# falcon-computing/bwa-flow

Measured on AMD Instinct MI355X. Metric: million reads/sec (2×150 bp PE) end-to-end align; SW-extend GCUPS at 1/2/4/8 MI355X, higher is better.
Workload: dtype int32

## Files before the change

### bwa-flow_amd/csrc/capi.hip

```cpp
#include <hip/hip_runtime.h>
#include <string.h>

#include <algorithm>
#include <chrono>
#include <cstdio>
#include <mutex>
#include <new>
#include <string>
#include <thread>
#include <vector>

#include "batch_host.h"
#include "ctx.h"
#include "engine.h"
#include "regpost.h"

using namespace bwagpu;

namespace {


__global__ void side_probe_spin(uint64_t ticks) {
  const uint64_t t0 = __builtin_amdgcn_s_memrealtime();
  while (__builtin_amdgcn_s_memrealtime() - t0 < ticks) __builtin_amdgcn_s_sleep(8);
// ... 49 lines not shown
    off[nr] = part[t];
    h_off[nr] = part[t];
  }
}

__global__ void __launch_bounds__(256) dense_copy_kernel(const bwagpu_alnreg_t* __restrict__ out,
                                                         const int32_t* __restrict__ n,
                                                         const int32_t* __restrict__ off,
                                                         const int32_t* __restrict__ rco,
                                                         const int32_t* __restrict__ cso, int nr,
                                                         bwagpu_alnreg_t* __restrict__ dense) {
  constexpr int kW = (int)(sizeof(bwagpu_alnreg_t) / 8);
  const int r = (int)((blockIdx.x * 256u + threadIdx.x) >> 4), l = (int)(threadIdx.x & 15);
  if (r >= nr) return;
  const int words = n[r] * kW;
  const uint2* src = reinterpret_cast<const uint2*>(out + cso[rco[r]]);
  uint2* dst = reinterpret_cast<uint2*>(dense + off[r]);
  for (int w = l; w < words; w += 16) dst[w] = src[w];
}

}

namespace {

bool make_opt(const bwagpu_opt_t* o, DevOpt* d, std::string* why) {
  if (!o) { *why = "opt is NULL"; return false; }
  if (o->e_del <= 0 || o->e_ins <= 0) { *why = "gap extension penalties must be > 0"; return false; }
  if (o->w < 0 || o->a < 0) { *why = "negative band width or match score"; return false; }
  if (o->a > 127 || o->e_del > 65535 || o->e_ins > 65535 || o->o_del < 0 || o->o_del > 65535 || o->o_ins < 0 ||
      o->o_ins > 65535 || o->pen_clip5 < 0 || o->pen_clip5 >= (1 << 20) || o->pen_clip3 < 0 ||
      o->pen_clip3 >= (1 << 20) || o->w > (1 << 20)) {
    *why = "scoring option out of range";
    return false;
  }
  memset(d, 0, sizeof(*d));
  d->a = o->a;
  d->o_del = o->o_del;
  d->e_del = o->e_del;
  d->o_ins = o->o_ins;
  d->e_ins = o->e_ins;
  d->oe_del = o->o_del + o->e_del;
  d->oe_ins = o->o_ins + o->e_ins;
  d->pen_clip5 = o->pen_clip5;
  d->pen_clip3 = o->pen_clip3;
  d->w = o->w;
  d->zdrop = o->zdrop;
  int mx = 0;
  for (int i = 0; i < 25; ++i) mx = std::max<int>(mx, o->mat[i]);
  d->max_mat = mx;
  d->row_bound = 1;
  memcpy(d->mat, o->mat, 25);
  for (int q = 0; q < 5; ++q) {
    uint32_t w = 0;
    for (int t = 0; t < 4; ++t) w |= (uint32_t)(uint8_t)o->mat[t * 5 + q] << (8 * t);
    d->qprof[q] = w;
    d->qprof4[q] = o->mat[20 + q];
  }
  return true;
}

int create_common(int device, const bwagpu_opt_t* opt, const bwagpu_bns_t* bns, bwagpu_ctx_t** out,
                  bwagpu_ctx_t** made) {
  if (!out || !bns || bns->l_pac <= 0 || bns->n_seqs <= 0 || !bns->ann_offset || !bns->ann_len)
    return BWAGPU_E_INVAL;
  int n = 0;
  if (hipGetDeviceCount(&n) != hipSuccess || n <= 0) return BWAGPU_E_NODEVICE;
  if (device < 0 || device >= n) return BWAGPU_E_NODEVICE;
  bwagpu_ctx_t* ctx = new (std::nothrow) bwagpu_ctx_t();
  if (!ctx) return BWAGPU_E_NOMEM;
  std::string why;
  if (!make_opt(opt, &ctx->opt, &why)) {
    delete ctx;
    return BWAGPU_E_INVAL;
  }
  ctx->device = device;
  ctx->opt_b = opt->b;
  ctx->ext_form = set_ext_form(-1);
  ctx->ext_short = ext_short_default();
  ctx->ext_short_fill = ext_short_fill_default();
  ctx->light_pack = light_pack_default();
  ctx->ungapped = ungapped_default();
  ctx->ungapped_right = ungapped_right_default();
  ctx->emu_finish = emu_finish_default();
  *made = ctx;
  HIPC(hipSetDevice(device), "hipSetDevice");
  HIPC(hipMalloc(&ctx->d_ann_off, sizeof(int64_t) * bns->n_seqs), "hipMalloc(ann_offset)");
  HIPC(hipMalloc(&ctx->d_ann_len, sizeof(int32_t) * bns->n_seqs), "hipMalloc(ann_len)");
  HIPC(hipMemcpy(ctx->d_ann_off, bns->ann_offset, sizeof(int64_t) * bns->n_seqs, hipMemcpyHostToDevice),
       "upload ann_offset");
  HIPC(hipMemcpy(ctx->d_ann_len, bns->ann_len, sizeof(int32_t) * bns->n_seqs, hipMemcpyHostToDevice),
       "upload ann_len");
  for (auto& s : ctx->slot) {
    HIPC(hipEventCreate(&s.ev0), "hipEventCreate");
    HIPC(hipEventCreate(&s.ev1), "hipEventCreate");
    HIPC(hipEventCreate(&s.ev2), "hipEventCreate");
    HIPC(hipEventCreate(&s.ev3), "hipEventCreate");
  }
  ctx->ref.l_pac = bns->l_pac;
  ctx->ref.n_seqs = bns->n_seqs;
  ctx->ref.ann_offset = ctx->d_ann_off;
  ctx->ref.ann_len = ctx->d_ann_len;
  return BWAGPU_OK;
}

std::vector<Slot*> all_slots(bwagpu_ctx_t* ctx) {
  std::vector<Slot*> v;
  for (auto& x : ctx->slot) v.push_back(&x);
  for (auto& x : ctx->dev_scratch) v.push_back(&x);
  v.push_back(&ctx->ch_slot);
  return v;
}

void destroy_ctx(bwagpu_ctx_t* ctx) {
  if (!ctx) return;
  (void)hipSetDevice(ctx->device);
  std::vector<hipStream_t> busy = ctx->side_graveyard;
  for (Slot* s : all_slots(ctx)) busy.insert(busy.end(), {s->stream, s->spec.side});
  busy.insert(busy.end(), ctx->dev_stream, ctx->dev_stream + BWAGPU_NUM_SLOTS);
  busy.insert(busy.end(), ctx->a2_st, ctx->a2_st + bwagpu_ctx::kA2Streams);
  busy.insert(busy.end(), ctx->ch_cs.side, ctx->ch_cs.side + 2);
  for (hipStream_t x : busy)
    if (x) (void)hipStreamSynchronize(x);
  if (ctx->sdh_done) (void)hipEventSynchronize(ctx->sdh_done);
  if (ctx->r2d_done && ctx->r2d_pending) (void)hipEventSynchronize(ctx->r2d_done);
  std::vector<hipStream_t> own = ctx->side_graveyard;
  own.insert(own.end(), ctx->a2_st, ctx->a2_st + bwagpu_ctx::kA2Streams);
  own.insert(own.end(), ctx->ch_cs.side, ctx->ch_cs.side + 2);
  for (hipStream_t x : own)
    if (x) (void)hipStreamDestroy(x);
  std::vector<hipEvent_t> evs = ctx->prof_ev;
  evs.insert(evs.end(), {ctx->sdh_done, ctx->r2d_done, ctx->r2d_ev[0], ctx->r2d_ev[1], ctx->a2_fork, ctx->ch_cs.fork,
                         ctx->ch_cs.join[0], ctx->ch_cs.join[1]});
  evs.insert(evs.end(), ctx->a2_join, ctx->a2_join + bwagpu_ctx::kA2Streams);
  evs.insert(evs.end(), ctx->rs_ev, ctx->rs_ev + 4 * kRescueMaxRounds);
  for (hipEvent_t e : evs)
    if (e) (void)hipEventDestroy(e);
  if (ctx->own_pac && ctx->d_pac) (void)hipFree(ctx->d_pac);
  if (ctx->d_ann_off) (void)hipFree(ctx->d_ann_off);
  if (ctx->d_ann_len) (void)hipFree(ctx->d_ann_len);
  delete ctx;
}

bool use_read_kernels() {
  const char* e = getenv("BWAGPU_C2A_PATH");
  return e && (strcmp(e, "fast") == 0 || strcmp(e, "read") == 0);
}

size_t variant_lds(const DevOpt& o, int v, int lq_max) {
  const Variant& vk = kVariants[v];
  const int lqv = std::min(lq_max, vk.max_len());
  const int tb = tb_bytes_for(o, std::max(lqv, 1));
  return vk.kind == VK_FAST ? (size_t)(kBlock / 64) * fast_wave_lds(tb) : (size_t)tb * (kBlock / vk.G);
}

}

int bwagpu::check_lds(bwagpu_ctx_t* ctx, int lq_max) {
  if (!use_read_kernels()) {
    if (spec_redo_cap(tb_bytes_for(ctx->opt, std::max(lq_max, 1))) < 64)
      return fail(ctx, BWAGPU_E_UNSUPPORTED, "LDS row buffer too large for these options (w, pen_clip, read length)");
    return BWAGPU_OK;
  }
  for (int v = 0; v < kNumVariants; ++v) {
    if (variant_lds(ctx->opt, v, lq_max) > 64 * 1024)
      return fail(ctx, BWAGPU_E_UNSUPPORTED, "LDS row buffer too large for these options (w, pen_clip, read length)");
  }
// ... 37 lines not shown
    hipStream_t c = nullptr;
    if ((e = hipStreamCreateWithFlags(&c, hipStreamNonBlocking)) != hipSuccess) break;
    bool ok = true;
    for (hipStream_t a : avoid)
      if (!streams_concurrent(c, a)) {
        ok = false;
        break;
      }
    if (ok) pick = c;
    else tried.push_back(c);
  }
  for (hipStream_t c : tried) (void)hipStreamDestroy(c);
  if (e != hipSuccess) return e;
  s.spec.side = pick;
  s.side_chosen = true;
  *snap = s.spec;
  return hipSuccess;
}

int enqueue_spec(bwagpu_ctx_t* ctx, Slot& s, const DevBatch& db, int lq_max, bwagpu_alnreg_t* d_out, int32_t* d_n,
                 int64_t* d_stats, hipStream_t st) {
  const size_t nc = (size_t)std::max(db.n_chains, 1), ns = (size_t)std::max(db.n_seeds, 1),
               nr = (size_t)std::max(db.n_reads, 1);
  const size_t n_tasks = kSpecBins * (nc + (kSpecRounds - 1) * ns);
  SpecArgs a;
  HIPC(s.d_win.get(a.win, nc), "hipMalloc(win)");
  HIPC(s.d_cread.get(a.chain_read, nc), "hipMalloc(chain_read)");
  HIPC(s.d_prog.get(a.prog, ns), "hipMalloc(prog)");
  HIPC(s.d_ext.get(a.ext, ns), "hipMalloc(ext)");
  HIPC(s.d_tasks.get(a.tasks, n_tasks), "hipMalloc(tasks)");
  HIPC(s.d_ctr.get(a.ctr, SPC_WORDS), "hipMalloc(ctr)");
  HIPC(s.d_regpos.get(a.regpos, ns), "hipMalloc(regpos)");
  HIPC(s.d_skipf.get(a.skipf, ns), "hipMalloc(skipf)");
  HIPC(s.d_heavy.get(a.heavy, nr), "hipMalloc(heavy)");
  HIPC(s.d_redo.get(a.redo, nr), "hipMalloc(redo)");
  HIPC(s.d_rbits.get(a.rbits, 2 * (nr / 32 + 1)), "hipMalloc(rbits)");
  a.fbits = a.rbits + (nr / 32 + 1);
  HIPC(s.d_rlist.get(a.rlist, nr), "hipMalloc(rlist)");
  HIPC(s.d_desc.get(a.rdesc, nr), "hipMalloc(desc)");
  HIPC(s.d_schain.get(a.seedchain, ns), "hipMalloc(seedchain)");
  HIPC(s.d_hinfo.get(a.hinfo, nr), "hipMalloc(hinfo)");
  HIPC(s.d_cov.get(a.cov, ns), "hipMalloc(cov)");
  HIPC(s.d_hflag.get(a.hflag, ns), "hipMalloc(hflag)");
  HIPC(s.d_colent.get(a.colent, ns), "hipMalloc(colent)");
  HIPC(s.d_longc.get(a.longc, nc), "hipMalloc(longc)");
  HIPC(s.d_qh.get(a.qh, kQHWords), "hipMalloc(qh)");
  HIPC(s.d_sorth.get(a.sorth, kSortWords), "hipMalloc(sorth)");
  HIPC(s.d_stasks.get(a.stasks, n_tasks), "hipMalloc(stasks)");
  HIPC(s.d_ftask.get(a.ftask, n_tasks), "hipMalloc(ftask)");
  HIPC(s.d_ftaskR.get(a.ftaskR, n_tasks), "hipMalloc(ftaskR)");
  a.ung = nullptr;
  if (ctx->ungapped && ctx->opt.row_bound) HIPC(s.d_ung.get(a.ung, n_tasks), "hipMalloc(ung)");
  a.ungt = nullptr;
  if (a.ung && ctx->ungapped_right) HIPC(s.d_ungt.get(a.ungt, n_tasks), "hipMalloc(ungt)");
  HIPC(s.d_mat.get(a.mat, (size_t)std::max<int64_t>(1 << 20, 16 * (int64_t)ns)), "hipMalloc(mat)");
  a.mat_words = (int64_t)(s.d_mat.cap / sizeof(uint64_t));
  static const int ext_prefetch = [] {
    const char* e = getenv("BWAGPU_EXT_PREFETCH");
    return e ? std::max(0, atoi(e)) : 0;
  }();
  a.ext_prefetch = ext_prefetch;
  static const int risky_first = [] {
    const char* e = getenv("BWAGPU_LIGHT_RISKY_FIRST");
    return e && e[0] == '1';
  }();
  a.risky_first = risky_first;
  static const int emu_strict = [] {
    const char* e = getenv("BWAGPU_EMU_STRICT");
    return !(e && e[0] == '0');
  }();
  a.emu_strict = emu_strict;
  a.light_pack = ctx->light_pack;
  a.emu_finish = ctx->emu_finish;
  a.out = d_out;
  a.out_n = d_n;
  a.stats = d_stats;
  SpecStreams ss;
  HIPC(choose_side(ctx, s, st, &ss), "side stream");
  a.lq_bound = lq_max;
  const int tb = tb_bytes_for(ctx->opt, std::max(lq_max, 1));
  ss.form = ctx->ext_form;
  ss.short_q = ctx->ext_short;
  ss.short_fill = ctx->ext_short_fill;
  ss.pool = ctx->prof_ev.empty() ? nullptr : ctx->prof_ev.data();
  ss.pool_n = (int)ctx->prof_ev.size();
  ss.pool_used = &ctx->prof_used;
  HIPC(launch_spec_clear(a, db.n_reads, db.n_seeds, st), "spec clear");
  HIPC(launch_spec_chain2aln(ctx->opt, ctx->ref, db, a, tb, lq_max, st, ss), "spec chain2aln launch");
  return BWAGPU_OK;
}

}

int bwagpu::enqueue_chain2aln(bwagpu_ctx_t* ctx, Slot& s, const DevBatch& db, int lq_max, bwagpu_alnreg_t* d_out,
                              int32_t* d_n, int64_t* d_stats, hipStream_t st) {
  if (!use_read_kernels()) return enqueue_spec(ctx, s, db, lq_max, d_out, d_n, d_stats, st);
  ChainWin* win = nullptr;
  bwagpu_seed_t* prog = nullptr;
  ReadDesc* desc = nullptr;
  C2AArgs a;
  HIPC(s.d_win.get(win, (size_t)db.n_chains), "hipMalloc(win)");
  HIPC(s.d_srt.get(a.srt, (size_t)db.n_seeds), "hipMalloc(srt)");
  HIPC(s.d_prog.get(prog, (size_t)db.n_seeds), "hipMalloc(prog)");
  const size_t nr = (size_t)std::max(db.n_reads, 1);
  HIPC(s.d_desc.get(desc, nr), "hipMalloc(desc)");
  HIPC(s.d_lists.ensure(2 * sizeof(int32_t) * nr), "hipMalloc(lists)");
  int32_t* bins = s.d_lists.as<int32_t>();
  int32_t* read_list = bins + nr;
  HIPC(s.d_counts.get(a.counts, kCountWords), "hipMalloc(counts)");
  HIPC(hipMemsetAsync(a.counts, 0, sizeof(int32_t) * kCountWords, st), "memset counts");
  if (db.n_reads) HIPC(hipMemsetAsync(d_n, 0, sizeof(int32_t) * db.n_reads, st), "memset out_n");
  HIPC(launch_chain_prep(ctx->opt, ctx->ref, db, win, a.srt, prog, d_stats, st), "chain_prep launch");
  HIPC(launch_read_order(db, bins, a.counts + kHistOff, a.counts, desc, read_list, d_stats, st), "read order launch");
  a.read_list = read_list;
  a.desc = desc;
  a.win = win;
  a.prog = prog;
  a.out = d_out;
  a.out_n = d_n;
  a.stats = d_stats;
  for (int v = 0; v < kNumVariants; ++v) {
    const int lqv = std::min(lq_max, kVariants[v].max_len());
    const int tb = tb_bytes_for(ctx->opt, std::max(lqv, 1));
    HIPC(launch_chain2aln(v, ctx->opt, ctx->ref, db, db.n_reads, tb, a, st), "chain2aln launch");
  }
  return BWAGPU_OK;
}

extern "C" {

int bwagpu_abi_version(void) { return BWAGPU_ABI_VERSION; }

int bwagpu_device_count(int* n) {
  if (!n) return BWAGPU_E_INVAL;
  int k = 0;
  if (hipGetDeviceCount(&k) != hipSuccess) k = 0;
  *n = k;
  return k > 0 ? BWAGPU_OK : BWAGPU_E_NODEVICE;
}

int bwagpu_create(int device, const bwagpu_opt_t* opt, const bwagpu_bns_t* bns, const uint8_t* pac_host,
                  bwagpu_ctx_t** out) {
  if (!pac_host) return BWAGPU_E_INVAL;
  bwagpu_ctx_t* ctx = nullptr;
  int rc = create_common(device, opt, bns, out, &ctx);
  if (rc == BWAGPU_OK) {
    const size_t pac_bytes = (size_t)(bns->l_pac / 4 + 1);
    hipError_t e = hipMalloc(&ctx->d_pac, pac_bytes);
    if (e == hipSuccess) {
      ctx->own_pac = true;
      e = hipMemcpy(ctx->d_pac, pac_host, pac_bytes, hipMemcpyHostToDevice);
    }
    if (e != hipSuccess) rc = hip_fail(ctx, e, "pac upload");
    ctx->ref.pac = (const uint8_t*)ctx->d_pac;
  }
  if (rc != BWAGPU_OK) {
    destroy_ctx(ctx);
    return rc;
  }
  *out = ctx;
  return BWAGPU_OK;
}

int bwagpu_create_resident(int device, const bwagpu_opt_t* opt, const bwagpu_bns_t* bns, const void* pac_device,
                           bwagpu_ctx_t** out) {
  if (!pac_device) return BWAGPU_E_INVAL;
// ... 391 lines not shown
  if (!ctx) return BWAGPU_E_INVAL;
  const int prev = ctx->ext_short;
  if (q >= 0) ctx->ext_short = q > 63 ? 63 : q;
  return prev;
}

int bwagpu_ctx_ext_short_fill(bwagpu_ctx_t* ctx, int percent) {
  if (!ctx) return BWAGPU_E_INVAL;
  const int prev = ctx->ext_short_fill;
  if (percent >= 0) ctx->ext_short_fill = percent > 100000 ? 100000 : percent;
  return prev;
}

int bwagpu_ctx_light_pack(bwagpu_ctx_t* ctx, int on) {
  if (!ctx) return BWAGPU_E_INVAL;
  const int prev = ctx->light_pack;
  if (on >= 0) ctx->light_pack = on != 0;
  return prev;
}

int bwagpu_debug_spec_short(bwagpu_ctx_t* ctx, void* stream, int64_t* out) {
  if (!ctx || !out) return BWAGPU_E_INVAL;
  int32_t c[SPC_WORDS];
  if (int rc = spec_ctr_words(ctx, stream, c)) return rc;
  out[0] = c[SPC_SHORT_N];
  for (int r = 0; r < 2; ++r) {
    const int l = r * kSpecBins;
    out[1 + 4 * r] = c[SPC_LCNT + l];
    out[2 + 4 * r] = c[SPC_LLONG + l];
    out[3 + 4 * r] = c[SPC_RCNT + l];
    out[4 + 4 * r] = c[SPC_RLONG + l];
  }
  return BWAGPU_OK;
}

int bwagpu_ctx_ungapped(bwagpu_ctx_t* ctx, int on) {
  if (!ctx) return BWAGPU_E_INVAL;
  const int prev = ctx->ungapped;
  if (on >= 0) ctx->ungapped = on ? 1 : 0;
  return prev;
}

int bwagpu_debug_spec_ungapped(bwagpu_ctx_t* ctx, void* stream, int64_t* out) {
  if (!ctx || !out) return BWAGPU_E_INVAL;
  int32_t c[SPC_WORDS];
  if (int rc = spec_ctr_words(ctx, stream, c)) return rc;
  for (int r = 0; r < kSpecRounds; ++r) {
    out[4 * r + 0] = c[SPC_UNG_N + r];
    out[4 * r + 1] = c[SPC_UNG_Q + r];
    out[4 * r + 2] = out[4 * r + 3] = 0;
    for (int bin = 0; bin < kSpecBins; ++bin) {
      out[4 * r + 2] += c[SPC_LCNT + r * kSpecBins + bin];
      out[4 * r + 3] += c[SPC_RCNT + r * kSpecBins + bin];
    }
  }
  return BWAGPU_OK;
}

int bwagpu_ctx_ungapped_right(bwagpu_ctx_t* ctx, int on) {
  if (!ctx) return BWAGPU_E_INVAL;
  const int prev = ctx->ungapped_right;
  if (on >= 0) ctx->ungapped_right = on ? 1 : 0;
  return prev;
}

int bwagpu_debug_spec_ungapped_right(bwagpu_ctx_t* ctx, void* stream, int64_t* out) {
  if (!ctx || !out) return BWAGPU_E_INVAL;
  int32_t c[SPC_WORDS];
  if (int rc = spec_ctr_words(ctx, stream, c)) return rc;
  for (int r = 0; r < kSpecRounds; ++r) {
    out[2 * r + 0] = c[SPC_UNGR_N + r];
    out[2 * r + 1] = c[SPC_UNGR_Q + r];
  }
  return BWAGPU_OK;
}

int bwagpu_ctx_emu_finish(bwagpu_ctx_t* ctx, int on) {
  if (!ctx) return BWAGPU_E_INVAL;
  const int prev = ctx->emu_finish;
  if (on >= 0) ctx->emu_finish = on ? 1 : 0;
  return prev;
}

int bwagpu_debug_spec_finish(bwagpu_ctx_t* ctx, void* stream, int64_t* out) {
  if (!ctx || !out) return BWAGPU_E_INVAL;
  int32_t c[SPC_WORDS];
  if (int rc = spec_ctr_words(ctx, stream, c)) return rc;
  out[0] = c[SPC_FIN_NAR];
  out[1] = c[SPC_FIN_WIDE];
  out[2] = c[SPC_LIST_N];
  out[3] = c[SPC_LIGHT_N];
  return BWAGPU_OK;
}

int bwagpu_ctx_row_bound(bwagpu_ctx_t* ctx, int on) {
  if (!ctx) return BWAGPU_E_INVAL;
  const int prev = ctx->opt.row_bound;
  if (on >= 0) ctx->opt.row_bound = on ? 1 : 0;
  return prev;
}

int bwagpu_debug_ext_kernel(bwagpu_ctx_t* ctx, int32_t lq_max) {
  if (!ctx || lq_max < 1 || lq_max > BWAGPU_MAX_READ_LEN) return BWAGPU_E_INVAL;
  return ext_kernel_for(ctx->opt, ctx->ext_form, tb_bytes_for(ctx->opt, lq_max));
}

int bwagpu_prof_start(bwagpu_ctx_t* ctx, int max_launches) {
  if (!ctx || max_launches < 0) return BWAGPU_E_INVAL;
  HIPC(hipSetDevice(ctx->device), "hipSetDevice");
  for (hipEvent_t e : ctx->prof_ev) HIPC(hipEventSynchronize(e), "hipEventSynchronize");
  for (hipEvent_t e : ctx->prof_ev) (void)hipEventDestroy(e);
  ctx->prof_ev.clear();
  ctx->prof_used = 0;
  for (int i = 0; i < 2 * max_launches; ++i) {
    hipEvent_t e = nullptr;
    HIPC(hipEventCreate(&e), "hipEventCreate");
    ctx->prof_ev.push_back(e);
  }
  return BWAGPU_OK;
}

int bwagpu_prof_read(bwagpu_ctx_t* ctx, double* total_ms, int32_t* launches) {
  if (!ctx || !total_ms || !launches) return BWAGPU_E_INVAL;
  HIPC(hipSetDevice(ctx->device), "hipSetDevice");
  double t = 0;
  for (int i = 0; i + 1 < ctx->prof_used; i += 2) {
    HIPC(hipEventSynchronize(ctx->prof_ev[i + 1]), "hipEventSynchronize");
    float ms = 0;
    HIPC(hipEventElapsedTime(&ms, ctx->prof_ev[i], ctx->prof_ev[i + 1]), "hipEventElapsedTime");
    t += ms;
  }
  *total_ms = t;
  *launches = ctx->prof_used / 2;
  return BWAGPU_OK;
}

int bwagpu_prof_intervals(bwagpu_ctx_t* ctx, double* start_ms, double* end_ms, int32_t max, int32_t* n) {
  if (!ctx || !n || max < 0 || (max && (!start_ms || !end_ms))) return BWAGPU_E_INVAL;
  HIPC(hipSetDevice(ctx->device), "hipSetDevice");
  int k = 0;
  for (int i = 0; i + 1 < ctx->prof_used && k < max; i += 2, ++k) {
    HIPC(hipEventSynchronize(ctx->prof_ev[i + 1]), "hipEventSynchronize");
    float a = 0, b = 0;
    HIPC(hipEventElapsedTime(&a, ctx->prof_ev[0], ctx->prof_ev[i]), "hipEventElapsedTime");
    HIPC(hipEventElapsedTime(&b, ctx->prof_ev[0], ctx->prof_ev[i + 1]), "hipEventElapsedTime");
    start_ms[k] = a;
    end_ms[k] = b;
  }
  *n = k;
  return BWAGPU_OK;
}

int bwagpu_last_stats(const bwagpu_ctx_t* ctx, int slot, bwagpu_stats_t* out) {
  if (!ctx || !out || slot < 0 || slot >= BWAGPU_NUM_SLOTS) return BWAGPU_E_INVAL;
  *out = ctx->slot[slot].last;
  return BWAGPU_OK;
}

}
```

### bwa-flow_amd/csrc/ctx.h

```cpp
#pragma once
#include <hip/hip_runtime.h>
#include <stdint.h>

#include <algorithm>
#include <atomic>
#include <chrono>
#include <mutex>
#include <string>
#include <type_traits>
#include <vector>

#include "bwagpu.h"
#include "chain.h"
#include "engine.h"
#include "rescue.h"
#include "seed.h"
#include "stage_host.h"
#include "task_host.h"

namespace bwagpu {

inline std::atomic<int64_t> g_live_bufs{0}, g_live_bytes{0};

template <bool kPinned>
// ... 31 lines not shown
      g_live_bytes.fetch_sub((int64_t)cap, std::memory_order_relaxed);
    }
    p = nullptr;
    cap = 0;
  }
  template <class T>
  T* as() const { return (T*)p; }
};
using DevBuf = GrowBuf<false>;
using HostBuf = GrowBuf<true>;
static_assert(!std::is_copy_constructible<DevBuf>::value, "a copy would free the buffer twice");

struct Slot {
  hipStream_t stream = nullptr;
  std::once_flag stream_once;
  hipError_t stream_err = hipSuccess;
  hipEvent_t ev0 = nullptr, ev1 = nullptr, ev2 = nullptr, ev3 = nullptr;
  DevBuf d_in, d_win, d_srt, d_prog, d_desc, d_out, d_n, d_stats, d_lists, d_counts;
  DevBuf d_cread, d_ext, d_tasks, d_ctr, d_regpos, d_skipf, d_heavy, d_redo, d_rbits, d_rlist;
  DevBuf d_schain, d_hinfo, d_mat, d_cov, d_hflag, d_colent, d_qh, d_longc, d_sorth, d_stasks, d_ftask, d_ftaskR, d_ung, d_ungt;
  SpecStreams spec;
  bool side_chosen = false;
  HostBuf h_in, h_out, h_n, h_stats;
  HostBuf h_dense, h_off;
  DevBuf d_off;
  size_t in_rco = 0, in_cso = 0;
  bool slot_view = false;
  bool busy = false;
  bool has_results = false;
  bool kept = false;
  std::vector<int32_t> keep_rco, keep_cso;
  int32_t n_reads = 0, n_chains = 0, n_seeds = 0;
  std::chrono::steady_clock::time_point t_submit;
  bwagpu_stats_t last{};
  int64_t h2d = 0, d2h = 0;
  ~Slot() {
    for (hipStream_t x : {stream, spec.side})
      if (x) {
        (void)hipStreamSynchronize(x);
        (void)hipStreamDestroy(x);
      }
    for (hipEvent_t e : {ev0, ev1, ev2, ev3, spec.fork, spec.join})
      if (e) (void)hipEventDestroy(e);
  }
};

inline hipError_t lazy_stream(Slot& s, hipStream_t* st) {
  std::call_once(s.stream_once, [&s] { s.stream_err = hipStreamCreateWithFlags(&s.stream, hipStreamNonBlocking); });
  *st = s.stream;
  return s.stream_err;
}

struct Staging {
  DevBuf regs, out_regs;
  DevBuf seq;
  DevBuf seq_off, reg_off, out_off;
  DevBuf n, out_n, n_pri, status, n_sw, mapq, sel;
  DevBuf pes;
};

}

struct bwagpu_ctx {
  using DevBuf = bwagpu::DevBuf;
  using HostBuf = bwagpu::HostBuf;
  using Slot = bwagpu::Slot;
  int device = 0;
  std::mutex side_mu;
  std::vector<hipStream_t> callers, side_graveyard;
  bwagpu::DevOpt opt{};
  bwagpu::DevRef ref{};
  bool own_pac = false;
  void* d_pac = nullptr;
  int64_t* d_ann_off = nullptr;
  int32_t* d_ann_len = nullptr;
  int watchdog_ms = 10000;
  int ext_form = 0;
  int ext_short = 0;
  int light_pack = 0;
  int ext_short_fill = 0;
  int ungapped = 1;
  int ungapped_right = 1;
  int emu_finish = 1;
  Slot slot[BWAGPU_NUM_SLOTS];
  hipStream_t dev_stream[BWAGPU_NUM_SLOTS] = {};
  Slot dev_scratch[BWAGPU_NUM_SLOTS];
  DevBuf ex_tasks, ex_list, ex_q, ex_t, ex_res, ex_stats;
  DevBuf a2_tasks, a2_q, a2_t, a2_out, a2_scratch, a2_lists, a2_counts, a2_boff;
  DevBuf r2_tasks, r2_q, r2_out, r2_cig, r2_md, r2_lists, r2_z, r2_stats;
  DevBuf r2d_keys, r2d_lists, r2d_tab, r2d_z, r2d_sums;
  HostBuf r2d_htab;
  hipEvent_t r2d_done = nullptr, r2d_ev[2] = {};
  bool r2d_pending = false, r2d_timing = false, r2d_timed = false;
  double r2d_wait_ms = 0, r2d_call_ms = 0;
  int32_t r2d_jobs = 0;
  static constexpr int kA2Streams = 4;
  hipStream_t a2_st[kA2Streams] = {};
  hipEvent_t a2_fork = nullptr, a2_join[kA2Streams] = {};
  DevBuf bwt_words, sa_d, sa_in, sa_out, occ_d, sup_d, sa_full;
  bwagpu::DevBwt bwt{};
  bool has_bwt = false;
  DevBuf sd_off, sd_seq, sd_out, sd_n, sd_scratch, sd_poff, sd_pack, sd_heavy, sd_dbg;
  DevBuf ch_npos, ch_posoff, ch_frac, ch_nout, ch_noseed, ch_nsw, ch_need, ch_swtab, ch_alt;
  DevBuf ch_kpos, ch_rbeg, ch_qinfo, ch_label, ch_score, ch_slist, ch_ord, ch_chains, ch_nodes;
  DevBuf ch_ochains, ch_oslist, ch_bins, ch_dbg;
  DevBuf ch_swoff, ch_swtasks, ch_swt, ch_swskip, ch_swres, ch_swscr;
  DevBuf ch_ocoff, ch_osoff, ch_rco, ch_cso, ch_rid, ch_cfrac, ch_out, ch_seeds;
  DevBuf ch_regoff, ch_regc;
  HostBuf chh_tot, chh_rco, chh_cso, chh_chains, chh_seeds, chh_regs, chh_n;
  HostBuf sdh_in;
  hipEvent_t sdh_done = nullptr;
  Slot ch_slot;
  bwagpu::ChainStreams ch_cs{};
  bool has_alt = false;
  bwagpu::Staging stg;
  int opt_b = 0;
  bwagpu_postopt_t post_opt{};
  int32_t post_flags = 0;
  int64_t post_id0 = 0;
  DevBuf rp_stats;
  DevBuf pe_isize, pe_cnt;
  DevBuf rs_pair, rs_soff, rs_tab, rs_toff, rs_boff, rs_qpool, rs_ctr, rs_scr;
  DevBuf rs_tasks[bwagpu::kRescueMaxRounds], rs_tpool[bwagpu::kRescueMaxRounds], rs_res[bwagpu::kRescueMaxRounds];
  int32_t rescue_drop = 0;
  hipEvent_t rs_ev[4 * bwagpu::kRescueMaxRounds] = {};
  int rs_ev_rounds = 0;
  hipStream_t rs_ev_stream = nullptr;
  DevBuf ps_scratch, ps_log, ps_erfc;
  bool ps_log_ready = false;
  DevBuf st_buf, st_start, st_q, st_tasks, st_lists, st_seen, st_ctr, st_out;
  int seed_budget = 1024;
  int sup_shift = 32;
  int dev_read_len = BWAGPU_MAX_READ_LEN;
  int fail_after = -1, fail_code = 0;
  std::vector<hipEvent_t> prof_ev;
  int prof_used = 0;
  std::string err;
};

namespace bwagpu {

inline int fail(bwagpu_ctx_t* c, int code, const std::string& msg) {
  if (c) c->err = msg;
  return code;
}

inline int hip_fail(bwagpu_ctx_t* c, hipError_t e, const char* what) {
  std::string m = std::string(what) + ": " + hipGetErrorString(e);
  if (e == hipErrorOutOfMemory || e == hipErrorMemoryAllocation) return fail(c, BWAGPU_E_NOMEM, m);
  return fail(c, BWAGPU_E_DEVICE, m);
}

#define HIPC(call, what)                             \
  do {                                               \
    hipError_t e_ = (call);                          \
    if (e_ != hipSuccess) return hip_fail(ctx, e_, what); \
  } while (0)
#define TRY(call)                     \
  do {                                \
    if (int rc_ = (call)) return rc_; \
  } while (0)

inline int refuse(bwagpu_ctx_t* c, int code, const char* why) { return why && *why ? fail(c, code, why) : code; }

inline int entry_stream(bwagpu_ctx_t* ctx, void* stream, hipStream_t* st) {
  HIPC(hipSetDevice(ctx->device), "hipSetDevice");
// ... 130 lines not shown
```

### bwa-flow_amd/csrc/engine.h

```cpp
#pragma once
#include <hip/hip_runtime.h>
#include <stdint.h>

#include "bwagpu.h"
#include "bwagpu_debug.h"
#include "pure.h"
#include "spec_plan.h"
#include "ungapped.h"

namespace bwagpu {

struct ReadDesc {
  int64_t qoff;
  int32_t rd;
  int32_t lq;
  int32_t c0;
  int32_t nch;
  int32_t s0;
  int32_t ns;
};

struct ChainWin {
  int64_t lo, hi;
};
// ... 17 lines not shown
  const int32_t* ann_len;
};

enum { ST_CELLS = 0, ST_ROWS = 1, ST_CALLS = 2, ST_ERR = 3, ST_N = 4 };
enum { ERR_RID = 1, ERR_LEN = 2, ERR_A2_RANGE = 4 };

constexpr int kFastMaxSeeds = 32;
constexpr int kFastMaxChains = 32;
constexpr int kSeqLds = 256;
constexpr int kNumVariants = 3;
extern const Variant kVariants[kNumVariants];
constexpr int kHistOff = 128;
constexpr int kCountWords = kHistOff + kNumVariants * 256;

hipError_t launch_chain_prep(const DevOpt& o, const DevRef& ref, const DevBatch& b, ChainWin* win, uint64_t* srt,
                             bwagpu_seed_t* prog, int64_t* stats, hipStream_t st);
hipError_t launch_read_order(const DevBatch& b, int32_t* bins, int32_t* hist, int32_t* counts, ReadDesc* desc,
                             int32_t* list, int64_t* stats, hipStream_t st);
struct C2AArgs {
  const int32_t* read_list;
  const ReadDesc* desc;
  int32_t* counts;
  const ChainWin* win;
  uint64_t* srt;
  const bwagpu_seed_t* prog;
  bwagpu_alnreg_t* out;
  int32_t* out_n;
  int64_t* stats;
};
hipError_t launch_chain2aln(int variant, const DevOpt& o, const DevRef& ref, const DevBatch& b, int32_t max_list,
                            int tb_bytes, const C2AArgs& a, hipStream_t st);
size_t fast_wave_lds(int tb);

hipError_t launch_extend(int variant, bool t5, const DevOpt& o, int32_t n_tasks,
                         const bwagpu_ext_task_t* tasks, const int32_t* task_list, int32_t n_list,
                         const uint8_t* qpool, const uint8_t* tpool, int tb_bytes,
                         bwagpu_ext_result_t* res, int64_t* stats, hipStream_t st);
hipError_t launch_extend4(const DevOpt& o, const bwagpu_ext_task_t* tasks, const int32_t* task_list, int32_t n_list,
                          const uint8_t* qpool, const uint8_t* tpool, int tb_bytes, bwagpu_ext_result_t* res,
                          int64_t* stats, hipStream_t st);

struct SeedExt {
  int64_t rb, re;
  int32_t qb, qe, score, truesc, w;
  int32_t cells, rows, calls;
};

constexpr int kSpecRounds = 3;
constexpr int kOrderLane = 8;
constexpr int kSelLight = 64;
constexpr int kSelRegLds = 256;
constexpr int kSelMatMaxSeeds = 4096;
enum {
  SPC_CNT = 0,
  SPC_HEAVY_N = 16,
  SPC_SEL_CUR = 17,
  SPC_REDO_N = 20,
  SPC_SPEC64 = 24,
  SPC_MISS = 26,
  SPC_MATW64 = 28,
  SPC_HCOLS = 30,
  SPC_LONG_N = 31,
  SPC_LCNT = 64,
  SPC_RCNT = 73,
  SPC_LIGHT_CUR = 82,
  SPC_LLONG = 84,
  SPC_RLONG = 93,
  SPC_SHORT_N = 102,
  SPC_UNG_N = 103,
  SPC_UNG_Q = 106,
  SPC_FIN_NAR = 109,
  SPC_FIN_WIDE = 110,
  SPC_LIST_N = 111,
  SPC_LIGHT_N = 112,
  SPC_UNGR_N = 113,
  SPC_UNGR_Q = 116,
  SPC_WORDS = 128
};
constexpr int kQHStride = 32;
constexpr int kQHShort = 2 * kSpecRounds * kSpecBins * 8 * kQHStride;
constexpr int kQHWords = 2 * kQHShort;
constexpr int kSortKeys = 1024;
constexpr int kSortWordsR = kSpecRounds * 2 * kSortKeys;
constexpr int kSortWords = 2 * kSortWordsR;
__host__ __device__ inline size_t spec_list_off(int list, int n_chains, int n_seeds) {
  const int round = list / kSpecBins, bin = list % kSpecBins;
  return round == 0 ? (size_t)bin * n_chains
                    : (size_t)kSpecBins * n_chains + ((size_t)(round - 1) * kSpecBins + bin) * n_seeds;
}
struct FatTask {
  int64_t rbeg, qoff;
  int32_t pos;
  int32_t dlo, dhi;
  uint32_t qls;
};
static_assert(sizeof(FatTask) == 32, "FatTask layout");
static_assert(BWAGPU_MAX_READ_LEN < 1024, "FatTask packs qbeg / len / lq in 10 bits each");
struct UngRec {
  struct Side {
    int32_t ok;
    UngappedSide s;
  } side[2];
};
static_assert(sizeof(UngRec) == 32, "UngRec layout");
struct UngTask {
  int64_t rbeg;
  int32_t pos;
  uint32_t qls;
};
static_assert(sizeof(UngTask) == 16, "UngTask layout");
struct SpecArgs {
  int lq_bound;
  ChainWin* win;
  int32_t* chain_read;
  bwagpu_seed_t* prog;
  SeedExt* ext;
  int2* tasks;
  int32_t* ctr;
  int32_t* regpos;
  int32_t* skipf;
  int32_t* heavy;
  int32_t* redo;
  uint32_t* rbits;
  uint32_t* fbits;
  int32_t* rlist;
  ReadDesc* rdesc;
  int32_t* seedchain;
  int4* hinfo;
  int32_t* colent;
  int32_t* longc;
  uint64_t* mat;
  int64_t mat_words;
  int32_t* cov;
  int32_t* hflag;
  int32_t* qh;
  int32_t* sorth;
  int2* stasks;
  FatTask* ftask;
  FatTask* ftaskR;
  UngRec* ung;
  UngTask* ungt;
  int risky_first;
  int emu_strict;
  int light_pack;
  int emu_finish;
  int ext_prefetch;
  bwagpu_alnreg_t* out;
  int32_t* out_n;
  int64_t* stats;
};
struct SpecStreams {
  hipStream_t side = nullptr;
  hipEvent_t fork = nullptr, join = nullptr;
  hipEvent_t* pool = nullptr;
  int pool_n = 0;
  int* pool_used = nullptr;
  int form = 0;
  int short_q = 0;
  int short_fill = 0;
};
int ungapped_default();
int ungapped_right_default();
int emu_finish_default();
int set_ext_form(int form);
int ext_short_default();
int ext_short_fill_default();
int light_pack_default();
int ext_kernel_for(const DevOpt& o, int form, int tb_bytes);
hipError_t launch_spec_clear(const SpecArgs& a, int n_reads, int n_seeds, hipStream_t st);
hipError_t launch_spec_chain2aln(const DevOpt& o, const DevRef& ref, const DevBatch& b, const SpecArgs& a,
                                 int tb_bytes, int lq_max, hipStream_t st, const SpecStreams& ss);
size_t spec_select_lds(int tb_bytes);
int spec_redo_cap(int tb_bytes);

struct StreamTask {
  bwagpu_seed_t s;
  int64_t lo, hi;
  int64_t qoff;
  int32_t lq, pad_;
};
enum { STR_ERR_RECORD = 1, STR_ERR_TASK = 2, STR_ERR_DUP = 4, STR_ERR_SEED = 8, STR_ERR_BASE = 16 };
enum { kStrDecoded = 4, kStrMax = 5, kStrErr = 6, kStrHeads = 64 };
constexpr int kStrCtrWords = kStrHeads + kSpecBins * 8 * kQHStride;
struct StreamArgs {
  const int32_t* buf;
  const int64_t* rstart;
  int32_t n_reads, cap;
  int64_t l_pac;
  uint8_t* qpool;
  StreamTask* tasks;
  int32_t* lists;
  int32_t* seen;
  int32_t* ctr;
  int32_t* out;
};
hipError_t launch_sw_stream(const DevOpt& o, const DevRef& ref, const StreamArgs& a, int tb_bytes, hipStream_t st);

hipError_t set_trace(void* dev_ptr);
hipError_t set_trace_spec(void* dev_ptr);

}
```

### bwa-flow_amd/csrc/spec.hip

```cpp
#include "spec_dev.h"

namespace bwagpu {

__device__ uint32_t* g_trace = nullptr;
hipError_t set_trace_spec(void* p) { return hipMemcpyToSymbol(HIP_SYMBOL(g_trace), &p, sizeof(p)); }


__global__ void __launch_bounds__(256) spec_chain_kernel(DevOpt o, DevRef ref, DevBatch b, SpecArgs a) {
  sel_prio();
  const int c = blockIdx.x * blockDim.x + threadIdx.x;
  bool task = false, longc = false;
  int bin = 0, s0 = 0;
  if (c < b.n_chains) {
    const int rd = a.chain_read[c];
    s0 = b.chain_seed_off[c];
    const int ns = b.chain_seed_off[c + 1] - s0;
    const int lq = (int)(b.seq_off[rd + 1] - b.seq_off[rd]);
    if (ns <= 0) {
      a.win[c] = ChainWin{0, 0};
    } else {
      int64_t wlo = ref.l_pac << 1, whi = 0;
      longc = ns > kOrderLane;
      if (!longc) {
        uint64_t key[kOrderLane];
// ... 811 lines not shown
enum { SEL_EMULATE = 0, SEL_FINAL = 1, SEL_REDO = 2 };
struct RegRec {
  int64_t rb, re;
  int32_t qb, qe, w, seedlen0;
};
constexpr int kSelHeavyLds = 64 * 1024;
constexpr int kSelExtCache = 256;
__host__ __device__ constexpr int sel_light_wave_lds() { return kSelLight * (int)sizeof(RegRec); }
__host__ __device__ constexpr int sel_heavy_cap(int mode, int tb) {
  return (kSelHeavyLds - 4 * (BWAGPU_MAX_READ_LEN + 1) - kSelExtCache * (int)(sizeof(SeedExt) + sizeof(bwagpu_seed_t)) -
          (mode == SEL_REDO ? 2 * tb : 0)) / (int)sizeof(RegRec);
}

constexpr int kMglN = BWAGPU_MAX_READ_LEN + 1;

__device__ __forceinline__ bool seed_near(const int32_t* MG, const bwagpu_seed_t& s, const RegRec& p) {
  const int qd1 = s.qbeg - p.qb;
  const int64_t rd1 = s.rbeg - p.rb;
  const int g1 = MG[min(max(qd1 < rd1 ? qd1 : (int)rd1, 0), kMglN - 1)];
  const int bw1 = g1 < p.w ? g1 : p.w;
  const int qd2 = p.qe - (s.qbeg + s.len);
  const int64_t rd2 = p.re - (s.rbeg + s.len);
  const int g2 = MG[min(max(qd2 < rd2 ? qd2 : (int)rd2, 0), kMglN - 1)];
  const int bw2 = g2 < p.w ? g2 : p.w;
  return (qd1 - rd1 < bw1 && rd1 - qd1 < bw1) || (qd2 - rd2 < bw2 && rd2 - qd2 < bw2);
}

__device__ __forceinline__ void write_region(bwagpu_alnreg_t* dst, const SeedExt& e, int rid, int cov, int slen,
                                             float frac) {
  const int r = (int)(threadIdx.x & 63);
  const int dw = r < 21 ? r : 21;
  uint32_t v = 0;
  v = dw == 0 ? (uint32_t)e.rb : v;
  v = dw == 1 ? (uint32_t)((uint64_t)e.rb >> 32) : v;
  v = dw == 2 ? (uint32_t)e.re : v;
  v = dw == 3 ? (uint32_t)((uint64_t)e.re >> 32) : v;
  v = dw == 4 ? (uint32_t)e.qb : v;
  v = dw == 5 ? (uint32_t)e.qe : v;
  v = dw == 6 ? (uint32_t)rid : v;
  v = dw == 7 ? (uint32_t)e.score : v;
  v = dw == 8 ? (uint32_t)e.truesc : v;
  v = dw == 13 ? (uint32_t)e.w : v;
  v = dw == 14 ? (uint32_t)cov : v;
  v = dw == 17 ? (uint32_t)slen : v;
  v = dw == 19 ? __float_as_uint(frac) : v;
  reinterpret_cast<uint32_t*>(dst)[dw] = v;
}

__device__ __forceinline__ void put_regrec(RegRec* dst, const SeedExt& e, int slen) {
  const int r = (int)(threadIdx.x & 63);
  const int f = r < 8 ? r : 7;
  int32_t v = 0;
  v = f == 0 ? (int32_t)(uint32_t)e.rb : v;
  v = f == 1 ? (int32_t)((uint64_t)e.rb >> 32) : v;
  v = f == 2 ? (int32_t)(uint32_t)e.re : v;
  v = f == 3 ? (int32_t)((uint64_t)e.re >> 32) : v;
  v = f == 4 ? e.qb : v;
  v = f == 5 ? e.qe : v;
  v = f == 6 ? e.w : v;
  v = f == 7 ? slen : v;
  if (r < 8) reinterpret_cast<int32_t*>(dst)[f] = v;
  __builtin_amdgcn_fence(__ATOMIC_RELEASE, "wavefront");
  __builtin_amdgcn_wave_barrier();
  __builtin_amdgcn_fence(__ATOMIC_ACQUIRE, "wavefront");
}

__device__ __forceinline__ void trace_read(int pass, int n_reads, int rd, uint64_t t0, int ns, int nreg, int shape) {
  uint32_t* const tr = g_trace;
  if (!tr) return;
  const uint64_t t1 = __builtin_amdgcn_s_memrealtime();
  const int r = (int)(threadIdx.x & 63);
  const int d = r < 7 ? r : 7;
  uint32_t v = (uint32_t)shape;
  v = d == 0 ? (uint32_t)t0 : v;
  v = d == 1 ? (uint32_t)(t0 >> 32) : v;
  v = d == 2 ? (uint32_t)t1 : v;
  v = d == 3 ? (uint32_t)(t1 >> 32) : v;
  v = d == 4 ? (uint32_t)ns : v;
  v = d == 5 ? (uint32_t)nreg : v;
  v = d == 6 ? __builtin_amdgcn_s_getreg((31 << 11) | 20) : v;
  if (r < 8) tr[((size_t)pass * n_reads + rd) * 8 + d] = v;
}

template <int MODE, bool HEAVY>
__global__ void __launch_bounds__(64) spec_select_kernel(DevOpt o, DevRef ref, DevBatch b, SpecArgs a, int tb_bytes) {
  sel_prio();
  static_assert(HEAVY, "one-wave heavy shape only");
  constexpr bool WRITE = MODE != SEL_EMULATE;
  extern __shared__ __attribute__((aligned(16))) uint8_t lds[];
  const int r = (int)(threadIdx.x & 63);
  int32_t* const MG = reinterpret_cast<int32_t*>(lds);
  bwagpu_seed_t* const SC = reinterpret_cast<bwagpu_seed_t*>(lds + 4 * kMglN);
  SeedExt* const EC = reinterpret_cast<SeedExt*>(SC + kSelExtCache);
  RegRec* const R = reinterpret_cast<RegRec*>(EC + kSelExtCache);
  const int cap_reg = sel_heavy_cap(MODE, tb_bytes);
  uint8_t* const tbl = reinterpret_cast<uint8_t*>(R + cap_reg);
  uint8_t* const tbr = tbl + tb_bytes;
  for (int x = r; x < kMglN; x += 64) MG[x] = max_gap_len(o, x);
  Tally tl{0, 0, 0};
  const int n_list = uni(__hip_atomic_load(&a.ctr[MODE == SEL_REDO ? SPC_REDO_N : SPC_HEAVY_N], __ATOMIC_RELAXED,
                                           __HIP_MEMORY_SCOPE_AGENT));
  const int32_t* const hlist = MODE == SEL_REDO ? a.redo : a.heavy;
  for (;;) {
    int t = 0;
    if (r == 0) t = atomicAdd(&a.ctr[SPC_SEL_CUR + MODE], 1);
    t = uni(__shfl(t, 0, 64));
    if (t >= n_list) break;
    if (MODE != SEL_REDO && uni(a.hinfo[t].y) >= 0) continue;
    const int rd = uni(hlist[t]);
    const uint64_t t_start = g_trace ? __builtin_amdgcn_s_memrealtime() : 0;
    const ReadDesc d = uniform_desc(a.rdesc[rd]);
    if (d.lq > a.lq_bound) continue;
    const uint8_t* const q = b.seq + d.qoff;
    const int rep_lim = (int)floor(.1 * d.lq) + 1;
    bool redo = false;
    Tally rt{0, 0, 0};
    int nreg = 0, n_inline = 0;
    for (int c = d.c0; c < d.c0 + d.nch && !redo; ++c) {
      const int s0 = uni(b.chain_seed_off[c]), ns = uni(b.chain_seed_off[c + 1]) - s0;
      if (ns == 0) continue;
      ChainWin cw = a.win[c];
      cw.lo = uni64(cw.lo);
      cw.hi = uni64(cw.hi);
      if (cw.hi < cw.lo) continue;
      const int rid = uni(b.chain_rid[c]);
      const float frac = __int_as_float(uni(__float_as_int(b.chain_frac_rep[c])));
      const bool big = ns > kSelExtCache;
      for (int i = r; i < min(ns, kSelExtCache); i += 64) {
        bwagpu_seed_t v = a.prog[s0 + i];
        v.pad_ = v.pad_ != 0 ? 1 : 0;
        SC[i] = v;
        const uint32_t* src = reinterpret_cast<const uint32_t*>(a.ext + s0 + i);
        uint32_t* dst = reinterpret_cast<uint32_t*>(EC + i);
#pragma unroll
        for (int w = 0; w < 12; ++w) dst[w] = __hip_atomic_load(src + w, __ATOMIC_RELAXED, __HIP_MEMORY_SCOPE_WORKGROUP);
      }
      if (big)
        for (int i = r; i < ns; i += 64)
          __hip_atomic_store(&a.skipf[s0 + i], a.prog[s0 + i].pad_ != 0 ? 1 : 0, __ATOMIC_RELAXED,
                             __HIP_MEMORY_SCOPE_WORKGROUP);
      mem_fence_group();
      auto seed_at = [&](int i) -> bwagpu_seed_t { return i < kSelExtCache ? SC[i] : a.prog[s0 + i]; };
      auto flag_at = [&](int i) -> int {
        return i < kSelExtCache ? SC[i].pad_
                                : __hip_atomic_load(&a.skipf[s0 + i], __ATOMIC_RELAXED, __HIP_MEMORY_SCOPE_WORKGROUP);
      };
      auto set_flag = [&](int i, int f) {
        if (r == 0) {
          if (i < kSelExtCache) SC[i].pad_ |= f;
          else __hip_atomic_store(&a.skipf[s0 + i], f | 0, __ATOMIC_RELAXED, __HIP_MEMORY_SCOPE_WORKGROUP);
        }
        mem_fence_group();
      };
      for (int k = 0; k < ns; ++k) {
        const bwagpu_seed_t s = uni_seed(seed_at(k));
        bool hit = false;
        for (int base = 0; base < nreg && !hit; base += 64) {
          const int i = min(base + r, nreg - 1);
          RegRec p;
          if (i < cap_reg) {
            p = R[i];
          } else {
            const int pp = __hip_atomic_load(&a.regpos[d.s0 + i], __ATOMIC_RELAXED, __HIP_MEMORY_SCOPE_WORKGROUP);
            const SeedExt* pe = a.ext + pp;
            p.rb = __hip_atomic_load(&pe->rb, __ATOMIC_RELAXED, __HIP_MEMORY_SCOPE_WORKGROUP);
            p.re = __hip_atomic_load(&pe->re, __ATOMIC_RELAXED, __HIP_MEMORY_SCOPE_WORKGROUP);
            p.qb = __hip_atomic_load(&pe->qb, __ATOMIC_RELAXED, __HIP_MEMORY_SCOPE_WORKGROUP);
            p.qe = __hip_atomic_load(&pe->qe, __ATOMIC_RELAXED, __HIP_MEMORY_SCOPE_WORKGROUP);
            p.w = __hip_atomic_load(&pe->w, __ATOMIC_RELAXED, __HIP_MEMORY_SCOPE_WORKGROUP);
            p.seedlen0 = a.prog[pp].len;
          }
          const bool inside = base + r < nreg &&
                              !(s.rbeg < p.rb || s.rbeg + s.len > p.re || s.qbeg < p.qb || s.qbeg + s.len > p.qe) &&
                              !(s.len - p.seedlen0 >= rep_lim);
          if (__builtin_amdgcn_ballot_w64(inside) == 0) continue;
          hit = __builtin_amdgcn_ballot_w64(inside && seed_near(MG, s, p)) != 0;
        }
        if (hit) {
          const int len95 = uni((int)ceil(s.len * .95));
          bool ov = false;
          for (int base = 0; base < k && !ov; base += 64) {
            const int i = min(base + r, k - 1);
            const bwagpu_seed_t t = seed_at(i);
            const bool tsk = (flag_at(i) & 1) != 0;
            const bool a1 = s.qbeg <= t.qbeg && s.qbeg + s.len - t.qbeg >= s.len >> 2 && (int64_t)(t.qbeg - s.qbeg) != t.rbeg - s.rbeg;
            const bool b1 = t.qbeg <= s.qbeg && t.qbeg + t.len - s.qbeg >= s.len >> 2 && (int64_t)(s.qbeg - t.qbeg) != s.rbeg - t.rbeg;
            ov = __builtin_amdgcn_ballot_w64(base + r < k && !tsk && t.len >= len95 && (a1 || b1)) != 0;
          }
          if (!ov) {
            set_flag(k, 1);
            continue;
          }
        }
        const int pos = s0 + k;
        const SeedExt* const pe = k < kSelExtCache ? EC + k : a.ext + pos;
        SeedExt e;
        e.calls = uni(__hip_atomic_load(&pe->calls, __ATOMIC_RELAXED, __HIP_MEMORY_SCOPE_WORKGROUP));
        if (e.calls == 0) {
          if constexpr (MODE == SEL_REDO) {
            e = extend_seed<16>(o, ref, s, d.lq, q, cw, tbl, tbr);
            store_ext(a.ext + pos, e);
            mem_fence_group();
            if (r == 0) atomicAdd(&a.ctr[SPC_MISS], 1);
            ++n_inline;
          } else if constexpr (MODE == SEL_EMULATE) {
            set_flag(k, 2);
            continue;
          } else {
            const int list = 2 * kSpecBins + spec_bin(d.lq);
            if (r == 0) {
              const int p = atomicAdd(&a.ctr[SPC_CNT + list], 1);
              a.tasks[spec_list_off(list, b.n_chains, b.n_seeds) + p] = make_int2(pos, c);
              a.redo[atomicAdd(&a.ctr[SPC_REDO_N], 1)] = rd;
            }
            redo = true;
            break;
          }
        } else {
          e.rb = uni64(__hip_atomic_load(&pe->rb, __ATOMIC_RELAXED, __HIP_MEMORY_SCOPE_WORKGROUP));
          e.re = uni64(__hip_atomic_load(&pe->re, __ATOMIC_RELAXED, __HIP_MEMORY_SCOPE_WORKGROUP));
          e.qb = uni(__hip_atomic_load(&pe->qb, __ATOMIC_RELAXED, __HIP_MEMORY_SCOPE_WORKGROUP));
          e.qe = uni(__hip_atomic_load(&pe->qe, __ATOMIC_RELAXED, __HIP_MEMORY_SCOPE_WORKGROUP));
          e.score = uni(__hip_atomic_load(&pe->score, __ATOMIC_RELAXED, __HIP_MEMORY_SCOPE_WORKGROUP));
          e.truesc = uni(__hip_atomic_load(&pe->truesc, __ATOMIC_RELAXED, __HIP_MEMORY_SCOPE_WORKGROUP));
          e.w = uni(__hip_atomic_load(&pe->w, __ATOMIC_RELAXED, __HIP_MEMORY_SCOPE_WORKGROUP));
          e.cells = uni(__hip_atomic_load(&pe->cells, __ATOMIC_RELAXED, __HIP_MEMORY_SCOPE_WORKGROUP));
          e.rows = uni(__hip_atomic_load(&pe->rows, __ATOMIC_RELAXED, __HIP_MEMORY_SCOPE_WORKGROUP));
        }
        if constexpr (WRITE) {
          long long cov = 0;
          for (int base = 0; base < ns; base += 64) {
            const int i = base + r;
            const bwagpu_seed_t t = seed_at(min(i, ns - 1));
            const bool in = i < ns && t.qbeg >= e.qb && t.qbeg + t.len <= e.qe && t.rbeg >= e.rb && t.rbeg + t.len <= e.re;
            cov += in ? t.len : 0;
          }
          cov = grp_sum64(cov, 64);
          write_region(a.out + d.s0 + nreg, e, rid, (int)cov, s.len, frac);
          rt.cells += e.cells;
          rt.rows += e.rows;
          rt.calls += e.calls - 1;
        }
        if (nreg < cap_reg) {
          put_regrec(R + nreg, e, s.len);
        } else {
          if (r == 0) __hip_atomic_store(&a.regpos[d.s0 + nreg], pos, __ATOMIC_RELAXED, __HIP_MEMORY_SCOPE_WORKGROUP);
          mem_fence_group();
        }
        ++nreg;
      }
      if constexpr (MODE == SEL_EMULATE) {
        const int list = kSpecBins + spec_bin(d.lq);
        for (int base = 0; base < ns; base += 64) {
          const int i = base + r;
          const bool pnd = i < ns && (flag_at(min(i, ns - 1)) & 2) != 0;
          const int p = wave_append(&a.ctr[SPC_CNT + list], pnd);
          if (p >= 0) a.tasks[spec_list_off(list, b.n_chains, b.n_seeds) + p] = make_int2(s0 + i, c);
        }
      }
    }
    trace_read(MODE, b.n_reads, rd, t_start, d.ns, nreg, 2 | (MODE == SEL_REDO ? n_inline << 4 : 0));
    if constexpr (WRITE) {
      if (!redo) {
        a.out_n[rd] = nreg;
        tl.cells += rt.cells;
        tl.rows += rt.rows;
        tl.calls += rt.calls;
      }
    }
  }
  if constexpr (WRITE) {
    if (r != 0) tl = Tally{0, 0, 0};
    block_stats<64>(tl, a.stats);
  }
}

#ifndef BWAGPU_LIGHT_INLINE
#define BWAGPU_LIGHT_INLINE 1
#endif
template <int MODE>
__device__ __forceinline__ bool light_read(const DevOpt& o, const DevRef& ref, const DevBatch& b, const SpecArgs& a,
                                           const int32_t* MG, uint8_t* tbl, uint8_t* tbr, int rd, const ReadDesc& d,
                                           Tally& tl) {
  constexpr bool WRITE = MODE != SEL_EMULATE;
  const int r = (int)(threadIdx.x & 63);
  const uint64_t lt_mask = r ? (~0ull >> (64 - r)) : 0ull;
  const uint64_t t_start = g_trace ? __builtin_amdgcn_s_memrealtime() : 0;
  bool finished = false;
    for (;;) {
    const int ci = min(r, max(d.nch - 1, 0)), si = min(r, d.ns - 1);
    const int cs_l = b.chain_seed_off[d.c0 + ci] - d.s0, ce_l = b.chain_seed_off[d.c0 + ci + 1] - d.s0;
    const ChainWin cw_l = a.win[d.c0 + ci];
    const int rid_l = b.chain_rid[d.c0 + ci];
    const float fr_l = b.chain_frac_rep[d.c0 + ci];
    const bwagpu_seed_t sd = a.prog[d.s0 + si];
    const SeedExt x = a.ext[d.s0 + si];
    int cid = 0, rid = 0;
    float frac = 0.f;
    bool vchain = false;
    for (int c = 0; c < d.nch; ++c) {
      const int cs = __builtin_amdgcn_readlane(cs_l, c), ce = __builtin_amdgcn_readlane(ce_l, c);
      const bool in = r >= cs && r < ce;
      const bool ok = readlane64(cw_l.hi, c) >= readlane64(cw_l.lo, c);
      cid = in ? c : cid;
      vchain = in ? ok : vchain;
      rid = in ? __builtin_amdgcn_readlane(rid_l, c) : rid;
      frac = in ? __int_as_float(__builtin_amdgcn_readlane(__float_as_int(fr_l), c)) : frac;
    }
    const bool present = r < d.ns && vchain;
    const bool computed = present && x.calls != 0;
    const uint64_t present_m = __builtin_amdgcn_ballot_w64(present);
    const uint64_t computed_m = __builtin_amdgcn_ballot_w64(computed);
    const uint64_t pad_m = __builtin_amdgcn_ballot_w64(r < d.ns && sd.pad_ != 0);
    const int rep_lim = (int)floor(.1 * d.lq) + 1;
    const int S = d.ns <= 8 ? 8 : d.ns <= 16 ? 16 : d.ns <= 32 ? 32 : 64;
    const int lgS = S == 8 ? 3 : S == 16 ? 4 : S == 32 ? 5 : 6;
    const int npass = (S * S) >> 6;
    uint32_t c_lo = 0, c_hi = 0, o_lo = 0, o_hi = 0;
    int cov = 0;
    const int j = r & (S - 1);
    const int jl = min(j, d.ns - 1) << 2;
    const int64_t j_rbeg = (int64_t)((uint64_t)(uint32_t)__builtin_amdgcn_ds_bpermute(jl, (int)(sd.rbeg >> 32)) << 32 |
                                     (uint32_t)__builtin_amdgcn_ds_bpermute(jl, (int)sd.rbeg));
    const int j_qbeg = __builtin_amdgcn_ds_bpermute(jl, sd.qbeg), j_len = __builtin_amdgcn_ds_bpermute(jl, sd.len);
    const int j_cid = __builtin_amdgcn_ds_bpermute(jl, cid);
    const bool j_pad = __builtin_amdgcn_ds_bpermute(jl, sd.pad_) != 0;
    const bool j_done = __builtin_amdgcn_ds_bpermute(jl, computed ? 1 : 0) != 0;
    RegRec pj;
    pj.rb = (int64_t)((uint64_t)(uint32_t)__builtin_amdgcn_ds_bpermute(jl, (int)(x.rb >> 32)) << 32 |
                      (uint32_t)__builtin_amdgcn_ds_bpermute(jl, (int)x.rb));
    pj.re = (int64_t)((uint64_t)(uint32_t)__builtin_amdgcn_ds_bpermute(jl, (int)(x.re >> 32)) << 32 |
                      (uint32_t)__builtin_amdgcn_ds_bpermute(jl, (int)x.re));
    pj.qb = __builtin_amdgcn_ds_bpermute(jl, x.qb);
    pj.qe = __builtin_amdgcn_ds_bpermute(jl, x.qe);
    pj.w = __builtin_amdgcn_ds_bpermute(jl, x.w);
    pj.seedlen0 = j_len;
    for (int it = 0; it < npass; ++it) {
      const int k = (it << (6 - lgS)) + (r >> lgS);
      const int kl = min(k, d.ns - 1) << 2;
      bwagpu_seed_t sk;
      sk.rbeg = (int64_t)((uint64_t)(uint32_t)__builtin_amdgcn_ds_bpermute(kl, (int)(sd.rbeg >> 32)) << 32 |
                          (uint32_t)__builtin_amdgcn_ds_bpermute(kl, (int)sd.rbeg));
      sk.qbeg = __builtin_amdgcn_ds_bpermute(kl, sd.qbeg);
      sk.len = __builtin_amdgcn_ds_bpermute(kl, sd.len);
      const int k_cid = __builtin_amdgcn_ds_bpermute(kl, cid);
      const bool valid = k < d.ns && j < d.ns;
      const bool inside = valid && j < k && j_done &&
                          !(sk.rbeg < pj.rb || sk.rbeg + sk.len > pj.re || sk.qbeg < pj.qb || sk.qbeg + sk.len > pj.qe) &&
                          !(sk.len - j_len >= rep_lim);
      uint64_t cm = __builtin_amdgcn_ballot_w64(inside);
      if (cm) cm = __builtin_amdgcn_ballot_w64(inside && seed_near(MG, sk, pj));
      const int len95 = (int)ceil(sk.len * .95);
// ... 484 lines not shown
      if (MODE == SEL_EMULATE) {
        const bool a1 = s.qbeg <= sc.qbeg && s.qbeg + s.len - sc.qbeg >= s.len >> 2 &&
                        (int64_t)(sc.qbeg - s.qbeg) != sc.rbeg - s.rbeg;
        const bool b1 = sc.qbeg <= s.qbeg && sc.qbeg + sc.len - s.qbeg >= s.len >> 2 &&
                        (int64_t)(s.qbeg - sc.qbeg) != s.rbeg - sc.rbeg;
        const uint64_t om =
            __builtin_amdgcn_ballot_w64(j < k && cc == ck && sc.pad_ == 0 && sc.len >= len95 && (a1 || b1));
        if (r == 0) a.mat[woff + tri_off(ns) + tri_off(k) + w] = om;
      }
      if (k_cov)
        cov += (j < ns && cc == ck && sc.qbeg >= kqb && sc.qbeg + sc.len <= kqe && sc.rbeg >= krb &&
                sc.rbeg + sc.len <= kre) ? sc.len : 0;
    }
    if (k_cov) {
      for (int w = nlow; w < nw; ++w) {
        const int j = 64 * w + r, jj = min(j, ns - 1);
        const bwagpu_seed_t sc = a.prog[d.s0 + jj];
        const int cc = a.seedchain[d.s0 + jj];
        cov += (j < ns && cc == ck && sc.qbeg >= kqb && sc.qbeg + sc.len <= kqe && sc.rbeg >= krb &&
                sc.rbeg + sc.len <= kre) ? sc.len : 0;
      }
      cov = (int)grp_sum64(cov, 64);
      if (r == 0) a.cov[d.s0 + k] = cov;
    } else if (MODE == SEL_EMULATE) {
      if (r == 0) a.cov[d.s0 + k] = -1;
    }
    hi = hin;
  }
}

__device__ __forceinline__ uint64_t lane64(uint64_t v, int l) { return (uint64_t)readlane64((int64_t)v, l); }

constexpr int kScanLds = 64 * 1024;

__device__ __forceinline__ void heavy_fill_missing(const DevOpt& o, const DevRef& ref, const DevBatch& b,
                                                   const SpecArgs& a, const ReadDesc& d, int k, int ns,
                                                   uint64_t* C, uint8_t* tbl, uint8_t* tbr) {
  const int r = (int)(threadIdx.x & 63);
  const bwagpu_seed_t sk = uni_seed(a.prog[d.s0 + k]);
  const int ck = uni(a.seedchain[d.s0 + k]);
  ChainWin cw = a.win[ck];
  cw.lo = uni64(cw.lo);
  cw.hi = uni64(cw.hi);
  const SeedExt e = d.lq <= 192 ? extend_seed<3>(o, ref, sk, d.lq, b.seq + d.qoff, cw, tbl, tbr)
                                 : extend_seed<4>(o, ref, sk, d.lq, b.seq + d.qoff, cw, tbl, tbr);
  store_ext(a.ext + d.s0 + k, e);
  if (r == 0) atomicAdd(&a.ctr[SPC_MISS], 1);
  RegRec p;
  p.rb = e.rb;
  p.re = e.re;
  p.qb = e.qb;
  p.qe = e.qe;
  p.w = e.w;
  p.seedlen0 = sk.len;
  const int rep_lim = (int)floor(.1 * d.lq) + 1;
  int cov = 0;
  for (int base = 0; base < ns; base += 64) {
    const int j = base + r, jj = min(j, ns - 1);
    const bwagpu_seed_t sj = a.prog[d.s0 + jj];
    bool in = j > k && j < ns && !(sj.rbeg < p.rb || sj.rbeg + sj.len > p.re || sj.qbeg < p.qb || sj.qbeg + sj.len > p.qe) &&
              !(sj.len - sk.len >= rep_lim);
    if (in) {
      const int qd1 = sj.qbeg - p.qb;
      const int64_t rd1 = sj.rbeg - p.rb;
      const int g1 = max_gap_len(o, max(qd1 < rd1 ? qd1 : (int)rd1, 0));
      const int bw1 = g1 < p.w ? g1 : p.w;
      const int qd2 = p.qe - (sj.qbeg + sj.len);
      const int64_t rd2 = p.re - (sj.rbeg + sj.len);
      const int g2 = max_gap_len(o, max(qd2 < rd2 ? qd2 : (int)rd2, 0));
      const int bw2 = g2 < p.w ? g2 : p.w;
      in = (qd1 - rd1 < bw1 && rd1 - qd1 < bw1) || (qd2 - rd2 < bw2 && rd2 - qd2 < bw2);
    }
    if (in) C[tri_off(j) + (k >> 6)] |= 1ull << (k & 63);
    const int cj = a.seedchain[d.s0 + jj];
    cov += (j < ns && cj == ck && sj.qbeg >= p.qb && sj.qbeg + sj.len <= p.qe && sj.rbeg >= p.rb &&
            sj.rbeg + sj.len <= p.re) ? sj.len : 0;
  }
  cov = (int)grp_sum64(cov, 64);
  if (r == 0) a.cov[d.s0 + k] = cov;
  __builtin_amdgcn_fence(__ATOMIC_SEQ_CST, "workgroup");
  __builtin_amdgcn_wave_barrier();
}

template <int MODE>
__global__ void __launch_bounds__(64) spec_scan_kernel(DevOpt o, DevRef ref, DevBatch b, SpecArgs a, int tb_bytes) {
  sel_prio();
  constexpr bool WRITE = MODE != SEL_EMULATE;
  extern __shared__ __attribute__((aligned(16))) uint64_t M[];
  uint8_t* const tbl = reinterpret_cast<uint8_t*>(M) + kScanLds;
  uint8_t* const tbr = tbl + tb_bytes;
  const int r = (int)(threadIdx.x & 63);
  const uint64_t lt_mask = r ? (~0ull >> (64 - r)) : 0ull;
  const int nh = uni(__hip_atomic_load(&a.ctr[SPC_HEAVY_N], __ATOMIC_RELAXED, __HIP_MEMORY_SCOPE_AGENT));
  Tally tl{0, 0, 0};
  for (int t = (int)blockIdx.x; t < nh; t += (int)gridDim.x) {
    const int4 hi = a.hinfo[t];
    const int rd = uni(hi.x), woff = uni(hi.y), ns = uni(hi.w);
    if (woff < 0) continue;
    const uint64_t t_start = g_trace ? __builtin_amdgcn_s_memrealtime() : 0;
    const int nw = (ns + 63) >> 6;
    const ReadDesc d = uniform_desc(a.rdesc[rd]);
    if (d.lq > a.lq_bound) continue;
    const int64_t tw = tri_off(ns);
    const uint64_t* Cg = a.mat + woff;
    const bool staged = 2 * tw * 8 <= kScanLds;
    if (staged) {
      for (int i = r; i < 2 * tw; i += 64) M[i] = Cg[i];
      __builtin_amdgcn_fence(__ATOMIC_RELEASE, "wavefront");
      __builtin_amdgcn_wave_barrier();
      __builtin_amdgcn_fence(__ATOMIC_ACQUIRE, "wavefront");
    }
    uint64_t* C = staged ? M : a.mat + woff;
    const uint64_t* O = C + tw;
    uint64_t present_w = 0, computed_w = 0, skip_w = 0;
    for (int w = 0; w < nw; ++w) {
      const int j = 64 * w + r;
      const int f = j < ns ? a.hflag[d.s0 + j] : 0;
      const uint64_t pm = __builtin_amdgcn_ballot_w64(f & 1);
      const uint64_t cm = __builtin_amdgcn_ballot_w64((f & 3) == 3);
      const uint64_t km = __builtin_amdgcn_ballot_w64(f & 4);
      present_w = r == w ? pm : present_w;
      computed_w = r == w ? cm : computed_w;
      skip_w = r == w ? km : skip_w;
    }
    uint64_t ext_w = 0, pend_w = 0, unc_w = 0;
    const bool strict = MODE == SEL_EMULATE && a.emu_strict;
    int fp = ns;
    int miss = -1;
    for (int bw = 0; bw < nw && miss < 0; ++bw) {
      const int kb = 64 * bw, k = kb + r;
      const bool valid = k < ns;
      const int64_t row = tri_off(valid ? k : ns - 1);
      bool cb = false, cbc = false;
      for (int w = 0; w < bw; ++w) {
        const uint64_t x = C[row + w] & lane64(ext_w, w);
        cb |= x != 0;
        if (strict) cbc |= (x & ~lane64(unc_w, w)) != 0;
      }
      uint64_t cin = valid && r > 0 ? C[row + bw] : 0;
      bool need = valid && (cb || cin != 0), ob = false, ou = false;
      uint64_t oin = 0;
      if (__builtin_amdgcn_ballot_w64(need)) {
        if (need) {
          for (int w = 0; w < bw; ++w) {
            const uint64_t x = O[row + w];
            ob |= (x & ~lane64(skip_w, w)) != 0;
            if (strict) ou |= (x & lane64(unc_w, w)) != 0;
          }
          oin = r > 0 ? O[row + bw] : 0;
        }
      }
      const uint64_t pres = lane64(present_w, bw);
      uint64_t comp = lane64(computed_w, bw), skp = lane64(skip_w, bw), ext = 0, pend = 0, spend = 0;
      uint64_t uncb = 0;
      const int nb = min(64, ns - kb);
      bool resolved = false;
      {
        const uint64_t skp0 = skp;
        const bool prs = (pres >> r) & 1, cmp = (comp >> r) & 1;
        const bool cb_k = valid && cb, ob_k = valid && ob, cbc_k = valid && cbc, ou_k = valid && ou;
        uint64_t e = 0, sk = skp0, pn = 0, sp = 0, un = 0, lack = 0;
        for (int it = 0; it <= nb + 1; ++it) {
          bool is_skip = false, is_ext = false, is_pend = false, is_spend = false, is_unc = false, is_lack = false;
          if (prs) {
            if ((cb_k || (cin & e)) && !ob_k && !(oin & ~sk)) {
              is_skip = true;
              if (strict && (!(cbc_k || (cin & e & ~un)) || ou_k || (oin & un))) {
                is_unc = true;
                is_spend = !cmp;
              }
            } else if (!cmp) {
              if (MODE == SEL_EMULATE) is_pend = is_unc = true;
              else is_lack = true;
            } else {
              is_ext = true;
              is_unc = strict && (fp < k || (pn & lt_mask));
            }
// ... 96 lines not shown
          const int p = atomicAdd(&a.ctr[SPC_CNT + list], 1);
          a.tasks[spec_list_off(list, b.n_chains, b.n_seeds) + p] = make_int2(d.s0 + miss, a.seedchain[d.s0 + miss]);
          a.redo[atomicAdd(&a.ctr[SPC_REDO_N], 1)] = rd;
        }
        continue;
      }
      for (int w = 0; w < nw; ++w) {
        const uint64_t ew = (uint64_t)__builtin_amdgcn_readlane((uint32_t)(ext_w >> 32), w) << 32 |
                            (uint32_t)__builtin_amdgcn_readlane((uint32_t)ext_w, w);
        const int j = 64 * w + r;
        if ((ew >> r) & 1) {
          const int slot = nreg + (int)__popcll(ew & lt_mask);
          const SeedExt x = a.ext[d.s0 + j];
          const int c = a.seedchain[d.s0 + j];
          uint2* dst = reinterpret_cast<uint2*>(a.out + d.s0 + slot);
          dst[0] = make_uint2((uint32_t)x.rb, (uint32_t)((uint64_t)x.rb >> 32));
          dst[1] = make_uint2((uint32_t)x.re, (uint32_t)((uint64_t)x.re >> 32));
          dst[2] = make_uint2((uint32_t)x.qb, (uint32_t)x.qe);
          dst[3] = make_uint2((uint32_t)b.chain_rid[c], (uint32_t)x.score);
          dst[4] = make_uint2((uint32_t)x.truesc, 0u);
          dst[5] = make_uint2(0u, 0u);
          dst[6] = make_uint2(0u, (uint32_t)x.w);
          dst[7] = make_uint2((uint32_t)a.cov[d.s0 + j], 0u);
          dst[8] = make_uint2(0u, (uint32_t)a.prog[d.s0 + j].len);
          dst[9] = make_uint2(0u, __float_as_uint(b.chain_frac_rep[c]));
          dst[10] = make_uint2(0u, 0u);
          tl.cells += x.cells;
          tl.rows += x.rows;
          tl.calls += x.calls - 1;
        }
        nreg += (int)__popcll(ew);
      }
      if (r == 0) a.out_n[rd] = nreg;
    }
    trace_read(MODE, b.n_reads, rd, t_start, ns, nreg, 3);
  }
  if constexpr (WRITE) block_stats<64>(tl, a.stats);
}

constexpr int kScanGrid = 1024;

#ifndef BWAGPU_LIGHT_PACK_DEFAULT
#define BWAGPU_LIGHT_PACK_DEFAULT 1
#endif
int light_pack_default() {
  static const int v = [] {
    const char* e = getenv("BWAGPU_LIGHT_PACK");
    return e && e[0] ? (atoi(e) != 0 ? 1 : 0) : BWAGPU_LIGHT_PACK_DEFAULT;
  }();
  return v;
}
#ifndef BWAGPU_LIGHT_PACK_WGS_DEFAULT
#define BWAGPU_LIGHT_PACK_WGS_DEFAULT 2
#endif
static int light_pack_wgs() {
  static const int v = [] {
    const char* e = getenv("BWAGPU_LIGHT_PACK_WGS");
    return std::min(std::max(e && e[0] ? atoi(e) : BWAGPU_LIGHT_PACK_WGS_DEFAULT, 1), 64);
  }();
  return v;
}
#ifndef BWAGPU_LIGHT_LIST_DIV_DEFAULT
#define BWAGPU_LIGHT_LIST_DIV_DEFAULT 4
#endif
static int light_list_div() {
  static const int v = [] {
    const char* e = getenv("BWAGPU_LIGHT_LIST_DIV");
    return std::min(std::max(e && e[0] ? atoi(e) : BWAGPU_LIGHT_LIST_DIV_DEFAULT, 1), 64);
  }();
  return v;
}
static int device_cus() {
  int dev = 0, ncu = 0;
  if (hipGetDevice(&dev) != hipSuccess ||
      hipDeviceGetAttribute(&ncu, hipDeviceAttributeMultiprocessorCount, dev) != hipSuccess || ncu < 1)
    return 256;
  return ncu;
}

template <int MODE>
static void launch_select(const DevOpt& o, const DevRef& ref, const DevBatch& b, const SpecArgs& a, int tb_bytes,
                          hipStream_t st, const SpecStreams& ss) {
  hipStream_t hs = st;
  if (MODE != SEL_REDO && ss.side) {
    (void)hipEventRecord(ss.fork, st);
    (void)hipStreamWaitEvent(ss.side, ss.fork, 0);
    hs = ss.side;
  }
  if (MODE != SEL_REDO) {
    const size_t lds = BWAGPU_LIGHT_INLINE && MODE == SEL_FINAL ? (size_t)(kBlock / 64) * 2 * tb_bytes : 0;
    int nb = resident_blocks(spec_select_light<MODE>, lds);
    if (a.light_pack && !(MODE == SEL_FINAL && a.risky_first)) {
      const int octets = (b.n_reads + kPackW - 1) / kPackW, per_wg = kBlock / 64;
      nb = std::min(nb, std::max(1, std::min((octets + per_wg - 1) / per_wg, light_pack_wgs() * device_cus())));
      if (MODE == SEL_FINAL && a.emu_finish) nb = std::max(1, nb / light_list_div());
    }
    hipLaunchKernelGGL((spec_select_light<MODE>), dim3(nb), dim3(kBlock), lds, st, o, ref, b, a, tb_bytes);
  }
  if (MODE != SEL_REDO) {
    const int nb = resident_blocks(spec_pairs_kernel<MODE>, 0);
    hipLaunchKernelGGL((spec_pairs_kernel<MODE>), dim3(nb), dim3(kBlock), 0, hs, o, b, a);
    hipLaunchKernelGGL((spec_scan_kernel<MODE>), dim3(kScanGrid), dim3(64), (size_t)kScanLds + 2 * (size_t)tb_bytes, hs, o,
                       ref, b, a, tb_bytes);
  }
  hipLaunchKernelGGL((spec_select_kernel<MODE, true>), dim3(MODE == SEL_REDO ? 256 : 1024), dim3(64),
                     (size_t)kSelHeavyLds, hs, o, ref, b, a, tb_bytes);
  if (hs != st) {
    (void)hipEventRecord(ss.join, hs);
    (void)hipStreamWaitEvent(st, ss.join, 0);
  }
}

static std::atomic<int> g_ext_form{0};
int ext_kernel_for(const DevOpt& o, int form, int tb_bytes) { return ext_plan(o, form, tb_bytes, 0).bin[0].code; }
int set_ext_form(int form) {
  const int prev = g_ext_form.load(std::memory_order_relaxed);
  if (form >= 0) g_ext_form.store(form > 2 ? 1 : form, std::memory_order_relaxed);
  return prev;
}

#ifndef BWAGPU_EXT_SHORT_Q_DEFAULT
#define BWAGPU_EXT_SHORT_Q_DEFAULT 63
#endif
int ext_short_default() {
  static const int q = [] {
    const char* e = getenv("BWAGPU_EXT_SHORT_Q");
    const int v = e && e[0] ? atoi(e) : BWAGPU_EXT_SHORT_Q_DEFAULT;
    return std::min(std::max(v, 0), kShortQMax);
  }();
  return q;
}
#ifndef BWAGPU_EXT_SHORT_FILL_DEFAULT
#define BWAGPU_EXT_SHORT_FILL_DEFAULT 150
#endif
int ungapped_default() {
  static const int on = [] {
    const char* e = getenv("BWAGPU_UNGAPPED");
    return !(e && e[0] == '0');
  }();
  return on;
}
int ungapped_right_default() {
  static const int on = [] {
    const char* e = getenv("BWAGPU_UNGAPPED_RIGHT");
    return !(e && e[0] == '0');
  }();
  return on;
}
int emu_finish_default() {
  static const int on = [] {
    const char* e = getenv("BWAGPU_EMU_FINISH");
    return !(e && e[0] == '0');
  }();
  return on;
}
int ext_short_fill_default() {
  static const int f = [] {
    const char* e = getenv("BWAGPU_EXT_SHORT_FILL");
    return std::min(std::max(e && e[0] ? atoi(e) : BWAGPU_EXT_SHORT_FILL_DEFAULT, 0), 100000);
  }();
  return f;
}


static void launch_sort(const ExtBin& k, const ExtRound& r, int bin0, int nbins, int short_q, int short_fill) {
  if (k.phased) launch_side_sort(r, bin0, nbins, short_q, short_fill);
  else launch_task_sort(r, bin0, nbins);
}
static void launch_ext_bin(const ExtBin& k, const ExtRound& r, int list, const ExtPlan& p, int short_fill) {
  if (k.family == SIDE4) launch_side_bin(k, r, list, p, short_fill);
  else launch_task_bin(k, r, list, p.quad);
}

static void launch_ext_round(const DevOpt& o, const DevRef& ref, const DevBatch& b, const SpecArgs& a, int round,
                             int tb_bytes, int lq_max, hipStream_t st, const SpecStreams& ss) {
  const int l = round * kSpecBins;
  const bool bin1 = lq_max > kSpecBinLen[0], bin2 = lq_max > kSpecBinLen[1];
  const ExtPlan plan = ext_plan(o, ss.form, tb_bytes, ss.short_q);
  const ExtRound r{o, ref, b, a, round, tb_bytes, st};
  if (!bin1 || plan.bin[0].phased == plan.bin[1].phased) {
    launch_sort(plan.bin[0], r, 0, bin1 ? 2 : 1, plan.short_q, ss.short_fill);
  } else {
    launch_sort(plan.bin[0], r, 0, 1, plan.short_q, ss.short_fill);
    launch_sort(plan.bin[1], r, 1, 1, 0, ss.short_fill);
  }
  const bool prof = ss.pool && *ss.pool_used + 2 <= ss.pool_n;
  if (prof) (void)hipEventRecord(ss.pool[*ss.pool_used], st);
  launch_ext_bin(plan.bin[0], r, l + 0, plan, ss.short_fill);
  if (prof) {
    (void)hipEventRecord(ss.pool[*ss.pool_used + 1], st);
    *ss.pool_used += 2;
  }
  if (!bin1) return;
  launch_ext_bin(plan.bin[1], r, l + 1, plan, ss.short_fill);
  if (bin2) launch_task_long(r, l + 2);
}

hipError_t launch_spec_chain2aln(const DevOpt& o, const DevRef& ref, const DevBatch& b, const SpecArgs& a,
                                 int tb_bytes, int lq_max, hipStream_t st, const SpecStreams& ss) {
  if (b.n_reads == 0) return hipSuccess;
  hipLaunchKernelGGL(spec_reads_kernel, dim3((b.n_reads + 255) / 256), dim3(256), 0, st, b, a);
  if (b.n_chains) {
    hipLaunchKernelGGL(spec_chain_kernel, dim3((b.n_chains + 255) / 256), dim3(256), 0, st, o, ref, b, a);
    hipLaunchKernelGGL(spec_order_kernel, dim3(kOrderBlocks), dim3(256), 0, st, o, ref, b, a);
  }
  if (b.n_chains) {
    launch_ext_round(o, ref, b, a, 0, tb_bytes, lq_max, st, ss);
    launch_select<SEL_EMULATE>(o, ref, b, a, tb_bytes, st, ss);
    launch_ext_round(o, ref, b, a, 1, tb_bytes, lq_max, st, ss);
  }
  SpecArgs af = a;
  if (!b.n_chains) af.emu_finish = 0;
  launch_select<SEL_FINAL>(o, ref, b, af, tb_bytes, st, ss);
  if (b.n_chains && lq_max > kSpecBinLen[0] && !a.emu_strict) launch_ext_round(o, ref, b, a, 2, tb_bytes, lq_max, st, ss);
  if (b.n_chains) launch_select<SEL_REDO>(o, ref, b, a, tb_bytes, st, ss);
  return hipGetLastError();
}

__global__ void __launch_bounds__(256) spec_clear_kernel(SpecArgs a, int nr, int ns) {
  const int t0 = (int)(blockIdx.x * 256 + threadIdx.x), nt = (int)(gridDim.x * 256);
  switch (blockIdx.y) {
    case 0:
      for (int i = t0; i < 3 * ns; i += nt) reinterpret_cast<uint4*>(a.ext)[i] = make_uint4(0, 0, 0, 0);
      break;
    case 1:
      for (int i = t0; i < nr; i += nt) a.out_n[i] = 0;
      break;
    case 2:
      for (int i = t0; i < nr / 32 + 1; i += nt) a.rbits[i] = a.fbits[i] = 0;
      break;
    case 3:
      for (int i = t0; i < kQHWords; i += nt) a.qh[i] = 0;
      break;
    case 4:
      for (int i = t0; i < kSortWords; i += nt) a.sorth[i] = 0;
      break;
    default:
      for (int i = t0; i < SPC_WORDS; i += nt) a.ctr[i] = 0;
  }
}
static_assert(sizeof(SeedExt) == 48, "spec_clear_kernel clears SeedExt as three uint4");

hipError_t launch_spec_clear(const SpecArgs& a, int n_reads, int n_seeds, hipStream_t st) {
  hipLaunchKernelGGL(spec_clear_kernel, dim3(256, 6), dim3(256), 0, st, a, n_reads, n_seeds);
  return hipGetLastError();
}

size_t spec_select_lds(int tb_bytes) { return (size_t)kSelHeavyLds + 0 * tb_bytes; }
int spec_redo_cap(int tb_bytes) { return sel_heavy_cap(SEL_REDO, tb_bytes); }

}
```

### bwa-flow_amd/csrc/spec_dev.h

```cpp
#pragma once
#include "ksw_dev.h"

namespace bwagpu {

__device__ __forceinline__ void sel_prio() { __builtin_amdgcn_s_setprio(3); }

__host__ __device__ inline int64_t tri_off(int k) {
  if (k <= 1) return 0;
  const int64_t q = (k - 1) >> 6;
  return 32 * q * (q + 1) + (int64_t)(k - 1 - 64 * q) * (q + 1);
}

template <int G = 32>
__device__ __forceinline__ void fill_two_half(uint8_t* tbl, int64_t x0l, int nl, uint8_t* tbr, int64_t x0r, int nr,
                                              const DevRef& ref) {
  const int r = (int)(threadIdx.x & (G - 1));
  const int64_t two1 = (ref.l_pac << 1) - 1;
  const int n = max(nl, nr);
  for (int base = 0; base < n; base += 4 * G) {
    uint32_t raw[8];
    int sh[8], kk[8];
    bool rev[8];
#pragma unroll
    for (int m = 0; m < 8; ++m) {
// ... 70 lines not shown
    fill_two_half<G>(tbl, x0l, nl, tbr, x0r, nr, ref);
    return;
  }
  const int r = (int)(threadIdx.x & (G - 1));
  const int64_t pac_bytes = (ref.l_pac >> 2) + 1;
  const int k0 = r * R;
  fill_side_run<G>(tbl, x0l, -1, k0, min(k0 + R, nl), ref, pac_bytes);
  fill_side_run<G>(tbr, x0r, 1, k0, min(k0 + R, nr), ref, pac_bytes);
  __builtin_amdgcn_fence(__ATOMIC_RELEASE, "wavefront");
  __builtin_amdgcn_wave_barrier();
  __builtin_amdgcn_fence(__ATOMIC_ACQUIRE, "wavefront");
}

template <int G = 32>
__device__ __forceinline__ void store_ext_half(SeedExt* dst, const SeedExt& e) {
  static_assert(G >= 12 || G == 8, "a SeedExt is 12 words");
  const int d = (int)(threadIdx.x & (G - 1));
  const uint32_t* w = reinterpret_cast<const uint32_t*>(&e);
  uint32_t v = 0;
#pragma unroll
  for (int k = 0; k < 12; ++k) v = d == k ? w[k] : v;
  if constexpr (G == 8) {
    reinterpret_cast<uint32_t*>(dst)[d] = v;
    uint32_t u = 0;
#pragma unroll
    for (int k = 0; k < 4; ++k) u = d == k ? w[8 + k] : u;
    if (d < 4) reinterpret_cast<uint32_t*>(dst)[8 + d] = u;
  } else {
    if (d < 12) reinterpret_cast<uint32_t*>(dst)[d] = v;
  }
}

#ifdef BWAGPU_OCC_DIAG
template <int G>
__device__ __forceinline__ void occ_diag(unsigned long long* acc, const QCall& ca, const QCall& cb, const Tally32& ta,
                                         const Tally32& tb) {
  int qm = 0, rm = 0;
  long long lr = 0, lq = 0, cc = 0;
#pragma unroll
  for (int g = 0; g < 64; g += G) {
    const int qa = __builtin_amdgcn_readlane(ca.qlen, g), qb = __builtin_amdgcn_readlane(cb.qlen, g);
    const int ra = __builtin_amdgcn_readlane(ta.rows, g), rb = __builtin_amdgcn_readlane(tb.rows, g);
    qm = max(qm, max(qa, qb));
    rm = max(rm, max(ra, rb));
    lr += ra + rb;
    lq += (long long)ra * (qa + 1) + (long long)rb * (qb + 1);
    cc += __builtin_amdgcn_readlane(ta.cells, g) + __builtin_amdgcn_readlane(tb.cells, g);
  }
  const int cpl = (qm + G) / G;
  acc[0] += 1ull;
  acc[1] += (unsigned long long)rm;
  acc[2] += (unsigned long long)rm * (2 * 64 / G);
  acc[3] += (unsigned long long)lr;
  acc[4] += (unsigned long long)rm * 128ull * cpl;
  acc[5] += (unsigned long long)lr * G * cpl;
  acc[6] += (unsigned long long)lq;
  acc[7] += (unsigned long long)cc;
}
#endif

__device__ __forceinline__ FatTask fat_task(const DevBatch& b, const SpecArgs& a, int2 tk) {
  const bwagpu_seed_t sd = a.prog[tk.x];
  const ChainWin cw = a.win[tk.y];
  const int rd = a.chain_read[tk.y];
  FatTask f;
  f.rbeg = sd.rbeg;
  f.qoff = b.seq_off[rd];
  f.pos = tk.x;
  f.dlo = (int32_t)(sd.rbeg - cw.lo);
  f.dhi = (int32_t)(cw.hi - sd.rbeg);
  const int lq = (int)(b.seq_off[rd + 1] - f.qoff);
  f.qls = (uint32_t)sd.qbeg | (uint32_t)sd.len << 10 | (uint32_t)lq << 20;
  return f;
}


struct ExtRound {
  const DevOpt& o;
  const DevRef& ref;
  const DevBatch& b;
  const SpecArgs& a;
  int round, tb_bytes;
  hipStream_t st;
};
int ext2_grid(int nb, bool packed);
void launch_side_sort(const ExtRound& r, int bin0, int nbins, int short_q, int short_fill);
void launch_side_bin(const ExtBin& k, const ExtRound& r, int list, const ExtPlan& p, int short_fill);
constexpr int ext_key(int family, int g, int pmax, bool k8) { return ((family * 64 + g) * 32 + pmax) * 2 + (k8 ? 1 : 0); }

}
```

### bwa-flow_amd/csrc/spec_side.hip

```cpp
#include "spec_dev.h"

namespace bwagpu {

__device__ __forceinline__ int side_key(int qlen) { return 255 - min(qlen, 255); }


struct UngSide {
  const uint8_t* rd;
  int64_t x0;
  int p0, d, qlen, lq;
};
__device__ __forceinline__ UngSeg ung_pass(const UngSide& s, const DevRef& ref, int base, const int8_t* mat,
                                           const int8_t* mat8, int max_mat) {
  const int last = min(base + 15, s.qlen - 1), cnt = last - base + 1;
  const int64_t two1 = (ref.l_pac << 1) - 1, pac_bytes = (ref.l_pac >> 2) + 1;
  const int64_t xa = s.x0 + (int64_t)s.d * base, xb = s.x0 + (int64_t)s.d * last;
  const bool rev = xa >= ref.l_pac;
  const int64_t fa = rev ? two1 - xa : xa, fb = rev ? two1 - xb : xb;
  UngSeg g;
  if (s.lq >= 16 && pac_bytes >= 8 && (xb >= ref.l_pac) == rev) {
    const int qa = s.p0 + s.d * base;
    const int ws = min(max(min(qa, qa + 15 * s.d), 0), s.lq - 16);
    const int64_t b0 = min(min(fa, fb) >> 2, pac_bytes - 8);
    uint64_t q[2], tw;
    __builtin_memcpy(q, s.rd + ws, 16);
    __builtin_memcpy(&tw, ref.pac + b0, 8);
    uint64_t lo = q[0], hi = q[1];
    int sh = qa - ws;
    if (s.d < 0) {
      lo = __builtin_bswap64(q[1]);
      hi = __builtin_bswap64(q[0]);
      sh = 15 - sh;
    }
    if (sh >= 8) {
      lo = hi;
      hi = 0;
    }
    const int sb = (sh & 7) * 8;
    if (sb) {
      lo = (lo >> sb) | (hi << (64 - sb));
      hi >>= sb;
    }
    constexpr uint64_t k7f = 0x7f7f7f7f7f7f7f7full, k80 = 0x8080808080808080ull, k04 = 0x0404040404040404ull,
                       k05 = 0x0505050505050505ull;
    uint64_t ge = ((((lo & k7f) + (k7f - k04)) | lo) & k80) >> 7;
    lo = (lo & ~(ge * 255)) | (ge * 4);
    ge = ((((hi & k7f) + (k7f - k04)) | hi) & k80) >> 7;
    hi = (hi & ~(ge * 255)) | (ge * 4);
    if (cnt < 8) lo = (lo & ~(~0ull << (8 * cnt))) | (k05 << (8 * cnt));
    if (cnt <= 8) hi = k05;
    else if (cnt < 16) hi = (hi & ~(~0ull << (8 * (cnt - 8)))) | (k05 << (8 * (cnt - 8)));
    const uint64_t T = __builtin_bswap64(tw);
    const int f0 = (int)(fa - (b0 << 2));
    uint32_t w;
    if ((s.d > 0) != rev) {
      w = __builtin_bitreverse32((uint32_t)((T << (2 * f0)) >> 32));
      w = ((w & 0x55555555u) << 1) | ((w >> 1) & 0x55555555u);
    } else {
      w = (uint32_t)(T >> (62 - 2 * f0));
    }
    if (rev) w = ~w;
    const uint32_t qw[4] = {(uint32_t)lo, (uint32_t)(lo >> 32), (uint32_t)hi, (uint32_t)(hi >> 32)};
    int c = 0, key = 31;
#pragma unroll
    for (int m = 0; m < 16; ++m) {
      const uint32_t qv = (qw[m >> 2] >> ((m & 3) * 8)) & 255u, tv = (w >> (2 * m)) & 3u;
      c += mat8[(tv << 3) | qv];
      key = max(key, c * 32 + 30 - m);
    }
    g.n = cnt;
    g.c = c;
    g.P = cnt * max_mat - c;
    g.M = key >> 5;
    g.am = 31 - (key & 31);
  } else {
    for (int j = base; j <= last; ++j)
      g = ungseg_combine(g, ungseg_base(mat[pac_base2(ref.pac, ref.l_pac, s.x0 + (int64_t)s.d * j) * 5 +
                                            min((int)s.rd[s.p0 + s.d * j], 4)], max_mat));
  }
  return g;
}

constexpr int kUngTasks = 128;
constexpr int kUngPassCap = 256 * 9;
struct UngSeg16 {
  int16_t c, P, M, am;
};

__global__ void __launch_bounds__(256) spec_ungapped_kernel(DevOpt o, DevRef ref, DevBatch b, SpecArgs a, int round,
                                                            int bin0, int keep_short) {
  sel_prio();
  __shared__ int8_t mat[25], mat8[32];
  __shared__ UngSide sd[256];
  __shared__ uint32_t plist[kUngPassCap];
  __shared__ UngSeg16 seg[kUngPassCap];
  __shared__ int wsum[4], listed;
  const int tid = (int)threadIdx.x;
  if (tid < 25) mat[tid] = o.mat[tid];
  if (tid < 32) mat8[tid] = (tid & 7) < 5 ? o.mat[(tid >> 3) * 5 + (tid & 7)] : 0;
  if (tid == 0) listed = 0;
  __syncthreads();
  const int bin = bin0 + (int)blockIdx.y;
  const int list = round * kSpecBins + bin;
  const int n = __hip_atomic_load(&a.ctr[SPC_CNT + list], __ATOMIC_RELAXED, __HIP_MEMORY_SCOPE_AGENT);
  const size_t off = spec_list_off(list, b.n_chains, b.n_seeds);
  const int2* tl = a.tasks + off;
  const int oe_min = ungapped_oe_min(o.o_del, o.e_del, o.o_ins, o.e_ins);
  const int keep = bin == 0 ? keep_short : 0;
  for (int t0 = (int)blockIdx.x * kUngTasks; t0 < n; t0 += (int)gridDim.x * kUngTasks) {
    const int i = t0 + (tid >> 1), right = tid & 1;
    UngSide s{};
    UngSeg g;
    bool ok = false;
    int extra = 0;
    if (i < n) {
      const FatTask f = fat_task(b, a, tl[i]);
      if (right && a.ungt) a.ungt[off + i] = UngTask{f.rbeg, f.pos, f.qls};
      const int qb = (int)(f.qls & 1023u), ln = (int)((f.qls >> 10) & 1023u), lq = (int)(f.qls >> 20);
      const int64_t xr = f.rbeg + ln;
      const int qlen = right ? lq - qb - ln : qb;
      const int tlen = right ? (int)(f.rbeg + f.dhi - xr) : f.dlo;
      ok = qlen > keep && ungapped_band_ok(o.w) &&
           ungapped_call_ok(qlen, tlen, ln * o.a, o.w, o.zdrop, o.max_mat, oe_min);
      if (ok) {
        s.rd = b.seq + f.qoff;
        s.p0 = right ? qb + ln : qb - 1;
        s.d = right ? 1 : -1;
        s.x0 = right ? xr : f.rbeg - 1;
        s.qlen = qlen;
        s.lq = lq;
        g = ung_pass(s, ref, 0, mat, mat8, o.max_mat);
        if (!g.dead(oe_min)) extra = (qlen - 1) >> 4;
      }
    }
    int inc = extra;
#pragma unroll
    for (int d = 1; d < 64; d <<= 1) {
      const int y = __shfl_up(inc, d, 64);
      if ((tid & 63) >= d) inc += y;
    }
    if ((tid & 63) == 63) wsum[tid >> 6] = inc;
    __syncthreads();
    int pos = inc - extra;
    for (int w = 0; w < (tid >> 6); ++w) pos += wsum[w];
    const bool fits = pos + extra <= kUngPassCap;
    if (extra > 0 && fits) {
      sd[tid] = s;
      for (int k = 1; k <= extra; ++k) plist[pos + k - 1] = (uint32_t)tid << 8 | (uint32_t)k;
      atomicMax(&listed, pos + extra);
    }
    __syncthreads();
    const int np = listed;
    for (int p = tid; p < np; p += 256) {
      const uint32_t e = plist[p];
      const UngSeg x = ung_pass(sd[e >> 8], ref, (int)(e & 255u) * 16, mat, mat8, o.max_mat);
      seg[p] = UngSeg16{(int16_t)x.c, (int16_t)x.P, (int16_t)x.M, (int16_t)x.am};
    }
    __syncthreads();
    UngRec::Side rec{0, {0, 0, 0}};
    if (ok) {
      for (int k = 1; k <= extra && !g.dead(oe_min); ++k) {
        UngSeg x;
        if (fits) {
          const UngSeg16 y = seg[pos + k - 1];
          x.n = min(16, s.qlen - 16 * k);
          x.c = y.c;
          x.P = y.P;
          x.M = y.M;
          x.am = y.am;
        } else {
          x = ung_pass(s, ref, 16 * k, mat, mat8, o.max_mat);
        }
        g = ungseg_combine(g, x);
      }
      if (!g.dead(oe_min)) rec = UngRec::Side{1, g.side()};
    }
    if (i < n) a.ung[off + i].side[right] = rec;
    if (tid == 0) listed = 0;
    __syncthreads();
  }
}

struct SideLists {
  bool cl, cr, in_l, in_r, late;
};
__device__ __forceinline__ SideLists side_lists(const SpecArgs& a, size_t slot, int qb, int qr) {
  SideLists s{false, false, qb > 0, qr > 0, false};
  if (a.ung) {
    s.cl = qb > 0 && a.ung[slot].side[0].ok;
    s.in_l = qb > 0 && !s.cl;
    const bool okr = qr > 0 && a.ung[slot].side[1].ok;
    s.cr = okr && !s.in_l;
    s.late = okr && s.in_l && a.ungt;
    s.in_r = qr > 0 && !s.cr && !s.late;
  }
  return s;
}

__device__ __forceinline__ void settle_right(const DevOpt& o, SeedExt& e, int64_t rbeg, int qb, int ln, int lq,
                                             const UngappedSide& u) {
  const int h0 = e.score;
  const UngappedOut x = ungapped_result(h0, lq - qb - ln, u);
  const bool local = x.gscore <= 0 || x.gscore <= x.score - o.pen_clip3;
  e.qe = local ? qb + ln + x.qle : lq;
  e.re = rbeg + ln + (local ? x.tle : x.gtle);
  e.score = x.score;
  e.truesc += (local ? x.score : x.gscore) - h0;
}

__device__ __forceinline__ SeedExt settle_sides(const DevOpt& o, const FatTask& f, const UngRec& u, bool right) {
  const int qb = (int)(f.qls & 1023u), ln = (int)((f.qls >> 10) & 1023u), lq = (int)(f.qls >> 20);
  const int qr = lq - qb - ln;
  SeedExt e;
  int calls = 0;
  e.rb = f.rbeg;
  e.qb = 0;
  e.score = e.truesc = ln * o.a;
  if (qb > 0) {
    const UngappedOut x = ungapped_result(ln * o.a, qb, u.side[0].s);
    const bool local = x.gscore <= 0 || x.gscore <= x.score - o.pen_clip5;
    e.rb = f.rbeg - (local ? x.tle : x.gtle);
    e.qb = local ? qb - x.qle : 0;
    e.score = x.score;
    e.truesc = local ? x.score : x.gscore;
    ++calls;
  }
  e.re = f.rbeg + ln;
  e.qe = lq;
  if (right) {
    settle_right(o, e, f.rbeg, qb, ln, lq, u.side[1].s);
    ++calls;
  } else if (qr > 0) {
    e.re = 0;
    e.qe = 0;
  }
  e.w = o.w;
  e.cells = e.rows = 0;
  e.calls = calls + (right || qr == 0 ? 1 : 0);
  return e;
}

__global__ void __launch_bounds__(256) spec_sort2_count(DevBatch b, SpecArgs a, int round, int bin0) {
  sel_prio();
  __shared__ int hist[2][256];
  __shared__ int tot[2];
  const int bin = bin0 + (int)blockIdx.y;
  const int list = round * kSpecBins + bin;
  int32_t* ghL = a.sorth + (round * 2 + bin) * kSortKeys;
  int32_t* ghR = ghL + kSortWordsR;
  for (int k = threadIdx.x; k < 2 * 256; k += 256) hist[k >> 8][k & 255] = 0;
  if (threadIdx.x < 2) tot[threadIdx.x] = 0;
  __syncthreads();
  const int n = __hip_atomic_load(&a.ctr[SPC_CNT + list], __ATOMIC_RELAXED, __HIP_MEMORY_SCOPE_AGENT);
  const size_t off = spec_list_off(list, b.n_chains, b.n_seeds);
  const int2* tl = a.tasks + off;
  const int chunk = (n + (int)gridDim.x - 1) / (int)gridDim.x;
  const int i0 = (int)blockIdx.x * chunk, i1 = min(n, i0 + chunk);
  for (int i = i0 + (int)threadIdx.x; i < i1; i += 256) {
    const FatTask f = fat_task(b, a, tl[i]);
    const int qb = (int)(f.qls & 1023u), ln = (int)((f.qls >> 10) & 1023u), lq = (int)(f.qls >> 20);
    const int qr = lq - qb - ln;
    const SideLists sl = side_lists(a, off + i, qb, qr);
    if (sl.in_l) atomicAdd(&hist[0][side_key(qb)], 1);
    if (sl.in_r) atomicAdd(&hist[1][side_key(qr)], 1);
  }
  __syncthreads();
  for (int k = threadIdx.x; k < 2 * 256; k += 256) {
    const int c = hist[k >> 8][k & 255];
    if (c) {
      atomicAdd((k >> 8) ? &ghR[k & 255] : &ghL[k & 255], c);
      atomicAdd(&tot[k >> 8], c);
    }
  }
  __syncthreads();
  if (threadIdx.x < 2 && tot[threadIdx.x])
    atomicAdd(&a.ctr[(threadIdx.x ? SPC_RCNT : SPC_LCNT) + list], tot[threadIdx.x]);
}

__global__ void __launch_bounds__(256) spec_sort2_scan(SpecArgs a, int round, int bin0, int nbins, int short_q) {
  sel_prio();
  __shared__ int part[256];
  const int bin = bin0 + (int)blockIdx.x % nbins, side = (int)blockIdx.x / nbins;
  int32_t* gh = a.sorth + (round * 2 + bin) * kSortKeys + side * kSortWordsR;
  const int t = (int)threadIdx.x;
  const int v = gh[t];
  part[t] = v;
  __syncthreads();
  for (int o = 1; o < 256; o <<= 1) {
    const int x = t >= o ? part[t - o] : 0;
    __syncthreads();
    part[t] += x;
    __syncthreads();
  }
  gh[t] = part[t] - v;
  if (short_q > 0 && bin == 0 && t == side_key(short_q))
    a.ctr[(side ? SPC_RLONG : SPC_LLONG) + round * kSpecBins + bin] = part[t] - v;
}

__global__ void __launch_bounds__(256) spec_sort2_scatter(DevOpt o, DevBatch b, SpecArgs a, int round, int bin0) {
  sel_prio();
  __shared__ int cnt[2][256];
  __shared__ int ung[2];
  const int bin = bin0 + (int)blockIdx.y;
  const int list = round * kSpecBins + bin;
  int32_t* ghL = a.sorth + (round * 2 + bin) * kSortKeys;
  int32_t* ghR = ghL + kSortWordsR;
  for (int k = threadIdx.x; k < 2 * 256; k += 256) cnt[k >> 8][k & 255] = 0;
  if (threadIdx.x < 2) ung[threadIdx.x] = 0;
  __syncthreads();
  const int n = __hip_atomic_load(&a.ctr[SPC_CNT + list], __ATOMIC_RELAXED, __HIP_MEMORY_SCOPE_AGENT);
  const size_t off = spec_list_off(list, b.n_chains, b.n_seeds);
  const int2* tl = a.tasks + off;
  FatTask* foL = a.ftask + off;
  FatTask* foR = a.ftaskR + off;
  const int chunk = (n + (int)gridDim.x - 1) / (int)gridDim.x;
  const int i0 = (int)blockIdx.x * chunk, i1 = min(n, i0 + chunk);
  constexpr int kPer = 8;
  int kl[kPer], kr[kPer], rl[kPer], rr[kPer];
  FatTask ft[kPer];
  for (int base = i0; base < i1; base += 256 * kPer) {
#pragma unroll
    for (int m = 0; m < kPer; ++m) {
      const int i = base + m * 256 + (int)threadIdx.x;
      kl[m] = kr[m] = -1;
      if (i < i1) {
        ft[m] = fat_task(b, a, tl[i]);
        const int qb = (int)(ft[m].qls & 1023u), ln = (int)((ft[m].qls >> 10) & 1023u), lq = (int)(ft[m].qls >> 20);
        const int qr = lq - qb - ln;
        const SideLists sl = side_lists(a, off + i, qb, qr);
        if (sl.in_l) {
          kl[m] = side_key(qb);
          rl[m] = atomicAdd(&cnt[0][kl[m]], 1);
        }
        if (sl.in_r) {
          kr[m] = side_key(qr);
          rr[m] = atomicAdd(&cnt[1][kr[m]], 1);
        }
        if (!sl.in_l) {
          if (qb > 0 || !sl.in_r)
            a.ext[ft[m].pos] = settle_sides(o, ft[m], sl.cl || sl.cr ? a.ung[off + i] : UngRec{}, sl.cr);
          if (sl.cl || sl.cr) {
            atomicAdd(&ung[0], (sl.cl ? 1 : 0) + (sl.cr ? 1 : 0));
            atomicAdd(&ung[1], (sl.cl ? qb : 0) + (sl.cr ? qr : 0));
          }
        }
      }
    }
    __syncthreads();
    for (int k = threadIdx.x; k < 2 * 256; k += 256) {
      const int c = cnt[k >> 8][k & 255];
      cnt[k >> 8][k & 255] = c ? atomicAdd((k >> 8) ? &ghR[k & 255] : &ghL[k & 255], c) : 0;
    }
    __syncthreads();
#pragma unroll
    for (int m = 0; m < kPer; ++m) {
      if (kl[m] >= 0) foL[cnt[0][kl[m]] + rl[m]] = ft[m];
      if (kr[m] >= 0) foR[cnt[1][kr[m]] + rr[m]] = ft[m];
    }
    __syncthreads();
    for (int k = threadIdx.x; k < 2 * 256; k += 256) cnt[k >> 8][k & 255] = 0;
    __syncthreads();
  }
  if (threadIdx.x < 2 && ung[threadIdx.x])
    atomicAdd(&a.ctr[(threadIdx.x ? SPC_UNG_Q : SPC_UNG_N) + round], ung[threadIdx.x]);
}

__global__ void __launch_bounds__(256) spec_settle_right_kernel(DevOpt o, DevBatch b, SpecArgs a, int round, int bin0) {
  sel_prio();
  __shared__ int tot[2];
  __shared__ unsigned long long cel;
  if (threadIdx.x < 2) tot[threadIdx.x] = 0;
  if (threadIdx.x == 0) cel = 0;
  __syncthreads();
  const int list = round * kSpecBins + bin0 + (int)blockIdx.y;
  const int n = __hip_atomic_load(&a.ctr[SPC_CNT + list], __ATOMIC_RELAXED, __HIP_MEMORY_SCOPE_AGENT);
  const size_t off = spec_list_off(list, b.n_chains, b.n_seeds);
  int sides = 0, bases = 0;
  unsigned long long cells = 0;
  for (int i = (int)(blockIdx.x * 256 + threadIdx.x); i < n; i += (int)gridDim.x * 256) {
    const UngTask t = a.ungt[off + i];
    const int qb = (int)(t.qls & 1023u), ln = (int)((t.qls >> 10) & 1023u), lq = (int)(t.qls >> 20);
    if (!side_lists(a, off + i, qb, lq - qb - ln).late) continue;
    SeedExt e = a.ext[t.pos];
    settle_right(o, e, t.rbeg, qb, ln, lq, a.ung[off + i].side[1].s);
    e.w = max(e.w, o.w);
    e.calls += 2;
    a.ext[t.pos] = e;
    ++sides;
    bases += lq - qb - ln;
    cells += (unsigned long long)e.cells;
  }
  if (sides) {
    atomicAdd(&tot[0], sides);
    atomicAdd(&tot[1], bases);
    atomicAdd(&cel, cells);
  }
  __syncthreads();
  if (threadIdx.x < 2 && tot[threadIdx.x])
    atomicAdd(&a.ctr[(threadIdx.x ? SPC_UNGR_Q : SPC_UNGR_N) + round], tot[threadIdx.x]);
  if (threadIdx.x == 0 && cel) atomicAdd(reinterpret_cast<unsigned long long*>(a.ctr + SPC_SPEC64), cel);
}

struct SideTask {
  int64_t rbeg, qoff, rb;
  int32_t pos, dlo, dhi, qbeg, len, lq;
  int32_t tt, score, h0, truesc, qb, aw0, cells, rows, calls, pad_;
};
static_assert(sizeof(SideTask) <= 96, "SideTask layout");
typedef __attribute__((address_space(3))) SideTask LdsS;
#define SIDE_FIELDS(X) X(rbeg) X(qoff) X(rb) X(pos) X(dlo) X(dhi) X(qbeg) X(len) X(lq) X(tt) X(score) X(h0) \
  X(truesc) X(qb) X(aw0) X(cells) X(rows) X(calls)
__device__ __forceinline__ void spark(LdsS* p, const SideTask& t) {
#define X(f) p->f = t.f;
  SIDE_FIELDS(X)
#undef X
  asm volatile("" ::: "memory");
}
__device__ __forceinline__ SideTask sload(LdsS* p) {
  asm volatile("" ::: "memory");
  SideTask t;
#define X(f) t.f = p->f;
  SIDE_FIELDS(X)
#undef X
  return t;
}
#undef SIDE_FIELDS

template <int G, bool RIGHT>
__device__ __forceinline__ void side_start(SideTask& t, const DevOpt& o, const DevRef& ref, const SpecArgs& a,
                                           const FatTask& f, uint8_t* tb) {
  t.rbeg = f.rbeg;
  t.qoff = f.qoff;
  t.pos = f.pos;
  t.dlo = f.dlo;
// ... 220 lines not shown
    const unsigned long long c2 = __builtin_amdgcn_s_memtime();
    tw[1] += c2 - c1;
#endif
    extend_quad_dispatch<G, PMAX, K8>(o, ca, cb, xa, xb, tla, tlb);
#ifdef BWAGPU_OCC_DIAG
    const unsigned long long c3 = __builtin_amdgcn_s_memtime();
    tw[2] += c3 - c2;
    occ_diag<G>(occ, ca, cb, tla, tlb);
#endif
    if (ha) {
      SideTask t = sload(sa);
      if (side_advance<G, RIGHT>(t, o, a, xa, tla, spec_cells)) ha = false;
      else spark(sa, t);
    }
    if (hb) {
      SideTask t = sload(sb);
      if (side_advance<G, RIGHT>(t, o, a, xb, tlb, spec_cells)) hb = false;
      else spark(sb, t);
    }
#ifdef BWAGPU_OCC_DIAG
    tw[3] += __builtin_amdgcn_s_memtime() - c3;
#endif
  }
  return started;
}

template <int G, int PMAX, bool K8, bool RIGHT>
__global__ void __launch_bounds__(kBlock) spec_side4_kernel(DevOpt o, DevRef ref, DevBatch b, SpecArgs a, int list,
                                                            int tb_bytes, int wave_lds, int short_q, int tb_short,
                                                            int short_fill) {
  extern __shared__ __attribute__((aligned(16))) uint8_t lds[];
  uint8_t* const wlds = lds + (size_t)(threadIdx.x >> 6) * (size_t)wave_lds;
  const int n = uni(__hip_atomic_load(&a.ctr[(RIGHT ? SPC_RCNT : SPC_LCNT) + list], __ATOMIC_RELAXED,
                                      __HIP_MEMORY_SCOPE_AGENT));
  const FatTask* fl = (RIGHT ? a.ftaskR : a.ftask) + spec_list_off(list, b.n_chains, b.n_seeds);
  constexpr bool kShort = G == 16 && K8;
  int n_long = n;
  if constexpr (kShort) {
    if (short_q > 0) {
      n_long = min(n, uni(__hip_atomic_load(&a.ctr[(RIGHT ? SPC_RLONG : SPC_LLONG) + list], __ATOMIC_RELAXED,
                                            __HIP_MEMORY_SCOPE_AGENT)));
      const long long slots = (long long)gridDim.x * (kBlock / 64) * (128 / kShortG);
      if ((long long)(n - n_long) * 100 < slots * short_fill) n_long = n;
    }
  }
  const int hl = RIGHT ? kSpecRounds * kSpecBins + list : list;
  long long spec_cells = 0;
#ifdef BWAGPU_OCC_DIAG
  unsigned long long tw[6] = {0, 0, 0, 0, 0, 0}, occ[8] = {0, 0, 0, 0, 0, 0, 0, 0};
  (void)side_loop<G, PMAX, K8, RIGHT>(o, ref, b, a, fl, n_long, a.qh + 8 * kQHStride * hl, wlds, tb_bytes, spec_cells,
                                      tw, occ);
#else
  (void)side_loop<G, PMAX, K8, RIGHT>(o, ref, b, a, fl, n_long, a.qh + 8 * kQHStride * hl, wlds, tb_bytes, spec_cells);
#endif
  if constexpr (kShort) {
    if (n_long < n) {
      int32_t* const hs = a.qh + kQHShort + 8 * kQHStride * hl;
      long long cells_s = 0;
#ifdef BWAGPU_OCC_DIAG
      const int ns = side_loop<kShortG, kShortPmax, true, RIGHT>(o, ref, b, a, fl + n_long, n - n_long, hs, wlds,
                                                                 tb_short, cells_s, tw, occ);
#else
      const int ns = side_loop<kShortG, kShortPmax, true, RIGHT>(o, ref, b, a, fl + n_long, n - n_long, hs, wlds,
                                                                 tb_short, cells_s);
#endif
      if ((threadIdx.x & (kShortG - 1)) == 0 && ns) {
        atomicAdd(&a.ctr[SPC_SHORT_N], ns);
        atomicAdd(reinterpret_cast<unsigned long long*>(a.ctr + SPC_SPEC64), (unsigned long long)cells_s);
      }
    }
  }
#ifdef BWAGPU_OCC_DIAG
  if ((threadIdx.x & 63) == 0) {
    for (int k = 0; k < 8; ++k) atomicAdd(reinterpret_cast<unsigned long long*>(a.ctr + 32) + k, occ[k]);
    for (int k = 0; k < 4; ++k) atomicAdd(reinterpret_cast<unsigned long long*>(a.ctr + 48) + k, tw[k]);
  }
#endif
  if ((threadIdx.x & (G - 1)) == 0 && spec_cells)
    atomicAdd(reinterpret_cast<unsigned long long*>(a.ctr + SPC_SPEC64), (unsigned long long)spec_cells);
}


void launch_side_sort(const ExtRound& r, int bin0, int nbins, int short_q, int short_fill) {
  if (r.a.ung)
    hipLaunchKernelGGL(spec_ungapped_kernel, dim3(512, nbins), dim3(256), 0, r.st, r.o, r.ref, r.b, r.a, r.round, bin0,
                       short_fill == 0 ? short_q : 0);
  hipLaunchKernelGGL(spec_sort2_count, dim3(256, nbins), dim3(256), 0, r.st, r.b, r.a, r.round, bin0);
  hipLaunchKernelGGL(spec_sort2_scan, dim3(2 * nbins), dim3(256), 0, r.st, r.a, r.round, bin0, nbins, short_q);
  hipLaunchKernelGGL(spec_sort2_scatter, dim3(256, nbins), dim3(256), 0, r.st, r.o, r.b, r.a, r.round, bin0);
}

template <int G, int PMAX, bool K8>
static void launch_side_pair(const ExtRound& r, int list, const ExtPlan& p, int short_fill) {
  const size_t lds = (size_t)(kBlock / 64) * p.wave_lds;
  const int nb = resident_blocks(spec_side4_kernel<G, PMAX, K8, false>, lds);
  const int gr = r.round == 2 ? std::min(nb, 64) : std::min(nb, ext2_grid(1 << 30, true));
  if (!(G == 16 && K8)) short_fill = 0;
  hipLaunchKernelGGL((spec_side4_kernel<G, PMAX, K8, false>), dim3(gr), dim3(kBlock), lds, r.st, r.o, r.ref, r.b, r.a,
                     list, r.tb_bytes, (int)p.wave_lds, p.short_q, p.tb_short, short_fill);
  if (r.a.ungt)
    hipLaunchKernelGGL(spec_settle_right_kernel, dim3(256, 1), dim3(256), 0, r.st, r.o, r.b, r.a, r.round,
                       list % kSpecBins);
  hipLaunchKernelGGL((spec_side4_kernel<G, PMAX, K8, true>), dim3(gr), dim3(kBlock), lds, r.st, r.o, r.ref, r.b, r.a,
                     list, r.tb_bytes, (int)p.wave_lds, p.short_q, p.tb_short, short_fill);
}

void launch_side_bin(const ExtBin& k, const ExtRound& r, int list, const ExtPlan& p, int short_fill) {
  switch (ext_key(k.family, k.G, k.PMAX, k.K8)) {
    case ext_key(SIDE4, 16, 10, true): return launch_side_pair<16, 10, true>(r, list, p, short_fill);
    case ext_key(SIDE4, 32, 5, true): return launch_side_pair<32, 5, true>(r, list, p, short_fill);
    case ext_key(SIDE4, 32, 8, false): return launch_side_pair<32, 8, false>(r, list, p, short_fill);
    default: abort();
  }
}

}
```

### bwa-flow_amd/python/bwagpu/abi.py

```python
from __future__ import annotations

import ctypes as C
import os

import numpy as np

HERE = os.path.dirname(os.path.abspath(__file__))
PKG_ROOT = os.path.normpath(os.path.join(HERE, "..", ".."))
REPO_ROOT = os.path.normpath(os.path.join(PKG_ROOT, ".."))
LIB_DIR = os.path.join(PKG_ROOT, "lib")

ABI_VERSION = 1
OK, E_INVAL, E_NOMEM, E_DEVICE, E_HANG, E_RESULTS, E_UNSUPPORTED, E_NODEVICE = range(8)
ERR_NAMES = {
    OK: "OK", E_INVAL: "E_INVAL", E_NOMEM: "E_NOMEM", E_DEVICE: "E_DEVICE", E_HANG: "E_HANG",
    E_RESULTS: "E_RESULTS", E_UNSUPPORTED: "E_UNSUPPORTED", E_NODEVICE: "E_NODEVICE",
}
MAX_READ_LEN = 1023
NUM_SLOTS = 4

SEED_DTYPE = np.dtype([("rbeg", "<i8"), ("qbeg", "<i4"), ("len", "<i4"), ("score", "<i4"),
                       ("pad", "<i4")])
ALNREG_DTYPE = np.dtype([
    ("rb", "<i8"), ("re", "<i8"), ("qb", "<i4"), ("qe", "<i4"), ("rid", "<i4"), ("score", "<i4"),
# ... 109 lines not shown
                ("drop_ratio", C.c_float), ("flags", C.c_int32)]


def default_selopt(flags: int = 0) -> SelOpt:
    return SelOpt(30, 17, 19, 50.0, 3, 0.50, 0.50, int(flags))


MEM_F_NOPAIRING, MEM_F_ALL, MEM_F_NO_MULTI, MEM_F_PRIMARY5, MEM_F_KEEP_SUPP_MAPQ = 0x4, 0x8, 0x10, 0x800, 0x1000
SEL_MAX_REGS = 512
SEL_DONE, SEL_TOO_MANY, SEL_SKIPPED = 0, 1, 2
SEL_NO_PAIRING, SEL_PAIRED = 0, 1
PAIRSEL_DTYPE = np.dtype([("status", "<i4"), ("branch", "<i4"), ("n_pri", "<i4", (2,)), ("z", "<i4", (2,)),
                          ("mapq", "<i4", (2,)), ("alt", "<i4", (2,)), ("extra_flag", "<i4"), ("o", "<i4"),
                          ("subo", "<i4"), ("n_sub", "<i4"), ("pad", "<i4", (2,))])
assert PAIRSEL_DTYPE.itemsize == 64 and C.sizeof(SelOpt) == 32


class SamOpt(C.Structure):
    _fields_ = [("flags", C.c_int32), ("XA_drop_ratio", C.c_float), ("max_XA_hits", C.c_int32),
                ("max_XA_hits_alt", C.c_int32)]


def default_samopt(flags: int = 0) -> SamOpt:
    return SamOpt(int(flags), 0.80, 5, 200)


def default_chainopt() -> dict:
    return dict(max_occ=500, max_chain_gap=10000, min_chain_weight=0, max_chain_extend=1 << 30, mask_level=0.5,
                drop_ratio=0.5)

_VP = C.c_void_p
PROTOS = {
    "bwagpu_abi_version": (C.c_int, []),
    "bwagpu_device_count": (C.c_int, [C.POINTER(C.c_int)]),
    "bwagpu_create": (C.c_int, [C.c_int, C.POINTER(Opt), C.POINTER(Bns), _VP, C.POINTER(_VP)]),
    "bwagpu_create_resident": (C.c_int, [C.c_int, C.POINTER(Opt), C.POINTER(Bns), _VP, C.POINTER(_VP)]),
    "bwagpu_destroy": (C.c_int, [_VP]),
    "bwagpu_last_error": (C.c_char_p, [_VP]),
    "bwagpu_set_watchdog_ms": (C.c_int, [_VP, C.c_int]),
    "bwagpu_chain2aln_submit": (C.c_int, [_VP, C.c_int, C.POINTER(BatchC)]),
    "bwagpu_chain2aln_wait": (C.c_int, [_VP, C.c_int, _VP, _VP]),
    "bwagpu_chain2aln_stage": (C.c_int, [_VP, C.c_int, C.c_int32, C.c_int32, C.c_int32, C.c_int64,
                                         C.POINTER(BatchC)]),
    "bwagpu_chain2aln_results": (C.c_int, [_VP, C.c_int, C.POINTER(_VP), C.POINTER(_VP)]),
    "bwagpu_chain2aln_results_dense": (C.c_int, [_VP, C.c_int, C.POINTER(_VP), C.POINTER(_VP), C.POINTER(_VP)]),
    "bwagpu_chain2aln": (C.c_int, [_VP, C.POINTER(BatchC), _VP, _VP]),
    "bwagpu_chain2aln_device": (C.c_int, [_VP, C.POINTER(BatchC), _VP, _VP, _VP, _VP]),
    "bwagpu_extend_batch": (C.c_int, [_VP, C.c_int32, _VP, _VP, C.c_int64, _VP, C.c_int64, _VP]),
    "bwagpu_align2_batch": (C.c_int, [_VP, C.c_int32, _VP, _VP, C.c_int64, _VP, C.c_int64, _VP]),
    "bwagpu_align2_device": (C.c_int, [_VP, C.c_int32, _VP, _VP, _VP, _VP, _VP, _VP]),
    "bwagpu_reg2aln_batch": (C.c_int, [_VP, C.c_int32, _VP, _VP, C.c_int64, C.c_int32, C.c_int32, _VP, _VP, _VP]),
    "bwagpu_reg2aln_device": (C.c_int, [_VP, C.c_int32, _VP, _VP, _VP, C.c_int64, C.c_int32, C.c_int32, _VP, _VP,
                                        _VP, _VP]),
    "bwagpu_reg2aln_jobs_device": (C.c_int, [_VP, C.c_int32, _VP, _VP, _VP, _VP, _VP, C.c_int32, _VP, _VP, _VP, _VP]),
    "bwagpu_xa_select_device": (C.c_int, [_VP, C.POINTER(SamOpt), C.c_int32, _VP, _VP, _VP, _VP, _VP, _VP, _VP, _VP]),
    "bwagpu_debug_reg2aln_times": (C.c_int, [_VP, _VP]),
    "bwagpu_last_stats": (C.c_int, [_VP, C.c_int, C.POINTER(Stats)]),
    "bwagpu_debug_set_trace": (C.c_int, [_VP, _VP]),
    "bwagpu_prof_start": (C.c_int, [_VP, C.c_int]),
    "bwagpu_debug_fail_wait": (C.c_int, [_VP, C.c_int, C.c_int]),
    "bwagpu_debug_live_buffers": (C.c_int, [C.POINTER(C.c_int64), C.POINTER(C.c_int64)]),
    "bwagpu_debug_spec_counters": (C.c_int, [_VP, _VP, _VP]),
    "bwagpu_debug_occupancy": (C.c_int, [_VP, _VP, _VP]),
    "bwagpu_debug_spec_ext": (C.c_int, [_VP, _VP, _VP, C.c_int32]),
    "bwagpu_prof_read": (C.c_int, [_VP, C.POINTER(C.c_double), C.POINTER(C.c_int32)]),
    "bwagpu_prof_intervals": (C.c_int, [_VP, _VP, _VP, C.c_int32, C.POINTER(C.c_int32)]),
    "bwagpu_set_bwt": (C.c_int, [_VP, C.POINTER(BwtC)]),
    "bwagpu_debug_seed_budget": (C.c_int, [_VP, C.c_int32]),
    "bwagpu_debug_sup_shift": (C.c_int, [_VP, C.c_int32]),
    "bwagpu_set_device_read_len": (C.c_int, [_VP, C.c_int32]),
    "bwagpu_debug_ext_form": (C.c_int, [C.c_int]),
    "bwagpu_ctx_ext_form": (C.c_int, [_VP, C.c_int]),
    "bwagpu_ctx_ext_short": (C.c_int, [_VP, C.c_int]),
    "bwagpu_ctx_ext_short_fill": (C.c_int, [_VP, C.c_int]),
    "bwagpu_ctx_light_pack": (C.c_int, [_VP, C.c_int]),
    "bwagpu_debug_spec_short": (C.c_int, [_VP, _VP, _VP]),
    "bwagpu_ctx_row_bound": (C.c_int, [_VP, C.c_int]),
    "bwagpu_ctx_ungapped": (C.c_int, [_VP, C.c_int]),
    "bwagpu_debug_spec_ungapped": (C.c_int, [_VP, _VP, _VP]),
    "bwagpu_ctx_ungapped_right": (C.c_int, [_VP, C.c_int]),
    "bwagpu_debug_spec_ungapped_right": (C.c_int, [_VP, _VP, _VP]),
    "bwagpu_ctx_emu_finish": (C.c_int, [_VP, C.c_int]),
    "bwagpu_debug_spec_finish": (C.c_int, [_VP, _VP, _VP]),
    "bwagpu_debug_ext_kernel": (C.c_int, [_VP, C.c_int32]),
    "bwagpu_streams_concurrent": (C.c_int, [_VP, _VP]),
    "bwagpu_bwt_sa": (C.c_int, [_VP, C.c_int64, _VP, _VP]),
    "bwagpu_sw_stream": (C.c_int, [_VP, _VP, C.c_int64, _VP, C.c_int32, C.POINTER(C.c_int32)]),
    "bwagpu_collect_intv": (C.c_int, [_VP, C.POINTER(SeedOpt), C.c_int32, _VP, _VP, C.c_int32, _VP, C.c_int64,
                                       _VP]),
    "bwagpu_set_alt": (C.c_int, [_VP, _VP]),
    "bwagpu_seqs2chains": (C.c_int, [_VP, C.POINTER(SeedOpt), C.POINTER(ChainOpt), C.c_int32, _VP, _VP, C.c_int32,
                                      C.POINTER(ChainsC)]),
    "bwagpu_seqs2regions": (C.c_int, [_VP, C.POINTER(SeedOpt), C.POINTER(ChainOpt), C.c_int32, _VP, _VP, _VP,
                                       C.POINTER(_VP), C.POINTER(C.c_int64)]),
    "bwagpu_regs_post": (C.c_int, [_VP, C.POINTER(PostOpt), C.c_int32, C.c_int64, C.c_int32, _VP, _VP, _VP, _VP,
                                    _VP]),
    "bwagpu_regs_post_device": (C.c_int, [_VP, C.POINTER(PostOpt), C.c_int32, C.c_int64, C.POINTER(BatchC), _VP,
                                           _VP, _VP, _VP]),
    "bwagpu_set_regs_post": (C.c_int, [_VP, C.POINTER(PostOpt), C.c_int32, C.c_int64]),
    "bwagpu_pestat": (C.c_int, [_VP, C.POINTER(PairOpt), C.c_int32, _VP, _VP, _VP, _VP]),
    "bwagpu_pestat_device": (C.c_int, [_VP, C.POINTER(PairOpt), C.c_int32, _VP, _VP, _VP, _VP, _VP]),
    "bwagpu_mate_rescue": (C.c_int, [_VP, C.POINTER(PairOpt), _VP, C.c_int32, _VP, _VP, _VP, _VP, _VP, _VP, _VP, _VP,
                                      _VP, _VP]),
    "bwagpu_mate_rescue_device": (C.c_int, [_VP, C.POINTER(PairOpt), _VP, C.POINTER(BatchC), _VP, _VP, _VP, _VP, _VP,
                                             _VP, _VP, _VP, _VP]),
    "bwagpu_mark_primary": (C.c_int, [_VP, C.POINTER(SelOpt), C.c_int64, C.c_int32, _VP, _VP, _VP, _VP, _VP]),
    "bwagpu_mark_primary_device": (C.c_int, [_VP, C.POINTER(SelOpt), C.c_int64, C.c_int32, _VP, _VP, _VP, _VP, _VP,
                                              _VP]),
    "bwagpu_pair_select": (C.c_int, [_VP, C.POINTER(SelOpt), _VP, C.c_int64, C.c_int32, _VP, _VP, _VP, _VP, _VP, _VP,
                                      _VP]),
    "bwagpu_pair_select_device": (C.c_int, [_VP, C.POINTER(SelOpt), _VP, C.c_int64, C.c_int32, _VP, _VP, _VP, _VP,
                                             _VP, _VP, _VP, _VP]),
    "bwagpu_debug_rescue_drop": (C.c_int, [_VP, C.c_int32]),
    "bwagpu_debug_rescue_times": (C.c_int, [_VP, _VP]),
}

_lib = None


def lib_path() -> str:
    return os.environ.get("BWAGPU_LIB", os.path.join(LIB_DIR, "libbwagpu.so"))


def load() -> C.CDLL:
    global _lib
    if _lib is not None:
        return _lib
    p = lib_path()
    if os.environ.get("BWAGPU_NO_TORCH") != "1":
        try:
            import torch
        except Exception:
            pass
    if not os.path.exists(p):
        raise RuntimeError(f"bwagpu: HIP engine library missing at {p}; run __graft_entry__.build()")
    lib = C.CDLL(p)
    for name, (res, args) in PROTOS.items():
        if (name.startswith("bwagpu_debug_") or name in ("bwagpu_ctx_light_pack", "bwagpu_ctx_ungapped", "bwagpu_ctx_ungapped_right", "bwagpu_ctx_emu_finish")) and not hasattr(lib, name):
            continue
        fn = getattr(lib, name)
        fn.restype = res
        fn.argtypes = args
    if lib.bwagpu_abi_version() != ABI_VERSION:
        raise RuntimeError("bwagpu: ABI version mismatch")
    _lib = lib
    return lib


def opt_from_dict(d: dict) -> Opt:
    o = Opt()
    for k in ("a", "b", "o_del", "e_del", "o_ins", "e_ins", "pen_clip5", "pen_clip3", "w", "zdrop"):
        setattr(o, k, int(d[k]))
    mat = d.get("mat")
    if mat is None:
        mat = fill_scmat(int(d["a"]), int(d["b"]))
    for i in range(25):
        o.mat[i] = int(mat[i])
    return o


def fill_scmat(a: int, b: int) -> np.ndarray:
    m = np.full((5, 5), -1, np.int8)
    for i in range(4):
        for j in range(4):
            m[i, j] = a if i == j else -b
    return m.reshape(-1)


def default_opt() -> dict:
    return dict(a=1, b=4, o_del=6, e_del=1, o_ins=6, e_ins=1, pen_clip5=5, pen_clip3=5, w=100,
                zdrop=100, mat=fill_scmat(1, 4))
```

### bwa-flow_amd/python/bwagpu/engine.py

```python
from __future__ import annotations

import ctypes as C
from dataclasses import dataclass

import numpy as np

from . import abi


class BwaGpuError(RuntimeError):
    def __init__(self, code: int, msg: str):
        super().__init__(f"{abi.ERR_NAMES.get(code, code)}: {msg}")
        self.code = code


def _ptr(a: np.ndarray | None):
    return None if a is None or a.size == 0 else a.ctypes.data_as(C.c_void_p)


@dataclass
class Batch:
    seq_off: np.ndarray
    seq: np.ndarray
    read_chain_off: np.ndarray
# ... 221 lines not shown
            C.c_void_p(dev_select), C.c_void_p(dev_seq_off), int(job_cap),
            C.c_void_p(dev_tasks) if dev_tasks else None, C.c_void_p(dev_job_of), C.c_void_p(dev_n_jobs),
            C.c_void_p(stream) if stream else None), "reg2aln_jobs_device")

    def xa_select_device(self, n_reads: int, dev_reg_off: int, dev_regs: int, dev_n: int, dev_sel: int,
                         dev_out_mapq: int, dev_xa_of: int, dev_job_select: int, xopt: abi.SamOpt | None = None,
                         stream: int | None = None):
        xo = abi.default_samopt() if xopt is None else xopt
        self._check(self.lib.bwagpu_xa_select_device(
            self.ctx, C.byref(xo), int(n_reads), C.c_void_p(dev_reg_off), C.c_void_p(dev_regs), C.c_void_p(dev_n),
            C.c_void_p(dev_sel), C.c_void_p(dev_out_mapq), C.c_void_p(dev_xa_of), C.c_void_p(dev_job_select),
            C.c_void_p(stream) if stream else None), "xa_select_device")

    def debug_reg2aln_times(self) -> dict:
        out = np.zeros(4, np.float64)
        self._check(self.lib.bwagpu_debug_reg2aln_times(self.ctx, _ptr(out)), "debug_reg2aln_times")
        return dict(wait_ms=float(out[0]), bins_ms=float(out[1]), call_ms=float(out[2]), jobs=int(out[3]))

    def set_bwt(self, hdr, words, sa=None, sa_intv: int = 32):
        hdr = np.asarray(hdr, np.int64)
        self._bwt_words = np.ascontiguousarray(words, np.uint32)
        self._bwt_sa = None if sa is None else np.ascontiguousarray(sa, np.uint64)
        b = abi.BwtC()
        b.primary = int(hdr[0])
        for i in range(5):
            b.L2[i] = int(hdr[1 + i])
        b.seq_len = int(hdr[6])
        b.bwt_size = len(self._bwt_words)
        b.bwt = self._bwt_words.ctypes.data
        if self._bwt_sa is not None:
            b.sa_intv = sa_intv
            b.n_sa = len(self._bwt_sa)
            b.sa = self._bwt_sa.ctypes.data
        self._check(self.lib.bwagpu_set_bwt(self.ctx, C.byref(b)), "set_bwt")

    def bwt_sa(self, ks) -> np.ndarray:
        ks = np.ascontiguousarray(ks, np.uint64)
        out = np.zeros(max(len(ks), 1), np.uint64)
        self._check(self.lib.bwagpu_bwt_sa(self.ctx, len(ks), _ptr(ks), _ptr(out)), "bwt_sa")
        return out[:len(ks)]

    def sw_stream(self, words: np.ndarray, cap_tasks: int) -> np.ndarray:
        words = np.ascontiguousarray(words, np.int32)
        out = np.zeros((max(cap_tasks, 1), 10), np.int16)
        n = C.c_int32(0)
        self._check(self.lib.bwagpu_sw_stream(self.ctx, _ptr(words), len(words), _ptr(out), int(cap_tasks),
                                              C.byref(n)), "sw_stream")
        return out[:n.value]

    EXT_KERNELS = {2: "spec_ext2_kernel<5>",
                   18: "spec_side4_kernel<16, 10, true>", 14: "spec_side4_kernel<32, 5, true>",
                   15: "spec_side4_kernel<32, 8, false>"}

    def ext_kernel(self, lq_max: int = 256) -> str:
        k = self.lib.bwagpu_debug_ext_kernel(self.ctx, int(lq_max))
        if k not in self.EXT_KERNELS:
            raise BwaGpuError(k, "debug_ext_kernel")
        return self.EXT_KERNELS[k]

    def ext_form(self, form: int = -1) -> int:
        return self.lib.bwagpu_ctx_ext_form(self.ctx, int(form))

    def ext_short(self, q: int = -1) -> int:
        return self.lib.bwagpu_ctx_ext_short(self.ctx, int(q))

    def ext_short_fill(self, percent: int = -1) -> int:
        return self.lib.bwagpu_ctx_ext_short_fill(self.ctx, int(percent))

    def light_pack(self, on: int = -1) -> int:
        return self.lib.bwagpu_ctx_light_pack(self.ctx, int(on))

    def ungapped(self, on: int = -1) -> int:
        return self.lib.bwagpu_ctx_ungapped(self.ctx, int(on))

    def ungapped_right(self, on: int = -1) -> int:
        return self.lib.bwagpu_ctx_ungapped_right(self.ctx, int(on))

    def ungapped_right_counters(self, stream=None):
        out = np.zeros(6, np.int64)
        self._check(self.lib.bwagpu_debug_spec_ungapped_right(self.ctx, C.c_void_p(stream), _ptr(out)),
                    "debug_spec_ungapped_right")
        return out.reshape(3, 2)

    def emu_finish(self, on: int = -1) -> int:
        return self.lib.bwagpu_ctx_emu_finish(self.ctx, int(on))

    def row_bound(self, on: int = -1) -> int:
        return self.lib.bwagpu_ctx_row_bound(self.ctx, int(on))

    def set_device_read_len(self, max_len: int):
        self._check(self.lib.bwagpu_set_device_read_len(self.ctx, int(max_len)), "set_device_read_len")

    def sup_shift(self, shift: int):
        self._check(self.lib.bwagpu_debug_sup_shift(self.ctx, shift), "sup_shift")

    def seed_budget(self, budget: int):
        self._check(self.lib.bwagpu_debug_seed_budget(self.ctx, budget), "seed_budget")

    def collect_intv(self, seq_off: np.ndarray, seq: np.ndarray, min_seed_len: int = 19, split_width: int = 10,
                     max_mem_intv: int = 20, split_factor: float = 1.5, max_per_read: int = 256,
                     out_cap: int | None = None, out: np.ndarray | None = None):
        seq_off = np.ascontiguousarray(seq_off, np.int64)
        seq = np.ascontiguousarray(seq, np.uint8)
        n = len(seq_off) - 1
        o = abi.SeedOpt(min_seed_len, split_width, max_mem_intv, split_factor)
        if out is not None:
            if out.dtype != abi.INTV_DTYPE or not out.flags.c_contiguous:
                raise ValueError("out must be a contiguous INTV_DTYPE array")
            cap = len(out)
        else:
            cap = max(n, 1) * max_per_read if out_cap is None else out_cap
            out = np.zeros(max(cap, 1), abi.INTV_DTYPE)
        cnt = np.zeros(max(n, 1), np.int32)
        self._check(self.lib.bwagpu_collect_intv(self.ctx, C.byref(o), n, _ptr(seq_off), _ptr(seq), max_per_read,
                                                 _ptr(out), cap, _ptr(cnt)), "collect_intv")
        cnt = cnt[:n]
        return cnt, out[:int(cnt.sum())]

    def set_alt(self, is_alt):
        self._alt = None if is_alt is None else np.ascontiguousarray(is_alt, np.uint8)
        self._check(self.lib.bwagpu_set_alt(self.ctx, None if self._alt is None else _ptr(self._alt)), "set_alt")

    @staticmethod
    def _seed_chain_opts(seedopt, split_factor, chainopt):
        so = np.asarray(seedopt, np.int32)
        co = abi.default_chainopt() if chainopt is None else chainopt
        return (abi.SeedOpt(int(so[0]), int(so[1]), int(so[2]), float(split_factor)),
                abi.ChainOpt(int(co["max_occ"]), int(co["max_chain_gap"]), int(co["min_chain_weight"]),
                             int(co["max_chain_extend"]), float(co["mask_level"]), float(co["drop_ratio"])))

    def seqs2chains(self, seq_off, seq, seedopt=(19, 10, 20), split_factor: float = 1.5, chainopt: dict | None = None,
                    raw: bool = False, copy: bool = True):
        seq_off = np.ascontiguousarray(seq_off, np.int64)
        seq = np.ascontiguousarray(seq, np.uint8)
        n = len(seq_off) - 1
        so, co = self._seed_chain_opts(seedopt, split_factor, chainopt)
        out = abi.ChainsC()
        self._check(self.lib.bwagpu_seqs2chains(self.ctx, C.byref(so), C.byref(co), n, _ptr(seq_off), _ptr(seq),
                                                int(raw), C.byref(out)), "seqs2chains")
        nc, ns = out.n_chains, out.n_seeds

        def view(p, dt, k):
            if k == 0:
                return np.zeros(0, dt)
            v = np.frombuffer((C.c_char * (k * np.dtype(dt).itemsize)).from_address(p), dt)
            return v.copy() if copy else v
        return (view(out.read_chain_off, np.int32, n + 1), view(out.chains, abi.CHAIN_DTYPE, nc),
                view(out.chain_seed_off, np.int32, nc + 1), view(out.seeds, abi.SEED_DTYPE, ns))

    def seqs2regions(self, seq_off, seq, seedopt=(19, 10, 20), split_factor: float = 1.5,
                     chainopt: dict | None = None, copy: bool = True):
        seq_off = np.ascontiguousarray(seq_off, np.int64)
        seq = np.ascontiguousarray(seq, np.uint8)
        n = len(seq_off) - 1
        so, co = self._seed_chain_opts(seedopt, split_factor, chainopt)
        cnt = np.zeros(max(n, 1), np.int32)
        regs, nreg = C.c_void_p(), C.c_int64()
        self._check(self.lib.bwagpu_seqs2regions(self.ctx, C.byref(so), C.byref(co), n, _ptr(seq_off), _ptr(seq),
                                                 _ptr(cnt), C.byref(regs), C.byref(nreg)), "seqs2regions")
        k = nreg.value
        out = np.zeros(0, abi.ALNREG_DTYPE) if k == 0 else np.frombuffer(
            (C.c_char * (k * abi.ALNREG_DTYPE.itemsize)).from_address(regs.value), abi.ALNREG_DTYPE)
        return cnt[:n], (out.copy() if copy else out)

    def regs_post(self, seq_off, seq, reg_off, regs, n, flags: int, id0: int = 0, popt: abi.PostOpt | None = None):
        seq_off = np.ascontiguousarray(seq_off, np.int64)
# ... 165 lines not shown
```

### include/bwagpu.h

```cpp
#ifndef BWAGPU_H
#define BWAGPU_H

#include <stddef.h>
#include <stdint.h>

#ifdef __cplusplus
extern "C" {
#endif

#define BWAGPU_ABI_VERSION 1

enum {
  BWAGPU_OK = 0,
  BWAGPU_E_INVAL = 1,
  BWAGPU_E_NOMEM = 2,
  BWAGPU_E_DEVICE = 3,
  BWAGPU_E_HANG = 4,
  BWAGPU_E_RESULTS = 5,
  BWAGPU_E_UNSUPPORTED = 6,
  BWAGPU_E_NODEVICE = 7
};

#define BWAGPU_MAX_READ_LEN 1023
#define BWAGPU_NUM_SLOTS 4
// ... 99 lines not shown
  uint64_t primary;
  uint64_t L2[5];
  uint64_t seq_len;
  uint64_t bwt_size;
  const uint32_t *bwt;
  int32_t sa_intv;
  int32_t pad_;
  uint64_t n_sa;
  const uint64_t *sa;
} bwagpu_bwt_t;

typedef struct {
  uint64_t x[3];
  uint64_t info;
} bwagpu_intv_t;

typedef struct {
  int32_t min_seed_len;
  int32_t split_width;
  int32_t max_mem_intv;
  float split_factor;
} bwagpu_seedopt_t;

#define BWAGPU_MAX_SEED_READ 4096

typedef struct {
  int32_t max_occ;
  int32_t max_chain_gap;
  int32_t min_chain_weight;
  int32_t max_chain_extend;
  float mask_level;
  float drop_ratio;
} bwagpu_chainopt_t;

typedef struct {
  int64_t pos;
  int32_t rid;
  int32_t n;
  int32_t w;
  int32_t kept;
  int32_t first;
  int32_t is_alt;
  float frac_rep;
  int32_t pad_;
} bwagpu_chain_t;

typedef struct {
  double kernel_ms;
  double total_ms;
  int64_t cells;
  int64_t rows;
  int64_t ext_calls;
  int64_t h2d_bytes, d2h_bytes;
} bwagpu_stats_t;

typedef struct bwagpu_ctx bwagpu_ctx_t;

int bwagpu_abi_version(void);
int bwagpu_device_count(int *n);

int bwagpu_create(int device, const bwagpu_opt_t *opt, const bwagpu_bns_t *bns,
                  const uint8_t *pac_host, bwagpu_ctx_t **ctx);
int bwagpu_create_resident(int device, const bwagpu_opt_t *opt, const bwagpu_bns_t *bns,
                           const void *pac_device, bwagpu_ctx_t **ctx);
int bwagpu_destroy(bwagpu_ctx_t *ctx);
const char *bwagpu_last_error(const bwagpu_ctx_t *ctx);

int bwagpu_set_watchdog_ms(bwagpu_ctx_t *ctx, int ms);

int bwagpu_chain2aln_submit(bwagpu_ctx_t *ctx, int slot, const bwagpu_batch_t *batch);
int bwagpu_chain2aln_wait(bwagpu_ctx_t *ctx, int slot, bwagpu_alnreg_t *out_regs, int32_t *out_n);
int bwagpu_chain2aln(bwagpu_ctx_t *ctx, const bwagpu_batch_t *batch, bwagpu_alnreg_t *out_regs,
                     int32_t *out_n);

int bwagpu_chain2aln_stage(bwagpu_ctx_t *ctx, int slot, int32_t n_reads, int32_t n_chains, int32_t n_seeds,
                           int64_t seq_bytes, bwagpu_batch_t *view);
int bwagpu_chain2aln_results(bwagpu_ctx_t *ctx, int slot, const bwagpu_alnreg_t **regs, const int32_t **n);
int bwagpu_chain2aln_results_dense(bwagpu_ctx_t *ctx, int slot, const bwagpu_alnreg_t **regs, const int32_t **n,
                                   const int32_t **off);
int bwagpu_chain2aln_device(bwagpu_ctx_t *ctx, const bwagpu_batch_t *dev_batch,
                            bwagpu_alnreg_t *dev_out, int32_t *dev_n, int64_t *dev_stats,
                            void *stream);
int bwagpu_set_device_read_len(bwagpu_ctx_t *ctx, int32_t max_len);

int bwagpu_extend_batch(bwagpu_ctx_t *ctx, int32_t n_tasks, const bwagpu_ext_task_t *tasks,
                        const uint8_t *qpool, int64_t qpool_len, const uint8_t *tpool,
                        int64_t tpool_len, bwagpu_ext_result_t *results);

int bwagpu_align2_batch(bwagpu_ctx_t *ctx, int32_t n_tasks, const bwagpu_align2_task_t *tasks,
                        const uint8_t *qpool, int64_t qpool_len, const uint8_t *tpool, int64_t tpool_len,
                        bwagpu_kswr_t *results);
int bwagpu_align2_device(bwagpu_ctx_t *ctx, int32_t n_tasks, const bwagpu_align2_task_t *dev_tasks,
                         const uint8_t *dev_qpool, const uint8_t *dev_tpool, bwagpu_kswr_t *dev_results,
                         void *dev_scratch, void *stream);

int bwagpu_reg2aln_batch(bwagpu_ctx_t *ctx, int32_t n_tasks, const bwagpu_reg2aln_task_t *tasks,
                         const uint8_t *qpool, int64_t qpool_len, int32_t max_ops, int32_t max_md,
                         bwagpu_aln_t *out, uint32_t *cigar, char *md);
int bwagpu_reg2aln_device(bwagpu_ctx_t *ctx, int32_t n_cap, const int32_t *dev_n_tasks,
                          const bwagpu_reg2aln_task_t *dev_tasks, const uint8_t *dev_qpool, int64_t qpool_len,
                          int32_t max_ops, int32_t max_md, bwagpu_aln_t *dev_out, uint32_t *dev_cigar,
                          char *dev_md, void *stream);
int bwagpu_reg2aln_jobs_device(bwagpu_ctx_t *ctx, int32_t n_reads, const int64_t *dev_reg_off,
                               const bwagpu_alnreg_t *dev_regs, const int32_t *dev_n, const int32_t *dev_select,
                               const int64_t *dev_seq_off, int32_t job_cap, bwagpu_reg2aln_task_t *dev_tasks,
                               int32_t *dev_job_of, int32_t *dev_n_jobs, void *stream);

int bwagpu_sw_stream(bwagpu_ctx_t *ctx, const int32_t *i_buf, int64_t i_words, int16_t *o_buf,
                     int32_t o_cap_tasks, int32_t *o_tasks);

int bwagpu_last_stats(const bwagpu_ctx_t *ctx, int slot, bwagpu_stats_t *stats);

int bwagpu_set_bwt(bwagpu_ctx_t *ctx, const bwagpu_bwt_t *bwt);

int bwagpu_collect_intv(bwagpu_ctx_t *ctx, const bwagpu_seedopt_t *opt, int32_t n_reads, const int64_t *seq_off,
                        const uint8_t *seq, int32_t max_per_read, bwagpu_intv_t *out, int64_t out_cap,
                        int32_t *out_n);

int bwagpu_bwt_sa(bwagpu_ctx_t *ctx, int64_t n, const uint64_t *k, uint64_t *out);


typedef struct {
  int32_t n_reads, n_chains;
  int64_t n_seeds;
  const int32_t *read_chain_off;
  const int32_t *chain_seed_off;
  const bwagpu_chain_t *chains;
  const bwagpu_seed_t *seeds;
} bwagpu_chains_t;

int bwagpu_set_alt(bwagpu_ctx_t *ctx, const uint8_t *is_alt);

int bwagpu_seqs2chains(bwagpu_ctx_t *ctx, const bwagpu_seedopt_t *sopt, const bwagpu_chainopt_t *copt,
                       int32_t n_reads, const int64_t *seq_off, const uint8_t *seq, int32_t raw,
                       bwagpu_chains_t *out);

int bwagpu_seqs2regions(bwagpu_ctx_t *ctx, const bwagpu_seedopt_t *sopt, const bwagpu_chainopt_t *copt,
                        int32_t n_reads, const int64_t *seq_off, const uint8_t *seq, int32_t *out_n,
                        const bwagpu_alnreg_t **regs, int64_t *n_regs);


#define BWAGPU_POST_DEDUP_PATCH 1
#define BWAGPU_POST_MARK_ALT    2
#define BWAGPU_POST_PRIMARY     4

typedef struct {
  int32_t max_chain_gap;
  float mask_level_redun;
  float mask_level;
  int32_t pad_;
} bwagpu_postopt_t;

int bwagpu_regs_post(bwagpu_ctx_t *ctx, const bwagpu_postopt_t *popt, int32_t flags, int64_t id0, int32_t n_reads,
                     const int64_t *seq_off, const uint8_t *seq, const int64_t *reg_off, bwagpu_alnreg_t *regs,
                     int32_t *n);
int bwagpu_regs_post_device(bwagpu_ctx_t *ctx, const bwagpu_postopt_t *popt, int32_t flags, int64_t id0,
                            const bwagpu_batch_t *dev_batch, const int64_t *dev_reg_off, bwagpu_alnreg_t *dev_regs,
                            int32_t *dev_n, void *stream);
int bwagpu_set_regs_post(bwagpu_ctx_t *ctx, const bwagpu_postopt_t *popt, int32_t flags, int64_t id0_of_next_batch);


typedef struct {
  int32_t max_ins;
  int32_t max_matesw;
  int32_t pen_unpaired;
  int32_t min_seed_len;
// ... 106 lines not shown
```

Baseline: 71.61.

## Fuse side-sort count/scan into ungapped and scatter kernels; overlap settle on side stream

Adds a fused-launch mask, default 5 (sort and heavy fusion on). With it, the ungapped kernel builds the per-side key histogram, and the scatter kernel does the prefix scan with wave shuffles, so the separate count and scan launches are dropped. Optionally, settle-right runs on a side stream with fork/join events, and the heavy select body is pulled into a device function, apparently so it can be fused. This cuts launch count and serial kernel gaps in a pipeline of small kernels, at the cost of a larger sort buffer (cursor region), redundant scans in every scatter block, and more complex ordering.

After: 75.82, median of 6. +5.9%, better.

```diff
diff --git a/bwa-flow_amd/csrc/capi.hip b/bwa-flow_amd/csrc/capi.hip
--- a/bwa-flow_amd/csrc/capi.hip
+++ b/bwa-flow_amd/csrc/capi.hip
@@ -155,6 +155,7 @@
   ctx->ungapped = ungapped_default();
   ctx->ungapped_right = ungapped_right_default();
   ctx->emu_finish = emu_finish_default();
+  ctx->fused_launches = fused_launches_default();
   *made = ctx;
   HIPC(hipSetDevice(device), "hipSetDevice");
   HIPC(hipMalloc(&ctx->d_ann_off, sizeof(int64_t) * bns->n_seqs), "hipMalloc(ann_offset)");
@@ -358,6 +359,7 @@
   ss.form = ctx->ext_form;
   ss.short_q = ctx->ext_short;
   ss.short_fill = ctx->ext_short_fill;
+  ss.fused = ctx->fused_launches;
   ss.pool = ctx->prof_ev.empty() ? nullptr : ctx->prof_ev.data();
   ss.pool_n = (int)ctx->prof_ev.size();
   ss.pool_used = &ctx->prof_used;
@@ -915,6 +917,13 @@
   return prev;
 }
 
+int bwagpu_ctx_fused_launches(bwagpu_ctx_t* ctx, int mask) {
+  if (!ctx) return BWAGPU_E_INVAL;
+  const int prev = ctx->fused_launches;
+  if (mask >= 0) ctx->fused_launches = mask & 7;
+  return prev;
+}
+
 int bwagpu_debug_spec_finish(bwagpu_ctx_t* ctx, void* stream, int64_t* out) {
   if (!ctx || !out) return BWAGPU_E_INVAL;
   int32_t c[SPC_WORDS];
diff --git a/bwa-flow_amd/csrc/ctx.h b/bwa-flow_amd/csrc/ctx.h
--- a/bwa-flow_amd/csrc/ctx.h
+++ b/bwa-flow_amd/csrc/ctx.h
@@ -137,6 +137,7 @@
   int ungapped = 1;
   int ungapped_right = 1;
   int emu_finish = 1;
+  int fused_launches = 5;
   Slot slot[BWAGPU_NUM_SLOTS];
   hipStream_t dev_stream[BWAGPU_NUM_SLOTS] = {};
   Slot dev_scratch[BWAGPU_NUM_SLOTS];
diff --git a/bwa-flow_amd/csrc/engine.h b/bwa-flow_amd/csrc/engine.h
--- a/bwa-flow_amd/csrc/engine.h
+++ b/bwa-flow_amd/csrc/engine.h
@@ -123,7 +123,8 @@
 constexpr int kQHWords = 2 * kQHShort;
 constexpr int kSortKeys = 1024;
 constexpr int kSortWordsR = kSpecRounds * 2 * kSortKeys;
-constexpr int kSortWords = 2 * kSortWordsR;
+constexpr int kSortCursor = 2 * kSortWordsR;
+constexpr int kSortWords = 2 * kSortCursor;
 __host__ __device__ inline size_t spec_list_off(int list, int n_chains, int n_seeds) {
   const int round = list / kSpecBins, bin = list % kSpecBins;
   return round == 0 ? (size_t)bin * n_chains
@@ -199,7 +200,14 @@
   int form = 0;
   int short_q = 0;
   int short_fill = 0;
-};
+  int fused = 0;
+};
+enum {
+  kFuseSort = 1,
+  kFuseSettle = 2,
+  kFuseHeavy = 4,
+};
+int fused_launches_default();
 int ungapped_default();
 int ungapped_right_default();
 int emu_finish_default();
diff --git a/bwa-flow_amd/csrc/side_sort.h b/bwa-flow_amd/csrc/side_sort.h
--- /dev/null
+++ b/bwa-flow_amd/csrc/side_sort.h
@@ -0,0 +1,45 @@
+#pragma once
+#include <stdint.h>
+
+#ifdef __HIPCC__
+#define BWAGPU_SS_HD __host__ __device__
+#else
+#define BWAGPU_SS_HD
+#endif
+
+namespace bwagpu {
+
+constexpr int kSideKeys = 256;
+constexpr int kSideLaneKeys = 4;
+
+BWAGPU_SS_HD inline int side_key(int qlen) { return 255 - (qlen < 255 ? qlen : 255); }
+
+BWAGPU_SS_HD inline int32_t side_lane_total(const int32_t* h) { return h[0] + h[1] + h[2] + h[3]; }
+BWAGPU_SS_HD inline void side_lane_prefix(const int32_t* h, int32_t before, int32_t* first) {
+  first[0] = before;
+  first[1] = before + h[0];
+  first[2] = first[1] + h[1];
+  first[3] = first[2] + h[2];
+}
+BWAGPU_SS_HD inline int32_t side_scan_step(int32_t own, int32_t below, int lane, int d) {
+  return lane >= d ? own + below : own;
+}
+
+BWAGPU_SS_HD inline void side_wave_scan(int32_t* inc) {
+  for (int d = 1; d < 64; d <<= 1) {
+    int32_t prev[64];
+    for (int l = 0; l < 64; ++l) prev[l] = inc[l];
+    for (int l = 0; l < 64; ++l) inc[l] = side_scan_step(prev[l], l >= d ? prev[l - d] : 0, l, d);
+  }
+}
+BWAGPU_SS_HD inline void side_prefix(const int32_t* hist, int32_t* first) {
+  int32_t inc[64];
+  for (int l = 0; l < 64; ++l) inc[l] = side_lane_total(hist + kSideLaneKeys * l);
+  side_wave_scan(inc);
+  for (int l = 0; l < 64; ++l)
+    side_lane_prefix(hist + kSideLaneKeys * l, inc[l] - side_lane_total(hist + kSideLaneKeys * l),
+                     first + kSideLaneKeys * l);
+}
+BWAGPU_SS_HD inline int32_t side_short_first(const int32_t* first, int short_q) { return first[side_key(short_q)]; }
+
+}
diff --git a/bwa-flow_amd/csrc/spec.hip b/bwa-flow_amd/csrc/spec.hip
--- a/bwa-flow_amd/csrc/spec.hip
+++ b/bwa-flow_amd/csrc/spec.hip
@@ -917,12 +917,11 @@
   if (r < 8) tr[((size_t)pass * n_reads + rd) * 8 + d] = v;
 }
 
-template <int MODE, bool HEAVY>
-__global__ void __launch_bounds__(64) spec_select_kernel(DevOpt o, DevRef ref, DevBatch b, SpecArgs a, int tb_bytes) {
-  sel_prio();
-  static_assert(HEAVY, "one-wave heavy shape only");
+template <int MODE>
+__device__ __forceinline__ void select_heavy_read(const DevOpt& o, const DevRef& ref, const DevBatch& b,
+                                                  const SpecArgs& a, int rd, uint8_t* lds, int tb_bytes, bool fill_mg,
+                                                  Tally& tl) {
   constexpr bool WRITE = MODE != SEL_EMULATE;
-  extern __shared__ __attribute__((aligned(16))) uint8_t lds[];
   const int r = (int)(threadIdx.x & 63);
   int32_t* const MG = reinterpret_cast<int32_t*>(lds);
   bwagpu_seed_t* const SC = reinterpret_cast<bwagpu_seed_t*>(lds + 4 * kMglN);
@@ -931,7 +930,178 @@
   const int cap_reg = sel_heavy_cap(MODE, tb_bytes);
   uint8_t* const tbl = reinterpret_cast<uint8_t*>(R + cap_reg);
   uint8_t* const tbr = tbl + tb_bytes;
-  for (int x = r; x < kMglN; x += 64) MG[x] = max_gap_len(o, x);
+  if (fill_mg)
+    for (int x = r; x < kMglN; x += 64) MG[x] = max_gap_len(o, x);
+  const uint64_t t_start = g_trace ? __builtin_amdgcn_s_memrealtime() : 0;
+  const ReadDesc d = uniform_desc(a.rdesc[rd]);
+  if (d.lq > a.lq_bound) return;
+  const uint8_t* const q = b.seq + d.qoff;
+  const int rep_lim = (int)floor(.1 * d.lq) + 1;
+  bool redo = false;
+  Tally rt{0, 0, 0};
+  int nreg = 0, n_inline = 0;
+  for (int c = d.c0; c < d.c0 + d.nch && !redo; ++c) {
+    const int s0 = uni(b.chain_seed_off[c]), ns = uni(b.chain_seed_off[c + 1]) - s0;
+    if (ns == 0) continue;
+    ChainWin cw = a.win[c];
+    cw.lo = uni64(cw.lo);
+    cw.hi = uni64(cw.hi);
+    if (cw.hi < cw.lo) continue;
+    const int rid = uni(b.chain_rid[c]);
+    const float frac = __int_as_float(uni(__float_as_int(b.chain_frac_rep[c])));
+    const bool big = ns > kSelExtCache;
+    for (int i = r; i < min(ns, kSelExtCache); i += 64) {
+      bwagpu_seed_t v = a.prog[s0 + i];
+      v.pad_ = v.pad_ != 0 ? 1 : 0;
+      SC[i] = v;
+      const uint32_t* src = reinterpret_cast<const uint32_t*>(a.ext + s0 + i);
+      uint32_t* dst = reinterpret_cast<uint32_t*>(EC + i);
+#pragma unroll
+      for (int w = 0; w < 12; ++w) dst[w] = __hip_atomic_load(src + w, __ATOMIC_RELAXED, __HIP_MEMORY_SCOPE_WORKGROUP);
+    }
+    if (big)
+      for (int i = r; i < ns; i += 64)
+        __hip_atomic_store(&a.skipf[s0 + i], a.prog[s0 + i].pad_ != 0 ? 1 : 0, __ATOMIC_RELAXED,
+                           __HIP_MEMORY_SCOPE_WORKGROUP);
+    mem_fence_group();
+    auto seed_at = [&](int i) -> bwagpu_seed_t { return i < kSelExtCache ? SC[i] : a.prog[s0 + i]; };
+    auto flag_at = [&](int i) -> int {
+      return i < kSelExtCache ? SC[i].pad_
+                              : __hip_atomic_load(&a.skipf[s0 + i], __ATOMIC_RELAXED, __HIP_MEMORY_SCOPE_WORKGROUP);
+    };
+    auto set_flag = [&](int i, int f) {
+      if (r == 0) {
+        if (i < kSelExtCache) SC[i].pad_ |= f;
+        else __hip_atomic_store(&a.skipf[s0 + i], f | 0, __ATOMIC_RELAXED, __HIP_MEMORY_SCOPE_WORKGROUP);
+      }
+      mem_fence_group();
+    };
+    for (int k = 0; k < ns; ++k) {
+      const bwagpu_seed_t s = uni_seed(seed_at(k));
+      bool hit = false;
+      for (int base = 0; base < nreg && !hit; base += 64) {
+        const int i = min(base + r, nreg - 1);
+        RegRec p;
+        if (i < cap_reg) {
+          p = R[i];
+        } else {
+          const int pp = __hip_atomic_load(&a.regpos[d.s0 + i], __ATOMIC_RELAXED, __HIP_MEMORY_SCOPE_WORKGROUP);
+          const SeedExt* pe = a.ext + pp;
+          p.rb = __hip_atomic_load(&pe->rb, __ATOMIC_RELAXED, __HIP_MEMORY_SCOPE_WORKGROUP);
+          p.re = __hip_atomic_load(&pe->re, __ATOMIC_RELAXED, __HIP_MEMORY_SCOPE_WORKGROUP);
+          p.qb = __hip_atomic_load(&pe->qb, __ATOMIC_RELAXED, __HIP_MEMORY_SCOPE_WORKGROUP);
+          p.qe = __hip_atomic_load(&pe->qe, __ATOMIC_RELAXED, __HIP_MEMORY_SCOPE_WORKGROUP);
+          p.w = __hip_atomic_load(&pe->w, __ATOMIC_RELAXED, __HIP_MEMORY_SCOPE_WORKGROUP);
+          p.seedlen0 = a.prog[pp].len;
+        }
+        const bool inside = base + r < nreg &&
+                            !(s.rbeg < p.rb || s.rbeg + s.len > p.re || s.qbeg < p.qb || s.qbeg + s.len > p.qe) &&
+                            !(s.len - p.seedlen0 >= rep_lim);
+        if (__builtin_amdgcn_ballot_w64(inside) == 0) continue;
+        hit = __builtin_amdgcn_ballot_w64(inside && seed_near(MG, s, p)) != 0;
+      }
+      if (hit) {
+        const int len95 = uni((int)ceil(s.len * .95));
+        bool ov = false;
+        for (int base = 0; base < k && !ov; base += 64) {
+          const int i = min(base + r, k - 1);
+          const bwagpu_seed_t t = seed_at(i);
+          const bool tsk = (flag_at(i) & 1) != 0;
+          const bool a1 = s.qbeg <= t.qbeg && s.qbeg + s.len - t.qbeg >= s.len >> 2 && (int64_t)(t.qbeg - s.qbeg) != t.rbeg - s.rbeg;
+          const bool b1 = t.qbeg <= s.qbeg && t.qbeg + t.len - s.qbeg >= s.len >> 2 && (int64_t)(s.qbeg - t.qbeg) != s.rbeg - t.rbeg;
+          ov = __builtin_amdgcn_ballot_w64(base + r < k && !tsk && t.len >= len95 && (a1 || b1)) != 0;
+        }
+        if (!ov) {
+          set_flag(k, 1);
+          continue;
+        }
+      }
+      const int pos = s0 + k;
+      const SeedExt* const pe = k < kSelExtCache ? EC + k : a.ext + pos;
+      SeedExt e;
+      e.calls = uni(__hip_atomic_load(&pe->calls, __ATOMIC_RELAXED, __HIP_MEMORY_SCOPE_WORKGROUP));
+      if (e.calls == 0) {
+        if constexpr (MODE == SEL_REDO) {
+          e = extend_seed<16>(o, ref, s, d.lq, q, cw, tbl, tbr);
+          store_ext(a.ext + pos, e);
+          mem_fence_group();
+          if (r == 0) atomicAdd(&a.ctr[SPC_MISS], 1);
+          ++n_inline;
+        } else if constexpr (MODE == SEL_EMULATE) {
+          set_flag(k, 2);
+          continue;
+        } else {
+          const int list = 2 * kSpecBins + spec_bin(d.lq);
+          if (r == 0) {
+            const int p = atomicAdd(&a.ctr[SPC_CNT + list], 1);
+            a.tasks[spec_list_off(list, b.n_chains, b.n_seeds) + p] = make_int2(pos, c);
+            a.redo[atomicAdd(&a.ctr[SPC_REDO_N], 1)] = rd;
+          }
+          redo = true;
+          break;
+        }
+      } else {
+        e.rb = uni64(__hip_atomic_load(&pe->rb, __ATOMIC_RELAXED, __HIP_MEMORY_SCOPE_WORKGROUP));
+        e.re = uni64(__hip_atomic_load(&pe->re, __ATOMIC_RELAXED, __HIP_MEMORY_SCOPE_WORKGROUP));
+        e.qb = uni(__hip_atomic_load(&pe->qb, __ATOMIC_RELAXED, __HIP_MEMORY_SCOPE_WORKGROUP));
+        e.qe = uni(__hip_atomic_load(&pe->qe, __ATOMIC_RELAXED, __HIP_MEMORY_SCOPE_WORKGROUP));
+        e.score = uni(__hip_atomic_load(&pe->score, __ATOMIC_RELAXED, __HIP_MEMORY_SCOPE_WORKGROUP));
+        e.truesc = uni(__hip_atomic_load(&pe->truesc, __ATOMIC_RELAXED, __HIP_MEMORY_SCOPE_WORKGROUP));
+        e.w = uni(__hip_atomic_load(&pe->w, __ATOMIC_RELAXED, __HIP_MEMORY_SCOPE_WORKGROUP));
+        e.cells = uni(__hip_atomic_load(&pe->cells, __ATOMIC_RELAXED, __HIP_MEMORY_SCOPE_WORKGROUP));
+        e.rows = uni(__hip_atomic_load(&pe->rows, __ATOMIC_RELAXED, __HIP_MEMORY_SCOPE_WORKGROUP));
+      }
+      if constexpr (WRITE) {
+        long long cov = 0;
+        for (int base = 0; base < ns; base += 64) {
+          const int i = base + r;
+          const bwagpu_seed_t t = seed_at(min(i, ns - 1));
+          const bool in = i < ns && t.qbeg >= e.qb && t.qbeg + t.len <= e.qe && t.rbeg >= e.rb && t.rbeg + t.len <= e.re;
+          cov += in ? t.len : 0;
+        }
+        cov = grp_sum64(cov, 64);
+        write_region(a.out + d.s0 + nreg, e, rid, (int)cov, s.len, frac);
+        rt.cells += e.cells;
+        rt.rows += e.rows;
+        rt.calls += e.calls - 1;
+      }
+      if (nreg < cap_reg) {
+        put_regrec(R + nreg, e, s.len);
+      } else {
+        if (r == 0) __hip_atomic_store(&a.regpos[d.s0 + nreg], pos, __ATOMIC_RELAXED, __HIP_MEMORY_SCOPE_WORKGROUP);
+        mem_fence_group();
+      }
+      ++nreg;
+    }
+    if constexpr (MODE == SEL_EMULATE) {
+      const int list = kSpecBins + spec_bin(d.lq);
+      for (int base = 0; base < ns; base += 64) {
+        const int i = base + r;
+        const bool pnd = i < ns && (flag_at(min(i, ns - 1)) & 2) != 0;
+        const int p = wave_append(&a.ctr[SPC_CNT + list], pnd);
+        if (p >= 0) a.tasks[spec_list_off(list, b.n_chains, b.n_seeds) + p] = make_int2(s0 + i, c);
+      }
+    }
+  }
+  trace_read(MODE, b.n_reads, rd, t_start, d.ns, nreg, 2 | (MODE == SEL_REDO ? n_inline << 4 : 0));
+  if constexpr (WRITE) {
+    if (!redo) {
+      a.out_n[rd] = nreg;
+      tl.cells += rt.cells;
+      tl.rows += rt.rows;
+      tl.calls += rt.calls;
+    }
+  }
+}
+
+template <int MODE, bool HEAVY>
+__global__ void __launch_bounds__(64) spec_select_kernel(DevOpt o, DevRef ref, DevBatch b, SpecArgs a, int tb_bytes) {
+  sel_prio();
+  static_assert(HEAVY, "one-wave heavy shape only");
+  constexpr bool WRITE = MODE != SEL_EMULATE;
+  extern __shared__ __attribute__((aligned(16))) uint8_t lds[];
+  const int r = (int)(threadIdx.x & 63);
+  for (int x = r; x < kMglN; x += 64) reinterpret_cast<int32_t*>(lds)[x] = max_gap_len(o, x);
   Tally tl{0, 0, 0};
   const int n_list = uni(__hip_atomic_load(&a.ctr[MODE == SEL_REDO ? SPC_REDO_N : SPC_HEAVY_N], __ATOMIC_RELAXED,
                                            __HIP_MEMORY_SCOPE_AGENT));
@@ -942,167 +1112,7 @@
     t = uni(__shfl(t, 0, 64));
     if (t >= n_list) break;
     if (MODE != SEL_REDO && uni(a.hinfo[t].y) >= 0) continue;
-    const int rd = uni(hlist[t]);
-    const uint64_t t_start = g_trace ? __builtin_amdgcn_s_memrealtime() : 0;
-    const ReadDesc d = uniform_desc(a.rdesc[rd]);
-    if (d.lq > a.lq_bound) continue;
-    const uint8_t* const q = b.seq + d.qoff;
-    const int rep_lim = (int)floor(.1 * d.lq) + 1;
-    bool redo = false;
-    Tally rt{0, 0, 0};
-    int nreg = 0, n_inline = 0;
-    for (int c = d.c0; c < d.c0 + d.nch && !redo; ++c) {
-      const int s0 = uni(b.chain_seed_off[c]), ns = uni(b.chain_seed_off[c + 1]) - s0;
-      if (ns == 0) continue;
-      ChainWin cw = a.win[c];
-      cw.lo = uni64(cw.lo);
-      cw.hi = uni64(cw.hi);
-      if (cw.hi < cw.lo) continue;
-      const int rid = uni(b.chain_rid[c]);
-      const float frac = __int_as_float(uni(__float_as_int(b.chain_frac_rep[c])));
-      const bool big = ns > kSelExtCache;
-      for (int i = r; i < min(ns, kSelExtCache); i += 64) {
-        bwagpu_seed_t v = a.prog[s0 + i];
-        v.pad_ = v.pad_ != 0 ? 1 : 0;
-        SC[i] = v;
-        const uint32_t* src = reinterpret_cast<const uint32_t*>(a.ext + s0 + i);
-        uint32_t* dst = reinterpret_cast<uint32_t*>(EC + i);
-#pragma unroll
-        for (int w = 0; w < 12; ++w) dst[w] = __hip_atomic_load(src + w, __ATOMIC_RELAXED, __HIP_MEMORY_SCOPE_WORKGROUP);
-      }
-      if (big)
-        for (int i = r; i < ns; i += 64)
-          __hip_atomic_store(&a.skipf[s0 + i], a.prog[s0 + i].pad_ != 0 ? 1 : 0, __ATOMIC_RELAXED,
-                             __HIP_MEMORY_SCOPE_WORKGROUP);
-      mem_fence_group();
-      auto seed_at = [&](int i) -> bwagpu_seed_t { return i < kSelExtCache ? SC[i] : a.prog[s0 + i]; };
-      auto flag_at = [&](int i) -> int {
-        return i < kSelExtCache ? SC[i].pad_
-                                : __hip_atomic_load(&a.skipf[s0 + i], __ATOMIC_RELAXED, __HIP_MEMORY_SCOPE_WORKGROUP);
-      };
-      auto set_flag = [&](int i, int f) {
-        if (r == 0) {
-          if (i < kSelExtCache) SC[i].pad_ |= f;
-          else __hip_atomic_store(&a.skipf[s0 + i], f | 0, __ATOMIC_RELAXED, __HIP_MEMORY_SCOPE_WORKGROUP);
-        }
-        mem_fence_group();
-      };
-      for (int k = 0; k < ns; ++k) {
-        const bwagpu_seed_t s = uni_seed(seed_at(k));
-        bool hit = false;
-        for (int base = 0; base < nreg && !hit; base += 64) {
-          const int i = min(base + r, nreg - 1);
-          RegRec p;
-          if (i < cap_reg) {
-            p = R[i];
-          } else {
-            const int pp = __hip_atomic_load(&a.regpos[d.s0 + i], __ATOMIC_RELAXED, __HIP_MEMORY_SCOPE_WORKGROUP);
-            const SeedExt* pe = a.ext + pp;
-            p.rb = __hip_atomic_load(&pe->rb, __ATOMIC_RELAXED, __HIP_MEMORY_SCOPE_WORKGROUP);
-            p.re = __hip_atomic_load(&pe->re, __ATOMIC_RELAXED, __HIP_MEMORY_SCOPE_WORKGROUP);
-            p.qb = __hip_atomic_load(&pe->qb, __ATOMIC_RELAXED, __HIP_MEMORY_SCOPE_WORKGROUP);
-            p.qe = __hip_atomic_load(&pe->qe, __ATOMIC_RELAXED, __HIP_MEMORY_SCOPE_WORKGROUP);
-            p.w = __hip_atomic_load(&pe->w, __ATOMIC_RELAXED, __HIP_MEMORY_SCOPE_WORKGROUP);
-            p.seedlen0 = a.prog[pp].len;
-          }
-          const bool inside = base + r < nreg &&
-                              !(s.rbeg < p.rb || s.rbeg + s.len > p.re || s.qbeg < p.qb || s.qbeg + s.len > p.qe) &&
-                              !(s.len - p.seedlen0 >= rep_lim);
-          if (__builtin_amdgcn_ballot_w64(inside) == 0) continue;
-          hit = __builtin_amdgcn_ballot_w64(inside && seed_near(MG, s, p)) != 0;
-        }
-        if (hit) {
-          const int len95 = uni((int)ceil(s.len * .95));
-          bool ov = false;
-          for (int base = 0; base < k && !ov; base += 64) {
-            const int i = min(base + r, k - 1);
-            const bwagpu_seed_t t = seed_at(i);
-            const bool tsk = (flag_at(i) & 1) != 0;
-            const bool a1 = s.qbeg <= t.qbeg && s.qbeg + s.len - t.qbeg >= s.len >> 2 && (int64_t)(t.qbeg - s.qbeg) != t.rbeg - s.rbeg;
-            const bool b1 = t.qbeg <= s.qbeg && t.qbeg + t.len - s.qbeg >= s.len >> 2 && (int64_t)(s.qbeg - t.qbeg) != s.rbeg - t.rbeg;
-            ov = __builtin_amdgcn_ballot_w64(base + r < k && !tsk && t.len >= len95 && (a1 || b1)) != 0;
-          }
-          if (!ov) {
-            set_flag(k, 1);
-            continue;
-          }
-        }
-        const int pos = s0 + k;
-        const SeedExt* const pe = k < kSelExtCache ? EC + k : a.ext + pos;
-        SeedExt e;
-        e.calls = uni(__hip_atomic_load(&pe->calls, __ATOMIC_RELAXED, __HIP_MEMORY_SCOPE_WORKGROUP));
-        if (e.calls == 0) {
-          if constexpr (MODE == SEL_REDO) {
-            e = extend_seed<16>(o, ref, s, d.lq, q, cw, tbl, tbr);
-            store_ext(a.ext + pos, e);
-            mem_fence_group();
-            if (r == 0) atomicAdd(&a.ctr[SPC_MISS], 1);
-            ++n_inline;
-          } else if constexpr (MODE == SEL_EMULATE) {
-            set_flag(k, 2);
-            continue;
-          } else {
-            const int list = 2 * kSpecBins + spec_bin(d.lq);
-            if (r == 0) {
-              const int p = atomicAdd(&a.ctr[SPC_CNT + list], 1);
-              a.tasks[spec_list_off(list, b.n_chains, b.n_seeds) + p] = make_int2(pos, c);
-              a.redo[atomicAdd(&a.ctr[SPC_REDO_N], 1)] = rd;
-            }
-            redo = true;
-            break;
-          }
-        } else {
-          e.rb = uni64(__hip_atomic_load(&pe->rb, __ATOMIC_RELAXED, __HIP_MEMORY_SCOPE_WORKGROUP));
-          e.re = uni64(__hip_atomic_load(&pe->re, __ATOMIC_RELAXED, __HIP_MEMORY_SCOPE_WORKGROUP));
-          e.qb = uni(__hip_atomic_load(&pe->qb, __ATOMIC_RELAXED, __HIP_MEMORY_SCOPE_WORKGROUP));
-          e.qe = uni(__hip_atomic_load(&pe->qe, __ATOMIC_RELAXED, __HIP_MEMORY_SCOPE_WORKGROUP));
-          e.score = uni(__hip_atomic_load(&pe->score, __ATOMIC_RELAXED, __HIP_MEMORY_SCOPE_WORKGROUP));
-          e.truesc = uni(__hip_atomic_load(&pe->truesc, __ATOMIC_RELAXED, __HIP_MEMORY_SCOPE_WORKGROUP));
-          e.w = uni(__hip_atomic_load(&pe->w, __ATOMIC_RELAXED, __HIP_MEMORY_SCOPE_WORKGROUP));
-          e.cells = uni(__hip_atomic_load(&pe->cells, __ATOMIC_RELAXED, __HIP_MEMORY_SCOPE_WORKGROUP));
-          e.rows = uni(__hip_atomic_load(&pe->rows, __ATOMIC_RELAXED, __HIP_MEMORY_SCOPE_WORKGROUP));
-        }
-        if constexpr (WRITE) {
-          long long cov = 0;
-          for (int base = 0; base < ns; base += 64) {
-            const int i = base + r;
-            const bwagpu_seed_t t = seed_at(min(i, ns - 1));
-            const bool in = i < ns && t.qbeg >= e.qb && t.qbeg + t.len <= e.qe && t.rbeg >= e.rb && t.rbeg + t.len <= e.re;
-            cov += in ? t.len : 0;
-          }
-          cov = grp_sum64(cov, 64);
-          write_region(a.out + d.s0 + nreg, e, rid, (int)cov, s.len, frac);
-          rt.cells += e.cells;
-          rt.rows += e.rows;
-          rt.calls += e.calls - 1;
-        }
-        if (nreg < cap_reg) {
-          put_regrec(R + nreg, e, s.len);
-        } else {
-          if (r == 0) __hip_atomic_store(&a.regpos[d.s0 + nreg], pos, __ATOMIC_RELAXED, __HIP_MEMORY_SCOPE_WORKGROUP);
-          mem_fence_group();
-        }
-        ++nreg;
-      }
-      if constexpr (MODE == SEL_EMULATE) {
-        const int list = kSpecBins + spec_bin(d.lq);
-        for (int base = 0; base < ns; base += 64) {
-          const int i = base + r;
-          const bool pnd = i < ns && (flag_at(min(i, ns - 1)) & 2) != 0;
-          const int p = wave_append(&a.ctr[SPC_CNT + list], pnd);
-          if (p >= 0) a.tasks[spec_list_off(list, b.n_chains, b.n_seeds) + p] = make_int2(s0 + i, c);
-        }
-      }
-    }
-    trace_read(MODE, b.n_reads, rd, t_start, d.ns, nreg, 2 | (MODE == SEL_REDO ? n_inline << 4 : 0));
-    if constexpr (WRITE) {
-      if (!redo) {
-        a.out_n[rd] = nreg;
-        tl.cells += rt.cells;
-        tl.rows += rt.rows;
-        tl.calls += rt.calls;
-      }
-    }
+    select_heavy_read<MODE>(o, ref, b, a, uni(hlist[t]), lds, tb_bytes, false, tl);
   }
   if constexpr (WRITE) {
     if (r != 0) tl = Tally{0, 0, 0};
@@ -1753,7 +1763,8 @@
   __builtin_amdgcn_wave_barrier();
 }
 
-template <int MODE>
+static_assert(kScanLds >= kSelHeavyLds, "spec_scan_kernel's LDS holds select_heavy_read's layout");
+template <int MODE, bool FOLD>
 __global__ void __launch_bounds__(64) spec_scan_kernel(DevOpt o, DevRef ref, DevBatch b, SpecArgs a, int tb_bytes) {
   sel_prio();
   constexpr bool WRITE = MODE != SEL_EMULATE;
@@ -1764,6 +1775,21 @@
   const uint64_t lt_mask = r ? (~0ull >> (64 - r)) : 0ull;
   const int nh = uni(__hip_atomic_load(&a.ctr[SPC_HEAVY_N], __ATOMIC_RELAXED, __HIP_MEMORY_SCOPE_AGENT));
   Tally tl{0, 0, 0};
+  if constexpr (MODE != SEL_REDO) {
+    if constexpr (FOLD) {
+      Tally ts{0, 0, 0};
+      bool mg = true;
+      for (int t = (int)blockIdx.x; t < nh; t += (int)gridDim.x) {
+        const int4 hi = a.hinfo[t];
+        if (uni(hi.y) >= 0) continue;
+        select_heavy_read<MODE>(o, ref, b, a, uni(hi.x), reinterpret_cast<uint8_t*>(M), tb_bytes, mg, ts);
+        mg = false;
+      }
+      __builtin_amdgcn_fence(__ATOMIC_SEQ_CST, "workgroup");
+      __builtin_amdgcn_wave_barrier();
+      if (r == 0) tl = ts;
+    }
+  }
   for (int t = (int)blockIdx.x; t < nh; t += (int)gridDim.x) {
     const int4 hi = a.hinfo[t];
     const int rd = uni(hi.x), woff = uni(hi.y), ns = uni(hi.w);
@@ -2026,6 +2052,7 @@
 static void launch_select(const DevOpt& o, const DevRef& ref, const DevBatch& b, const SpecArgs& a, int tb_bytes,
                           hipStream_t st, const SpecStreams& ss) {
   hipStream_t hs = st;
+  const bool fold = MODE != SEL_REDO && (ss.fused & kFuseHeavy);
   if (MODE != SEL_REDO && ss.side) {
     (void)hipEventRecord(ss.fork, st);
     (void)hipStreamWaitEvent(ss.side, ss.fork, 0);
@@ -2044,11 +2071,16 @@
   if (MODE != SEL_REDO) {
     const int nb = resident_blocks(spec_pairs_kernel<MODE>, 0);
     hipLaunchKernelGGL((spec_pairs_kernel<MODE>), dim3(nb), dim3(kBlock), 0, hs, o, b, a);
-    hipLaunchKernelGGL((spec_scan_kernel<MODE>), dim3(kScanGrid), dim3(64), (size_t)kScanLds + 2 * (size_t)tb_bytes, hs, o,
-                       ref, b, a, tb_bytes);
-  }
-  hipLaunchKernelGGL((spec_select_kernel<MODE, true>), dim3(MODE == SEL_REDO ? 256 : 1024), dim3(64),
-                     (size_t)kSelHeavyLds, hs, o, ref, b, a, tb_bytes);
+    if (fold)
+      hipLaunchKernelGGL((spec_scan_kernel<MODE, true>), dim3(kScanGrid), dim3(64),
+                         (size_t)kScanLds + 2 * (size_t)tb_bytes, hs, o, ref, b, a, tb_bytes);
+    else
+      hipLaunchKernelGGL((spec_scan_kernel<MODE, false>), dim3(kScanGrid), dim3(64),
+                         (size_t)kScanLds + 2 * (size_t)tb_bytes, hs, o, ref, b, a, tb_bytes);
+  }
+  if (!fold)
+    hipLaunchKernelGGL((spec_select_kernel<MODE, true>), dim3(MODE == SEL_REDO ? 256 : 1024), dim3(64),
+                       (size_t)kSelHeavyLds, hs, o, ref, b, a, tb_bytes);
   if (hs != st) {
     (void)hipEventRecord(ss.join, hs);
     (void)hipStreamWaitEvent(st, ss.join, 0);
@@ -2098,6 +2130,13 @@
   }();
   return on;
 }
+int fused_launches_default() {
+  static const int m = [] {
+    const char* e = getenv("BWAGPU_FUSED_LAUNCHES");
+    return (e && e[0] ? atoi(e) : 5) & 7;
+  }();
+  return m;
+}
 int ext_short_fill_default() {
   static const int f = [] {
     const char* e = getenv("BWAGPU_EXT_SHORT_FILL");
@@ -2121,7 +2160,7 @@
   const int l = round * kSpecBins;
   const bool bin1 = lq_max > kSpecBinLen[0], bin2 = lq_max > kSpecBinLen[1];
   const ExtPlan plan = ext_plan(o, ss.form, tb_bytes, ss.short_q);
-  const ExtRound r{o, ref, b, a, round, tb_bytes, st};
+  const ExtRound r{o, ref, b, a, round, tb_bytes, st, ss};
   if (!bin1 || plan.bin[0].phased == plan.bin[1].phased) {
     launch_sort(plan.bin[0], r, 0, bin1 ? 2 : 1, plan.short_q, ss.short_fill);
   } else {
diff --git a/bwa-flow_amd/csrc/spec_dev.h b/bwa-flow_amd/csrc/spec_dev.h
--- a/bwa-flow_amd/csrc/spec_dev.h
+++ b/bwa-flow_amd/csrc/spec_dev.h
@@ -176,6 +176,7 @@
   const SpecArgs& a;
   int round, tb_bytes;
   hipStream_t st;
+  const SpecStreams& ss;
 };
 int ext2_grid(int nb, bool packed);
 void launch_side_sort(const ExtRound& r, int bin0, int nbins, int short_q, int short_fill);
diff --git a/bwa-flow_amd/csrc/spec_side.hip b/bwa-flow_amd/csrc/spec_side.hip
--- a/bwa-flow_amd/csrc/spec_side.hip
+++ b/bwa-flow_amd/csrc/spec_side.hip
@@ -1,8 +1,7 @@
+#include "side_sort.h"
 #include "spec_dev.h"
 
 namespace bwagpu {
-
-__device__ __forceinline__ int side_key(int qlen) { return 255 - min(qlen, 255); }
 
 
 struct UngSide {
@@ -81,6 +80,24 @@
   return g;
 }
 
+struct SideLists {
+  bool cl, cr, in_l, in_r, late;
+};
+__device__ __forceinline__ SideLists side_lists(const UngRec& u, bool ungt, int qb, int qr) {
+  SideLists s;
+  s.cl = qb > 0 && u.side[0].ok;
+  s.in_l = qb > 0 && !s.cl;
+  const bool okr = qr > 0 && u.side[1].ok;
+  s.cr = okr && !s.in_l;
+  s.late = okr && s.in_l && ungt;
+  s.in_r = qr > 0 && !s.cr && !s.late;
+  return s;
+}
+__device__ __forceinline__ SideLists side_lists(const SpecArgs& a, size_t slot, int qb, int qr) {
+  if (!a.ung) return SideLists{false, false, qb > 0, qr > 0, false};
+  return side_lists(a.ung[slot], a.ungt != nullptr, qb, qr);
+}
+
 constexpr int kUngTasks = 128;
 constexpr int kUngPassCap = 256 * 9;
 struct UngSeg16 {
@@ -88,8 +105,10 @@
 };
 
 __global__ void __launch_bounds__(256) spec_ungapped_kernel(DevOpt o, DevRef ref, DevBatch b, SpecArgs a, int round,
-                                                            int bin0, int keep_short) {
+                                                            int bin0, int keep_short, int count) {
   sel_prio();
+  __shared__ int hist[2][kSideKeys];
+  __shared__ int tot[2];
   __shared__ int8_t mat[25], mat8[32];
   __shared__ UngSide sd[256];
   __shared__ uint32_t plist[kUngPassCap];
@@ -99,6 +118,10 @@
   if (tid < 25) mat[tid] = o.mat[tid];
   if (tid < 32) mat8[tid] = (tid & 7) < 5 ? o.mat[(tid >> 3) * 5 + (tid & 7)] : 0;
   if (tid == 0) listed = 0;
+  if (count) {
+    for (int k = tid; k < 2 * kSideKeys; k += 256) hist[k >> 8][k & 255] = 0;
+    if (tid < 2) tot[tid] = 0;
+  }
   __syncthreads();
   const int bin = bin0 + (int)blockIdx.y;
   const int list = round * kSpecBins + bin;
@@ -113,6 +136,7 @@
     UngSeg g;
     bool ok = false;
     int extra = 0;
+    int qside = 0;
     if (i < n) {
       const FatTask f = fat_task(b, a, tl[i]);
       if (right && a.ungt) a.ungt[off + i] = UngTask{f.rbeg, f.pos, f.qls};
@@ -120,6 +144,7 @@
       const int64_t xr = f.rbeg + ln;
       const int qlen = right ? lq - qb - ln : qb;
       const int tlen = right ? (int)(f.rbeg + f.dhi - xr) : f.dlo;
+      qside = qlen;
       ok = qlen > keep && ungapped_band_ok(o.w) &&
            ungapped_call_ok(qlen, tlen, ln * o.a, o.w, o.zdrop, o.max_mat, oe_min);
       if (ok) {
@@ -176,25 +201,31 @@
       if (!g.dead(oe_min)) rec = UngRec::Side{1, g.side()};
     }
     if (i < n) a.ung[off + i].side[right] = rec;
+    if (count) {
+      const int ok2 = __shfl_xor(rec.ok, 1, 64), q2 = __shfl_xor(qside, 1, 64);
+      if (i < n) {
+        UngRec u{};
+        u.side[0].ok = right ? ok2 : rec.ok;
+        u.side[1].ok = right ? rec.ok : ok2;
+        const SideLists sl = side_lists(u, a.ungt != nullptr, right ? q2 : qside, right ? qside : q2);
+        if (right ? sl.in_r : sl.in_l) atomicAdd(&hist[right][side_key(qside)], 1);
+      }
+    }
     if (tid == 0) listed = 0;
     __syncthreads();
   }
-}
-
-struct SideLists {
-  bool cl, cr, in_l, in_r, late;
-};
-__device__ __forceinline__ SideLists side_lists(const SpecArgs& a, size_t slot, int qb, int qr) {
-  SideLists s{false, false, qb > 0, qr > 0, false};
-  if (a.ung) {
-    s.cl = qb > 0 && a.ung[slot].side[0].ok;
-    s.in_l = qb > 0 && !s.cl;
-    const bool okr = qr > 0 && a.ung[slot].side[1].ok;
-    s.cr = okr && !s.in_l;
-    s.late = okr && s.in_l && a.ungt;
-    s.in_r = qr > 0 && !s.cr && !s.late;
-  }
-  return s;
+  if (!count) return;
+  int32_t* ghL = a.sorth + (round * 2 + bin) * kSortKeys;
+  int32_t* ghR = ghL + kSortWordsR;
+  for (int k = tid; k < 2 * kSideKeys; k += 256) {
+    const int c = hist[k >> 8][k & 255];
+    if (c) {
+      atomicAdd((k >> 8) ? &ghR[k & 255] : &ghL[k & 255], c);
+      atomicAdd(&tot[k >> 8], c);
+    }
+  }
+  __syncthreads();
+  if (tid < 2 && tot[tid]) atomicAdd(&a.ctr[(tid ? SPC_RCNT : SPC_LCNT) + list], tot[tid]);
 }
 
 __device__ __forceinline__ void settle_right(const DevOpt& o, SeedExt& e, int64_t rbeg, int qb, int ln, int lq,
@@ -297,9 +328,11 @@
     a.ctr[(side ? SPC_RLONG : SPC_LLONG) + round * kSpecBins + bin] = part[t] - v;
 }
 
-__global__ void __launch_bounds__(256) spec_sort2_scatter(DevOpt o, DevBatch b, SpecArgs a, int round, int bin0) {
+__global__ void __launch_bounds__(256) spec_sort2_scatter(DevOpt o, DevBatch b, SpecArgs a, int round, int bin0,
+                                                          int short_q, int scan) {
   sel_prio();
   __shared__ int cnt[2][256];
+  __shared__ int first[2][kSideKeys];
   __shared__ int ung[2];
   const int bin = bin0 + (int)blockIdx.y;
   const int list = round * kSpecBins + bin;
@@ -307,7 +340,26 @@
   int32_t* ghR = ghL + kSortWordsR;
   for (int k = threadIdx.x; k < 2 * 256; k += 256) cnt[k >> 8][k & 255] = 0;
   if (threadIdx.x < 2) ung[threadIdx.x] = 0;
+  if (scan) {
+    const int side = (int)(threadIdx.x >> 6), lane = (int)(threadIdx.x & 63);
+    if (side < 2) {
+      const int4 h4 = reinterpret_cast<const int4*>(side ? ghR : ghL)[lane];
+      const int32_t h[kSideLaneKeys] = {h4.x, h4.y, h4.z, h4.w};
+      const int32_t own = side_lane_total(h);
+      int32_t inc = own;
+#pragma unroll
+      for (int d = 1; d < 64; d <<= 1) inc = side_scan_step(inc, __shfl_up(inc, d, 64), lane, d);
+      int32_t f[kSideLaneKeys];
+      side_lane_prefix(h, inc - own, f);
+#pragma unroll
+      for (int j = 0; j < kSideLaneKeys; ++j) first[side][kSideLaneKeys * lane + j] = f[j];
+    }
+    ghL += kSortCursor;
+    ghR += kSortCursor;
+  }
   __syncthreads();
+  if (scan && short_q > 0 && bin == 0 && blockIdx.x == 0 && threadIdx.x < 2)
+    a.ctr[(threadIdx.x ? SPC_RLONG : SPC_LLONG) + list] = side_short_first(first[threadIdx.x], short_q);
   const int n = __hip_atomic_load(&a.ctr[SPC_CNT + list], __ATOMIC_RELAXED, __HIP_MEMORY_SCOPE_AGENT);
   const size_t off = spec_list_off(list, b.n_chains, b.n_seeds);
   const int2* tl = a.tasks + off;
@@ -349,7 +401,8 @@
     __syncthreads();
     for (int k = threadIdx.x; k < 2 * 256; k += 256) {
       const int c = cnt[k >> 8][k & 255];
-      cnt[k >> 8][k & 255] = c ? atomicAdd((k >> 8) ? &ghR[k & 255] : &ghL[k & 255], c) : 0;
+      cnt[k >> 8][k & 255] =
+          c ? (scan ? first[k >> 8][k & 255] : 0) + atomicAdd((k >> 8) ? &ghR[k & 255] : &ghL[k & 255], c) : 0;
     }
     __syncthreads();
 #pragma unroll
@@ -736,12 +789,15 @@
 
 
 void launch_side_sort(const ExtRound& r, int bin0, int nbins, int short_q, int short_fill) {
+  const int fuse = (r.ss.fused & kFuseSort) ? 1 : 0;
   if (r.a.ung)
     hipLaunchKernelGGL(spec_ungapped_kernel, dim3(512, nbins), dim3(256), 0, r.st, r.o, r.ref, r.b, r.a, r.round, bin0,
-                       short_fill == 0 ? short_q : 0);
-  hipLaunchKernelGGL(spec_sort2_count, dim3(256, nbins), dim3(256), 0, r.st, r.b, r.a, r.round, bin0);
-  hipLaunchKernelGGL(spec_sort2_scan, dim3(2 * nbins), dim3(256), 0, r.st, r.a, r.round, bin0, nbins, short_q);
-  hipLaunchKernelGGL(spec_sort2_scatter, dim3(256, nbins), dim3(256), 0, r.st, r.o, r.b, r.a, r.round, bin0);
+                       short_fill == 0 ? short_q : 0, fuse);
+  if (!(fuse && r.a.ung)) hipLaunchKernelGGL(spec_sort2_count, dim3(256, nbins), dim3(256), 0, r.st, r.b, r.a, r.round, bin0);
+  if (!fuse)
+    hipLaunchKernelGGL(spec_sort2_scan, dim3(2 * nbins), dim3(256), 0, r.st, r.a, r.round, bin0, nbins, short_q);
+  hipLaunchKernelGGL(spec_sort2_scatter, dim3(256, nbins), dim3(256), 0, r.st, r.o, r.b, r.a, r.round, bin0, short_q,
+                     fuse);
 }
 
 template <int G, int PMAX, bool K8>
@@ -752,11 +808,20 @@
   if (!(G == 16 && K8)) short_fill = 0;
   hipLaunchKernelGGL((spec_side4_kernel<G, PMAX, K8, false>), dim3(gr), dim3(kBlock), lds, r.st, r.o, r.ref, r.b, r.a,
                      list, r.tb_bytes, (int)p.wave_lds, p.short_q, p.tb_short, short_fill);
-  if (r.a.ungt)
+  const bool beside = r.a.ungt && r.ss.side && (r.ss.fused & kFuseSettle);
+  if (beside) {
+    (void)hipEventRecord(r.ss.fork, r.st);
+    (void)hipStreamWaitEvent(r.ss.side, r.ss.fork, 0);
+    hipLaunchKernelGGL(spec_settle_right_kernel, dim3(256, 1), dim3(256), 0, r.ss.side, r.o, r.b, r.a, r.round,
+                       list % kSpecBins);
+    (void)hipEventRecord(r.ss.join, r.ss.side);
+  } else if (r.a.ungt) {
     hipLaunchKernelGGL(spec_settle_right_kernel, dim3(256, 1), dim3(256), 0, r.st, r.o, r.b, r.a, r.round,
                        list % kSpecBins);
+  }
   hipLaunchKernelGGL((spec_side4_kernel<G, PMAX, K8, true>), dim3(gr), dim3(kBlock), lds, r.st, r.o, r.ref, r.b, r.a,
                      list, r.tb_bytes, (int)p.wave_lds, p.short_q, p.tb_short, short_fill);
+  if (beside) (void)hipStreamWaitEvent(r.st, r.ss.join, 0);
 }
 
 void launch_side_bin(const ExtBin& k, const ExtRound& r, int list, const ExtPlan& p, int short_fill) {
diff --git a/bwa-flow_amd/python/bwagpu/abi.py b/bwa-flow_amd/python/bwagpu/abi.py
--- a/bwa-flow_amd/python/bwagpu/abi.py
+++ b/bwa-flow_amd/python/bwagpu/abi.py
@@ -215,6 +215,7 @@
     "bwagpu_debug_spec_ungapped_right": (C.c_int, [_VP, _VP, _VP]),
     "bwagpu_ctx_emu_finish": (C.c_int, [_VP, C.c_int]),
     "bwagpu_debug_spec_finish": (C.c_int, [_VP, _VP, _VP]),
+    "bwagpu_ctx_fused_launches": (C.c_int, [_VP, C.c_int]),
     "bwagpu_debug_ext_kernel": (C.c_int, [_VP, C.c_int32]),
     "bwagpu_streams_concurrent": (C.c_int, [_VP, _VP]),
     "bwagpu_bwt_sa": (C.c_int, [_VP, C.c_int64, _VP, _VP]),
@@ -269,7 +270,7 @@
         raise RuntimeError(f"bwagpu: HIP engine library missing at {p}; run __graft_entry__.build()")
     lib = C.CDLL(p)
     for name, (res, args) in PROTOS.items():
-        if (name.startswith("bwagpu_debug_") or name in ("bwagpu_ctx_light_pack", "bwagpu_ctx_ungapped", "bwagpu_ctx_ungapped_right", "bwagpu_ctx_emu_finish")) and not hasattr(lib, name):
+        if (name.startswith("bwagpu_debug_") or name in ("bwagpu_ctx_light_pack", "bwagpu_ctx_ungapped", "bwagpu_ctx_ungapped_right", "bwagpu_ctx_emu_finish", "bwagpu_ctx_fused_launches")) and not hasattr(lib, name):
             continue
         fn = getattr(lib, name)
         fn.restype = res
diff --git a/bwa-flow_amd/python/bwagpu/engine.py b/bwa-flow_amd/python/bwagpu/engine.py
--- a/bwa-flow_amd/python/bwagpu/engine.py
+++ b/bwa-flow_amd/python/bwagpu/engine.py
@@ -327,6 +327,9 @@
                     "debug_spec_ungapped_right")
         return out.reshape(3, 2)
 
+    def fused_launches(self, mask: int = -1) -> int:
+        return self.lib.bwagpu_ctx_fused_launches(self.ctx, int(mask))
+
     def emu_finish(self, on: int = -1) -> int:
         return self.lib.bwagpu_ctx_emu_finish(self.ctx, int(on))
 
diff --git a/include/bwagpu.h b/include/bwagpu.h
--- a/include/bwagpu.h
+++ b/include/bwagpu.h
@@ -205,6 +205,7 @@
                             bwagpu_alnreg_t *dev_out, int32_t *dev_n, int64_t *dev_stats,
                             void *stream);
 int bwagpu_set_device_read_len(bwagpu_ctx_t *ctx, int32_t max_len);
+int bwagpu_ctx_fused_launches(bwagpu_ctx_t *ctx, int mask);
 
 int bwagpu_extend_batch(bwagpu_ctx_t *ctx, int32_t n_tasks, const bwagpu_ext_task_t *tasks,
                         const uint8_t *qpool, int64_t qpool_len, const uint8_t *tpool,
```
